# rednote-hilab/dots.ocr

Measured on AMD Instinct MI355X. Metric: pages/sec, dots.ocr 1.7B bf16, A4@200dpi page batch (preprocess + ViT + prefill + 1024-token greedy decode + detokenise), higher is better.
Workload: dtype bf16; 1 GPU; a4: 8 pages/GPU of 1654x2339 px -> 19824 patches, 5200 prompt tokens/page, max_new_tokens=1024, EOS disabled; pages_per_gpu=8, parallelism=dp1, decode_rows_in_flight=64

## Files before the change

### dots_ocr_amd/csrc/engine.hip

```cpp
#include "engine.h"

namespace engine {
namespace {
thread_local std::string g_create_error;

int dense_on(DotsEngine* e, hipStream_t st, uint8_t* aq, float* as, const bf16_t* A, const bf16_t* W, const uint8_t* W8, const float* wscale,
             const bf16_t* bias, const bf16_t* R, void* C, int64_t M, int N, int K, int ldc, int epi) {
    if (!W8) {
        CK(launch_gemm(st, A, W, bias, R, C, M, N, K, K, ldc, epi, wscale));
        return DOTS_OK;
    }
    CK(launch_quant_act_fp8(st, A, aq, as, M, K, K));
    CK(launch_gemm_fp8(st, aq, as, W8, wscale, bias, R, C, M, N, K, ldc, epi));
    return DOTS_OK;
}
int dense(DotsEngine* e, const bf16_t* A, const bf16_t* W, const uint8_t* W8, const float* wscale, const bf16_t* bias, const bf16_t* R, void* C,
          int64_t M, int N, int K, int ldc, int epi) {
    return dense_on(e, e->stream, e->act_q, e->act_s, A, W, W8, wscale, bias, R, C, M, N, K, ldc, epi);
}
int vdense(DotsEngine* e, const bf16_t* A, const bf16_t* W, const uint8_t* W8, const float* wscale, const bf16_t* bias, const bf16_t* R, void* C,
           int64_t M, int N, int K, int ldc, int epi) {
    return dense_on(e, e->vs, e->act_q_v, e->act_s_v, A, W, W8, wscale, bias, R, C, M, N, K, ldc, epi);
}

// ... 696 lines not shown
    if (n_eos) std::copy(eos_ids, eos_ids + n_eos, e->h_eos);
    e->out_cap = max_new_tokens;
    RET(prefill(e, input_ids, prompt_lens, B));

    CK(hipEventRecord(e->ev[4], s));
    const int n_splits = splits_for_ctx(e->cfg.max_seq_len);
    const bool use_graph = getenv("DOTS_OCR_NO_GRAPH") == nullptr;
    hipGraphExec_t exec = nullptr;
    hipGraphExec_t exec_part = nullptr;
    if (use_graph && max_new_tokens > 1) {
        if (e->step_graphs.size() >= 30) drop_step_graphs(e);
        if (e->s_vit) RET(step_graph(e, B, n_splits, max_new_tokens, &exec_part, 1));
        RET(step_graph(e, B, n_splits, max_new_tokens, &exec));
    }
    std::vector<int32_t> fin(DOTS_MAX_BATCH);
    int steps = 0;
    hipStream_t cur = s;
    for (int step = 1; step < max_new_tokens; ++step) {
        if (exec && (step & 15) == 1) RET(pick_decode_stream(e, &cur));
        if (exec) CK(hipGraphLaunch(cur != s && exec_part ? exec_part : exec, cur));
        else RET(decode_step_launches(e, n_splits));
        ++steps;
        if ((n_eos || e->stage.rows(ROW_STOP) > 0) && (step % 16 == 0)) {
            CK(hipMemcpyAsync(fin.data(), e->finished, B * 4, hipMemcpyDeviceToHost, cur));
            CK(hipStreamSynchronize(cur));
            bool all = true;
            for (int b = 0; b < B; ++b) all = all && fin[b];
            if (all) break;
        }
        if (exec && !n_eos && cur != s && (step & 63) == 0) CK(hipStreamSynchronize(cur));
    }
    RET(chain_streams(e, cur, s));
    CK(hipEventRecord(e->ev[5], s));
    CK(hipEventRecord(e->ev[7], s));
    e->steps_done = steps;
    std::vector<int32_t> tmp((size_t)B * max_new_tokens);
    CK(hipMemcpyAsync(tmp.data(), e->out_ids, tmp.size() * 4, hipMemcpyDeviceToHost, s));
    CK(hipMemcpyAsync(out_lens, e->out_lens, B * 4, hipMemcpyDeviceToHost, s));
    CK(hipStreamSynchronize(s));
    std::memcpy(out_ids, tmp.data(), tmp.size() * 4);

    e->stats.decode_steps = steps;
    int64_t newtok = 0;
    double kvb = 0;
    const double kv_tok = (double)e->cfg.num_layers * e->cfg.num_kv_heads * 128 * 2 * (e->kv8 ? 1 : 2);
    for (int b = 0; b < B; ++b) {
        newtok += out_lens[b];
        for (int st = 0; st < steps; ++st) kvb += (double)(prompt_lens[b] + st + 1) * kv_tok;
    }
    e->stats.new_tokens = newtok;
    e->stats.decode_bytes = (double)steps * decode_step_bytes(e->cfg) + kvb;
    return DOTS_OK;
}

int dots_get_stats(DotsEngine* e, DotsStats* out) {
    if (!e || !out) return DOTS_E_INVALID;
    CK(hipSetDevice(e->device));
    CK(hipStreamSynchronize(e->stream));
    if (e->s_vit) CK(hipStreamSynchronize(e->s_vit));
    auto elapsed = [&](hipEvent_t a, hipEvent_t b) {
        float ms = 0;
        if (hipEventElapsedTime(&ms, a, b) != hipSuccess) { (void)hipGetLastError(); ms = 0; }
        return ms;
    };
    auto el = [&](int a, int b) { return elapsed(e->ev[a], e->ev[b]); };
    e->stats.vit_ms = e->stats.vit_patches ? el(0, 1) : 0;
    e->stats.prefill_ms = e->stats.prefill_tokens ? el(2, 3) : 0;
    e->stats.decode_ms = e->stats.decode_steps ? el(4, 5) : 0;
    e->stats.total_ms = e->stats.decode_steps || e->stats.new_tokens ? el(6, 7) : 0;
    float a = 0;
    for (int i = 0; i < e->attn_pairs; ++i) a += elapsed(e->attn_ev[2 * i], e->attn_ev[2 * i + 1]);
    e->stats.vit_attn_ms = a;
    e->stats.vit_attn_launches = e->attn_pairs;
    *out = e->stats;
    return DOTS_OK;
}

int dots_preprocess_image(DotsEngine* e, const uint8_t* rgb, int on_device, int h, int w, int rh, int rw,
                          const int32_t* hcoef, const int32_t* hbounds, int hk, const int32_t* vcoef, const int32_t* vbounds, int vk,
                          const float* mean3, const float* std3, float rescale, float* out) {
    if (!e) return DOTS_E_INVALID;
    const DotsConfig& c = e->cfg;
    const int P = c.v_patch, m = c.v_merge;
    if (!rgb || !out || !mean3 || !std3 || h < 1 || w < 1 || rh < 1 || rw < 1) return e->fail(DOTS_E_INVALID, "bad preprocess arguments");
    if (rh % (P * m) || rw % (P * m)) return e->fail(DOTS_E_INVALID, "resized size %dx%d is not a multiple of patch*merge", rh, rw);
    if ((rw != w && (!hcoef || !hbounds || hk < 1)) || (rh != h && (!vcoef || !vbounds || vk < 1)))
        return e->fail(DOTS_E_INVALID, "missing resample table for a resized axis");
    if (c.v_channels != 3) return e->fail(DOTS_E_INVALID, "only 3-channel images are supported");
    CK(hipSetDevice(e->device));
    hipStream_t s = e->stream;
    auto grow = [&](uint8_t** p, size_t* cap, size_t need) -> hipError_t {
        if (need <= *cap) return hipSuccess;
        if (*p) { hipStreamSynchronize(s); e->release(*p); *p = nullptr; }
        *cap = need + need / 4;
        return e->alloc(p, *cap);
    };
    const size_t in_bytes = (size_t)h * w * 3, tmp_bytes = (size_t)h * rw * 3, out_bytes = (size_t)rh * rw * 3;
    const uint8_t* src = rgb;
    if (!on_device) {
        CK(grow(&e->pp_in, &e->pp_in_cap, in_bytes));
        CK(hipMemcpyAsync(e->pp_in, rgb, in_bytes, hipMemcpyHostToDevice, s));
        src = e->pp_in;
    }
    const size_t tab_ints = (rw != w ? (size_t)rw * (hk + 2) : 0) + (rh != h ? (size_t)rh * (vk + 2) : 0);
    if (tab_ints > e->pp_tab_cap) {
        if (e->pp_tab) { hipStreamSynchronize(s); e->release(e->pp_tab); e->pp_tab = nullptr; }
        e->pp_tab_cap = tab_ints + tab_ints / 4;
        CK(e->alloc(&e->pp_tab, e->pp_tab_cap));
    }
    int32_t* tab = e->pp_tab;
    if (rw != w) {
        CK(grow(&e->pp_tmp, &e->pp_tmp_cap, tmp_bytes));
        CK(hipMemcpyAsync(tab, hcoef, (size_t)rw * hk * 4, hipMemcpyHostToDevice, s));
        CK(hipMemcpyAsync(tab + (size_t)rw * hk, hbounds, (size_t)rw * 2 * 4, hipMemcpyHostToDevice, s));
        CK(launch_resize_h(s, src, e->pp_tmp, tab, tab + (size_t)rw * hk, hk, h, w, rw));
        src = e->pp_tmp;
        tab += (size_t)rw * (hk + 2);
    }
    if (rh != h) {
        CK(grow(&e->pp_out, &e->pp_out_cap, out_bytes));
        CK(hipMemcpyAsync(tab, vcoef, (size_t)rh * vk * 4, hipMemcpyHostToDevice, s));
        CK(hipMemcpyAsync(tab + (size_t)rh * vk, vbounds, (size_t)rh * 2 * 4, hipMemcpyHostToDevice, s));
        CK(launch_resize_v(s, src, e->pp_out, tab, tab + (size_t)rh * vk, vk, rw, rh));
        src = e->pp_out;
    }
    CK(launch_normalize_patchify(s, src, out, rw, rh / P, rw / P, P, m, rescale, mean3, std3));
    CK(hipStreamSynchronize(s));
    return DOTS_OK;
}

int dots_set_decode_plan(DotsEngine* e, int plan) {
    if (!e) return DOTS_E_INVALID;
    if (plan < 0 || plan > 5 || (plan & 6) == 6)
        return e->fail(DOTS_E_INVALID, "decode plan must be 0 (by stream) or 1 (partition plan on every step), + 2 (streaming attention) or + 4 (per-split attention)");
    const int part = plan & 1, stream = (plan & 2) ? 1 : (plan & 4) ? 0 : -1;
    if (part != e->force_part || stream != e->attn_stream) {
        e->force_part = part;
        e->attn_stream = stream;
        drop_step_graphs(e);
    }
    return DOTS_OK;
}

int dots_tower_tail(DotsEngine* e, int set, int* now) {
    if (!e) return DOTS_E_INVALID;
    if (set < -2 || set > e->cfg.v_layers) return e->fail(DOTS_E_INVALID, "tower tail must be -2 (query), -1 (adaptive) or 0 .. v_layers");
    if (set >= -1) e->tail_fixed = set;
    if (now) *now = e->tail_now;
    return DOTS_OK;
}

int dots_set_gemm_plan(DotsEngine* e, int plan) {
    if (!e) return DOTS_E_INVALID;
    if (plan < 0 || plan > 1) return e->fail(DOTS_E_INVALID, "gemm plan must be 0 (8-wave ping-pong) or 1 (one wave per SIMD)");
    gemm_set_plan(plan);
    return DOTS_OK;
}

int dots_get_logits(DotsEngine* e, float* out) {
    if (!e || !out) return DOTS_E_INVALID;
    if (e->B < 1) return e->fail(DOTS_E_STATE, "no prefilled batch");
    CK(hipSetDevice(e->device));
    CK(hipMemcpyAsync(out, e->d_logits, (size_t)e->B * e->cfg.vocab_size * 4, hipMemcpyDeviceToHost, e->stream));
    CK(hipStreamSynchronize(e->stream));
    return DOTS_OK;
}

int dots_set_next_tokens(DotsEngine* e, const int32_t* tokens, int B) {
    if (!e || !tokens || B != e->B) return e ? e->fail(DOTS_E_INVALID, "bad set_next_tokens arguments") : DOTS_E_INVALID;
    CK(hipSetDevice(e->device));
    CK(hipMemcpyAsync(e->cur_tokens, tokens, B * 4, hipMemcpyHostToDevice, e->stream));
    CK(hipStreamSynchronize(e->stream));
    return DOTS_OK;
}

int dots_get_last_tokens(DotsEngine* e, int32_t* out) {
    if (!e || !out) return DOTS_E_INVALID;
    if (e->B < 1) return e->fail(DOTS_E_STATE, "no prefilled batch");
    CK(hipSetDevice(e->device));
    std::vector<int32_t> lens(DOTS_MAX_BATCH), ids((size_t)DOTS_MAX_BATCH * std::max(1, e->out_cap));
    CK(hipMemcpyAsync(lens.data(), e->out_lens, e->B * 4, hipMemcpyDeviceToHost, e->stream));
    CK(hipMemcpyAsync(ids.data(), e->out_ids, (size_t)e->B * e->out_cap * 4, hipMemcpyDeviceToHost, e->stream));
    CK(hipStreamSynchronize(e->stream));
    for (int b = 0; b < e->B; ++b) out[b] = lens[b] > 0 ? ids[(size_t)b * e->out_cap + lens[b] - 1] : -1;
    return DOTS_OK;
}

int dots_debug_capture_hidden(DotsEngine* e, int64_t capacity_elems) {
    if (!e || capacity_elems < 0) return DOTS_E_INVALID;
    CK(hipSetDevice(e->device));
    CK(hipStreamSynchronize(e->stream));
    if (e->dbg_hidden) { e->release(e->dbg_hidden); e->dbg_hidden = nullptr; }
    e->dbg_cap = 0; e->dbg_vit_rows = e->dbg_lm_rows = 0;
    if (capacity_elems > 0) {
        CK(e->alloc(&e->dbg_hidden, (size_t)capacity_elems));
        e->dbg_cap = (size_t)capacity_elems;
    }
    return DOTS_OK;
}

int dots_debug_read_hidden(DotsEngine* e, int which, int layer, void* out_host, int64_t* rows_out) {
    if (!e || !out_host || !rows_out || !e->dbg_hidden) return e ? e->fail(DOTS_E_STATE, "hidden-state capture is off") : DOTS_E_INVALID;
    CK(hipSetDevice(e->device));
    const DotsConfig& c = e->cfg;
    const int64_t rows = which == 0 ? e->dbg_vit_rows : e->dbg_lm_rows;
    const int dim = which == 0 ? c.v_embed_dim : c.hidden_size, n_layers = which == 0 ? c.v_layers : c.num_layers;
    if (rows <= 0 || layer < 0 || layer >= n_layers) return e->fail(DOTS_E_INVALID, "no captured hidden state for layer %d", layer);
    const size_t off = (which == 0 ? 0 : (size_t)c.v_layers * e->dbg_vit_rows * c.v_embed_dim) + (size_t)layer * rows * dim;
    if (off + (size_t)rows * dim > e->dbg_cap) return e->fail(DOTS_E_CAPACITY, "capture buffer too small for layer %d", layer);
    CK(hipMemcpyAsync(out_host, e->dbg_hidden + off, (size_t)rows * dim * 2, hipMemcpyDeviceToHost, e->stream));
    CK(hipStreamSynchronize(e->stream));
    *rows_out = rows;
    return DOTS_OK;
}

int dots_debug_read_kv(DotsEngine* e, int layer, int seq, int pos0, int n, int which, void* out_host) {
    if (!e || !out_host) return e ? e->fail(DOTS_E_INVALID, "null argument") : DOTS_E_INVALID;
    const DotsConfig& c = e->cfg;
    if (layer < 0 || layer >= c.num_layers || seq < 0 || seq >= c.max_batch || pos0 < 0 || n < 1 || (which != 0 && which != 1) ||
        (int64_t)pos0 + n > (int64_t)e->max_pages * PAGE)
        return e->fail(DOTS_E_INVALID, "bad dots_debug_read_kv arguments (layer %d, row %d, positions %d + %d, which %d)", layer, seq, pos0, n, which);
    RET(dots_synchronize(e));
    const int Hkv = c.num_kv_heads, es = e->kv8 ? 1 : 2;
    const size_t page_bytes = (size_t)PAGE_ELEMS * es;
    const uint8_t* base = reinterpret_cast<const uint8_t*>(e->pool) + e->pool_layer_elems * 2 * layer;
    std::vector<uint8_t> pg(page_bytes);
    uint8_t* out = static_cast<uint8_t*>(out_host);
    for (int p = pos0 / PAGE; p <= (pos0 + n - 1) / PAGE; ++p) {
        const int page = e->hp_table[(size_t)seq * e->max_pages + p];
        if (page >= e->n_pool_pages) return e->fail(DOTS_E_STATE, "position %d of row %d is not in the KV cache", std::max(pos0, p * PAGE), seq);
        for (int h = 0; h < Hkv; ++h) {
            CK(hipMemcpyAsync(pg.data(), base + ((size_t)(page * Hkv + h) * 2 + which) * page_bytes, page_bytes, hipMemcpyDeviceToHost, e->stream));
            CK(hipStreamSynchronize(e->stream));
            for (int pos = std::max(pos0, p * PAGE); pos < std::min(pos0 + n, (p + 1) * PAGE); ++pos)
                for (int d = 0; d < 128; ++d) {
                    const int key = pos & (PAGE - 1), el = which == 0 ? k_chunk(key, d) * 8 + (d & 7) : v_off(key, d);
                    const size_t o = ((size_t)h * n + (pos - pos0)) * 128 + d;
                    if (e->kv8) out[o] = pg[kv8_byte(el)];
                    else std::memcpy(out + o * 2, pg.data() + (size_t)el * 2, 2);
                }
        }
    }
    return DOTS_OK;
}

int dots_synchronize(DotsEngine* e) {
    if (!e) return DOTS_E_INVALID;
    CK(hipSetDevice(e->device));
    if (e->s_vit) CK(hipStreamSynchronize(e->s_vit));
    if (e->s_dec) CK(hipStreamSynchronize(e->s_dec));
    CK(hipStreamSynchronize(e->stream));
    return DOTS_OK;
}

int dots_dev_alloc(DotsEngine* e, int64_t bytes, void** out) {
    if (!e || !out || bytes < 0) return DOTS_E_INVALID;
    CK(hipSetDevice(e->device));
    uint8_t* p = nullptr;
    CK(e->alloc(&p, (size_t)bytes));
    *out = p;
    return DOTS_OK;
}
int dots_dev_free(DotsEngine* e, void* p) {
    if (!e) return DOTS_E_INVALID;
    CK(hipSetDevice(e->device));
    CK(hipStreamSynchronize(e->stream));
    e->release(p);
    return DOTS_OK;
}
int dots_memcpy_h2d(DotsEngine* e, void* dst, const void* src, int64_t bytes) {
    if (!e) return DOTS_E_INVALID;
    CK(hipSetDevice(e->device));
    CK(hipMemcpyAsync(dst, src, bytes, hipMemcpyHostToDevice, e->stream));
    CK(hipStreamSynchronize(e->stream));
    return DOTS_OK;
}
int dots_memcpy_d2h(DotsEngine* e, void* dst, const void* src, int64_t bytes) {
    if (!e) return DOTS_E_INVALID;
    CK(hipSetDevice(e->device));
    CK(hipMemcpyAsync(dst, src, bytes, hipMemcpyDeviceToHost, e->stream));
    CK(hipStreamSynchronize(e->stream));
    return DOTS_OK;
}
}
```

### dots_ocr_amd/csrc/gemm.hip

```cpp
#include <cstdlib>
#include <utility>

#include "common.h"
#include "kernels.h"

namespace {

constexpr int BM = 128, BN = 128, BK = 64;
constexpr int TILE_BYTES = 128 * 128;
#ifndef GEMM_GROUP_M
#define GEMM_GROUP_M 8
#endif
constexpr int GROUP_M = GEMM_GROUP_M;

DEVI float gelu_erf(float x) { return 0.5f * x * (1.0f + erff(x * 0.70710678118654752440f)); }
#ifdef GEMM_EXACT_SILU
DEVI float silu(float x) { return x / (1.0f + __expf(-x)); }
#else
DEVI float silu(float x) {
    const float d = 1.0f + __expf(fminf(-x, 80.f));
    const float r = __builtin_amdgcn_rcpf(d);
    const float q = x * r;
    return __builtin_fmaf(__builtin_fmaf(-q, d, x), r, q);
}
#endif

template <int EPI, int FN, int FM = 2>
DEVI void gemm_epilogue(const f32x16 (&acc)[FN][FM], const bf16_t* __restrict__ bias, const float* __restrict__ colscale, const bf16_t* R,
                        void* Cout, int M, int ldc, int nw0, int mw0, int l31, int hi, const float* __restrict__ rowscale = nullptr) {
#pragma unroll
    for (int fm = 0; fm < FM; ++fm) {
        const int m = mw0 + fm * 32 + l31;
        if (m >= M) continue;
        const float rs = rowscale ? rowscale[m] : 1.f;
        if constexpr (EPI == EPI_SWIGLU) {
            bf16_t* C = reinterpret_cast<bf16_t*>(Cout);
#pragma unroll
            for (int fp = 0; fp < FN / 2; ++fp)
#pragma unroll
            for (int rq = 0; rq < 4; ++rq) {
                const int nb = nw0 + fp * 64 + 8 * rq + 4 * hi;
                float o[4];
#pragma unroll
                for (int e = 0; e < 4; ++e) {
                    float g = acc[2 * fp][fm][4 * rq + e], u = acc[2 * fp + 1][fm][4 * rq + e];
                    if (colscale) { g *= colscale[nb + e] * rs; u *= colscale[nb + 32 + e] * rs; }
                    if (bias) { g += bf2f(bias[nb + e]); u += bf2f(bias[nb + 32 + e]); }
                    o[e] = silu(g) * u;
                }
                const int j = (nw0 + fp * 64) / 2 + 8 * rq + 4 * hi;
                u32x2 pk = {pack_bf2(o[0], o[1]), pack_bf2(o[2], o[3])};
                *reinterpret_cast<u32x2*>(C + (size_t)m * ldc + j) = pk;
            }
        } else {
#pragma unroll
            for (int fn = 0; fn < FN; ++fn)
#pragma unroll
                for (int rq = 0; rq < 4; ++rq) {
                    const int nb = nw0 + fn * 32 + 8 * rq + 4 * hi;
                    float o[4];
#pragma unroll
                    for (int e = 0; e < 4; ++e) o[e] = acc[fn][fm][4 * rq + e];
                    if (colscale) {
                        const f32x4 sc = *reinterpret_cast<const f32x4*>(colscale + nb);
#pragma unroll
                        for (int e = 0; e < 4; ++e) o[e] *= sc[e] * rs;
                    }
                    if (bias) {
                        u32x2 bb = *reinterpret_cast<const u32x2*>(bias + nb);
                        o[0] += lo_bf(bb[0]); o[1] += hi_bf(bb[0]); o[2] += lo_bf(bb[1]); o[3] += hi_bf(bb[1]);
                    }
                    if constexpr (EPI == EPI_RESIDUAL) {
                        u32x2 rr = *reinterpret_cast<const u32x2*>(R + (size_t)m * ldc + nb);
                        o[0] += lo_bf(rr[0]); o[1] += hi_bf(rr[0]); o[2] += lo_bf(rr[1]); o[3] += hi_bf(rr[1]);
                    }
                    if constexpr (EPI == EPI_GELU) {
#pragma unroll
                        for (int e = 0; e < 4; ++e) o[e] = gelu_erf(o[e]);
                    }
                    if constexpr (EPI == EPI_F32) {
                        f32x4 v = {o[0], o[1], o[2], o[3]};
                        *reinterpret_cast<f32x4*>(reinterpret_cast<float*>(Cout) + (size_t)m * ldc + nb) = v;
                    } else {
                        u32x2 pk = {pack_bf2(o[0], o[1]), pack_bf2(o[2], o[3])};
                        *reinterpret_cast<u32x2*>(reinterpret_cast<bf16_t*>(Cout) + (size_t)m * ldc + nb) = pk;
                    }
                }
        }
    }
}

template <int EPI, int FM = 2>
DEVI void gemm_epilogue_lds(const f32x16 (&acc)[4][FM], const bf16_t* __restrict__ bias, const float* __restrict__ colscale, const bf16_t* R,
                            bf16_t* __restrict__ C, int M, int ldc, int nw0, int mw0, int l, char* stage, const float* __restrict__ rowscale = nullptr) {
    const int hi = l >> 5, l31 = l & 31;
    constexpr bool SW = EPI == EPI_SWIGLU;
    const int rrow = SW ? (l >> 3) : (l >> 4);
    const int gcol = SW ? ((l & 7) >> 2) * 64 + (l & 3) * 8 : (l & 15) * 8;
    float sc0[8], sc1[8], bi0[8], bi1[8];
#pragma unroll
    for (int e = 0; e < 8; ++e) {
        sc0[e] = colscale ? colscale[nw0 + gcol + e] : 1.f;
        bi0[e] = bias ? bf2f(bias[nw0 + gcol + e]) : 0.f;
        sc1[e] = (SW && colscale) ? colscale[nw0 + gcol + 32 + e] : 1.f;
        bi1[e] = (SW && bias) ? bf2f(bias[nw0 + gcol + 32 + e]) : 0.f;
    }
#pragma unroll
    for (int fm = 0; fm < FM; ++fm) {
#pragma unroll
        for (int fn = 0; fn < 4; ++fn)
#pragma unroll
            for (int rq = 0; rq < 4; ++rq) {
                const int slot = (fn * 8 + rq * 2 + hi) ^ ((l31 & 15) << 1);
                const f32x4 v = {acc[fn][fm][4 * rq], acc[fn][fm][4 * rq + 1], acc[fn][fm][4 * rq + 2], acc[fn][fm][4 * rq + 3]};
                *reinterpret_cast<f32x4*>(stage + l31 * 512 + slot * 16) = v;
            }
#pragma unroll
        for (int it = 0; it < (SW ? 4 : 8); ++it) {
            const int row = it * (SW ? 8 : 4) + rrow;
            const int m = mw0 + fm * 32 + row;
            const int sw = (row & 15) << 1;
            const char* rp = stage + row * 512;
            const int s0 = gcol >> 2;
            const f32x4 a0 = *reinterpret_cast<const f32x4*>(rp + ((s0 ^ sw) << 4)), a1 = *reinterpret_cast<const f32x4*>(rp + (((s0 + 1) ^ sw) << 4));
            float o[8] = {a0[0], a0[1], a0[2], a0[3], a1[0], a1[1], a1[2], a1[3]};
            const float rs = rowscale ? rowscale[min(m, M - 1)] : 1.f;
#pragma unroll
            for (int e = 0; e < 8; ++e) o[e] = o[e] * (sc0[e] * rs) + bi0[e];
            if constexpr (SW) {
                const f32x4 u0 = *reinterpret_cast<const f32x4*>(rp + (((s0 + 8) ^ sw) << 4)), u1 = *reinterpret_cast<const f32x4*>(rp + (((s0 + 9) ^ sw) << 4));
                const float u[8] = {u0[0], u0[1], u0[2], u0[3], u1[0], u1[1], u1[2], u1[3]};
#pragma unroll
                for (int e = 0; e < 8; ++e) o[e] = silu(o[e]) * (u[e] * (sc1[e] * rs) + bi1[e]);
            }
            if (m >= M) continue;
            const int col = SW ? nw0 / 2 + ((l & 7) >> 2) * 32 + (l & 3) * 8 : nw0 + gcol;
            if constexpr (EPI == EPI_RESIDUAL) {
                const u32x4 rr = *reinterpret_cast<const u32x4*>(R + (size_t)m * ldc + col);
#pragma unroll
                for (int e = 0; e < 4; ++e) { o[2 * e] += lo_bf(rr[e]); o[2 * e + 1] += hi_bf(rr[e]); }
            }
            if constexpr (EPI == EPI_GELU) {
#pragma unroll
                for (int e = 0; e < 8; ++e) o[e] = gelu_erf(o[e]);
            }
            const u32x4 pk = {pack_bf2(o[0], o[1]), pack_bf2(o[2], o[3]), pack_bf2(o[4], o[5]), pack_bf2(o[6], o[7])};
            *reinterpret_cast<u32x4*>(C + (size_t)m * ldc + col) = pk;
        }
    }
}

template <int EPI>
__global__ __launch_bounds__(256, 2) void gemm_bf16_kernel(
// ... 178 lines not shown

    const int tid = threadIdx.x;
    const int l = tid & 63;
    const int w = __builtin_amdgcn_readfirstlane(tid >> 6);
    const int hi = l >> 5, l31 = l & 31;
    const int grp = w >> 2;

    int bid = xcd_remap(blockIdx.x, m_tiles * n_tiles);
    const int per_group = group_m * n_tiles;
    const int g = bid / per_group;
    const int first_m = g * group_m;
    const int gsz = min(m_tiles - first_m, group_m);
    const int in_grp = bid - g * per_group;
    const int tm = first_m + in_grp % gsz;
    const int tn = in_grp / gsz;
    const int m0 = tm * BM2, n0 = tn * BN2;

    const bf16_t* gw[2];
    const bf16_t* gx[2];
#pragma unroll
    for (int i = 0; i < 2; ++i) {
        const int row = (i * 8 + w) * 16 + (l >> 2);
        const int slot = (l & 3) ^ ((l >> 4) & 3);
        gw[i] = W + (size_t)(n0 + row) * K + slot * 8;
        gx[i] = A + (size_t)min(m0 + row, M - 1) * lda + slot * 8;
    }
    auto issue_sub = [&](int p) {
        char* base = smem2 + (p & (PP_STAGES - 1)) * SUB_STAGE;
#ifdef PP_DMA_SAME
        p &= 1;
#endif
#pragma unroll
        for (int i = 0; i < 2; ++i) {
            __builtin_amdgcn_global_load_lds((const __attribute__((address_space(1))) void*)(gw[i] + p * SUBK),
                                             (__attribute__((address_space(3))) void*)(base + (i * 8 + w) * 1024), 16, 0, 0);
            __builtin_amdgcn_global_load_lds((const __attribute__((address_space(1))) void*)(gx[i] + p * SUBK),
                                             (__attribute__((address_space(3))) void*)(base + SUB_OP + (i * 8 + w) * 1024), 16, 0, 0);
        }
    };

    const int wn = w >> 2, wm = w & 3;
    const int rsw = (l31 >> 2) & 3;
    const int a_off = (wn * 128 + l31) * 64;
    const int b_off = SUB_OP + (wm * 64 + l31) * 64;

    f32x16 acc[4][2];
#pragma unroll
    for (int i = 0; i < 4; ++i)
#pragma unroll
        for (int j = 0; j < 2; ++j)
#pragma unroll
            for (int r = 0; r < 16; ++r) acc[i][j][r] = 0.f;

    const int ns = K / SUBK;
    issue_sub(0);
    if (ns > 1) issue_sub(1);
    if (ns > 2) issue_sub(2);
    if (ns > 2) asm volatile("s_waitcnt vmcnt(8)" ::: "memory");
    else if (ns > 1) asm volatile("s_waitcnt vmcnt(4)" ::: "memory");
    else asm volatile("s_waitcnt vmcnt(0)" ::: "memory");
    __builtin_amdgcn_s_barrier();
    if (grp == 1) __builtin_amdgcn_s_barrier();
    __builtin_amdgcn_sched_barrier(0);

    for (int p = 0; p < ns; ++p) {
        const char* base = smem2 + (p & (PP_STAGES - 1)) * SUB_STAGE;
        bf16x8 af[2][4], bf_[2][2];
#ifdef PP_NO_LDS
        if (p == 0)
#endif
#pragma unroll
        for (int ks = 0; ks < 2; ++ks) {
            const int slot = ((ks * 2 + hi) ^ rsw) << 4;
            bf_[ks][0] = *reinterpret_cast<const bf16x8*>(base + b_off + slot);
            bf_[ks][1] = *reinterpret_cast<const bf16x8*>(base + b_off + 32 * 64 + slot);
#pragma unroll
            for (int fn = 0; fn < 4; ++fn) af[ks][fn] = *reinterpret_cast<const bf16x8*>(base + a_off + fn * 32 * 64 + slot);
        }
        __builtin_amdgcn_sched_barrier(0);
#ifdef PP_NO_DMA
        if (false) {
#else
        if (p + PP_LOOKAHEAD < ns) {
#endif
            issue_sub(p + PP_LOOKAHEAD);
            asm volatile("s_waitcnt vmcnt(8)" ::: "memory");
        } else {
            asm volatile("s_waitcnt vmcnt(0)" ::: "memory");
        }
        asm volatile("s_waitcnt lgkmcnt(0)" ::: "memory");
        __builtin_amdgcn_sched_barrier(0);
        __builtin_amdgcn_s_barrier();
        __builtin_amdgcn_sched_barrier(0);
        __builtin_amdgcn_s_setprio(1);
#ifdef PP_NO_MFMA
        if (p == 0)
#endif
#pragma unroll
        for (int ks = 0; ks < 2; ++ks)
#pragma unroll
            for (int fn = 0; fn < 4; ++fn) {
                acc[fn][0] = __builtin_amdgcn_mfma_f32_32x32x16_bf16(af[ks][fn], bf_[ks][0], acc[fn][0], 0, 0, 0);
                acc[fn][1] = __builtin_amdgcn_mfma_f32_32x32x16_bf16(af[ks][fn], bf_[ks][1], acc[fn][1], 0, 0, 0);
            }
#ifdef PP_NO_MFMA
        else { PINV(af[0][0]); PINV(af[1][3]); PINV(bf_[0][0]); PINV(bf_[1][1]); }
#endif
        __builtin_amdgcn_s_setprio(0);
        __builtin_amdgcn_sched_barrier(0);
        if (grp == 0 || p + 1 < ns) __builtin_amdgcn_s_barrier();
        __builtin_amdgcn_sched_barrier(0);
    }
#ifdef PP_NO_STORE
#pragma unroll
    for (int i = 0; i < 4; ++i) { PINV(acc[i][0]); PINV(acc[i][1]); }
#else
    if constexpr (EPI == EPI_F32 || EPI == EPI_SWIGLU) {
        gemm_epilogue<EPI, 4>(acc, bias, colscale, R, Cout, M, ldc, n0 + wn * 128, m0 + wm * 64, l31, hi);
    } else {
        __syncthreads();
        gemm_epilogue_lds<EPI>(acc, bias, colscale, R, reinterpret_cast<bf16_t*>(Cout), M, ldc, n0 + wn * 128, m0 + wm * 64, l, smem2 + w * 16384);
    }
#endif
}

constexpr int W4_UNIT = 256 * 128, W4_RING = 5;

struct W4Cols { float sc0[8], bi0[8], sc1[8], bi1[8]; };
template <bool SW>
DEVI void w4_load_cols(W4Cols& cc, const bf16_t* __restrict__ bias, const float* __restrict__ colscale, int nw0, int l) {
    const int gcol = SW ? ((l & 7) >> 2) * 64 + (l & 3) * 8 : (l & 15) * 8;
    u32x4 b0 = {0, 0, 0, 0}, b1 = {0, 0, 0, 0};
    f32x4 s00 = {1.f, 1.f, 1.f, 1.f}, s01 = s00, s10 = s00, s11 = s00;
    if (bias) {
        b0 = *reinterpret_cast<const u32x4*>(bias + nw0 + gcol);
        if (SW) b1 = *reinterpret_cast<const u32x4*>(bias + nw0 + gcol + 32);
    }
    if (colscale) {
        s00 = *reinterpret_cast<const f32x4*>(colscale + nw0 + gcol);
        s01 = *reinterpret_cast<const f32x4*>(colscale + nw0 + gcol + 4);
        if (SW) {
            s10 = *reinterpret_cast<const f32x4*>(colscale + nw0 + gcol + 32);
            s11 = *reinterpret_cast<const f32x4*>(colscale + nw0 + gcol + 36);
        }
    }
#pragma unroll
    for (int e = 0; e < 4; ++e) {
        cc.sc0[e] = s00[e]; cc.sc0[4 + e] = s01[e]; cc.sc1[e] = s10[e]; cc.sc1[4 + e] = s11[e];
        cc.bi0[2 * e] = lo_bf(b0[e]); cc.bi0[2 * e + 1] = hi_bf(b0[e]);
        cc.bi1[2 * e] = lo_bf(b1[e]); cc.bi1[2 * e + 1] = hi_bf(b1[e]);
    }
}

template <int EPI, bool FULL>
DEVI void w4_epilogue_lds(const f32x16 (&acc)[4][4], const W4Cols& cc, bool has_cols, const bf16_t* R,
                          bf16_t* __restrict__ C, int M, int ldc, int nw0, int mw0, int l, char* stage2) {
    const int hi = l >> 5, l31 = l & 31;
    constexpr bool SW = EPI == EPI_SWIGLU;
    constexpr int ITS = SW ? 4 : 8, RPI = SW ? 8 : 4;
    const int rrow = SW ? (l >> 3) : (l >> 4);
    const int gcol = SW ? ((l & 7) >> 2) * 64 + (l & 3) * 8 : (l & 15) * 8;
    const int col = SW ? nw0 / 2 + ((l & 7) >> 2) * 32 + (l & 3) * 8 : nw0 + gcol;
    u32x4 rr[2][8];
    auto load_r = [&](int fm, u32x4 (&dst)[8]) {
        if constexpr (EPI == EPI_RESIDUAL) {
#pragma unroll
            for (int it = 0; it < ITS; ++it) {
                const int m = FULL ? mw0 + fm * 32 + it * RPI + rrow : min(mw0 + fm * 32 + it * RPI + rrow, M - 1);
                dst[it] = *reinterpret_cast<const u32x4*>(R + (size_t)m * ldc + col);
            }
        }
    };
#ifdef W4_OLD_SWZ
    auto swz = [](int row) { return (row & 15) << 1; };
#else
    auto swz = [](int row) { return ((row & 15) << 1) ^ (row & 1) ^ ((row & 2) << 2); };
#endif
    const int wslot = swz(l31);
    char* const wrow = stage2 + l31 * 512;
#define W4_PUT(FM, IMG)                                                                                                   \
    _Pragma("unroll") for (int fn = 0; fn < 4; ++fn) _Pragma("unroll") for (int rq = 0; rq < 4; ++rq) {                     \
        const f32x4 v = {acc[fn][FM][4 * rq], acc[fn][FM][4 * rq + 1], acc[fn][FM][4 * rq + 2], acc[fn][FM][4 * rq + 3]};   \
        *reinterpret_cast<f32x4*>(wrow + (IMG) * 16384 + (((fn * 8 + rq * 2 + hi) ^ wslot) << 4)) = v;                      \
    }
    load_r(0, rr[0]);
    W4_PUT(0, 0)
#pragma unroll
    for (int fm = 0; fm < 4; ++fm) {
        if (fm + 1 < 4) {
            load_r(fm + 1, rr[(fm + 1) & 1]);
            if (fm == 0) { W4_PUT(1, 1) } else if (fm == 1) { W4_PUT(2, 0) } else { W4_PUT(3, 1) }
        }
        __builtin_amdgcn_sched_barrier(0);
        const char* img = stage2 + (fm & 1) * 16384;
        f32x4 a[ITS][SW ? 4 : 2];
#pragma unroll
        for (int it = 0; it < ITS; ++it) {
            const int row = it * RPI + rrow;
            const int sw = swz(row);
            const char* rp = img + row * 512;
            const int s0 = gcol >> 2;
            a[it][0] = *reinterpret_cast<const f32x4*>(rp + ((s0 ^ sw) << 4));
            a[it][1] = *reinterpret_cast<const f32x4*>(rp + (((s0 + 1) ^ sw) << 4));
            if constexpr (SW) {
                a[it][2] = *reinterpret_cast<const f32x4*>(rp + (((s0 + 8) ^ sw) << 4));
                a[it][3] = *reinterpret_cast<const f32x4*>(rp + (((s0 + 9) ^ sw) << 4));
            }
        }
        __builtin_amdgcn_sched_barrier(0);
#pragma unroll
        for (int it = 0; it < ITS; ++it) {
            const int m = mw0 + fm * 32 + it * RPI + rrow;
            float o[8] = {a[it][0][0], a[it][0][1], a[it][0][2], a[it][0][3], a[it][1][0], a[it][1][1], a[it][1][2], a[it][1][3]};
            float u[8];
            if constexpr (SW) {
#pragma unroll
                for (int e = 0; e < 8; ++e) u[e] = a[it][2 + (e >> 2)][e & 3];
            }
            if (has_cols) {
#pragma unroll
                for (int e = 0; e < 8; ++e) o[e] = o[e] * cc.sc0[e] + cc.bi0[e];
                if constexpr (SW) {
#pragma unroll
                    for (int e = 0; e < 8; ++e) u[e] = u[e] * cc.sc1[e] + cc.bi1[e];
                }
            }
            if constexpr (SW) {
#pragma unroll
                for (int e = 0; e < 8; ++e) o[e] = silu(o[e]) * u[e];
            }
            if constexpr (EPI == EPI_RESIDUAL) {
                const u32x4 r4 = rr[fm & 1][it];
#pragma unroll
                for (int e = 0; e < 4; ++e) { o[2 * e] += lo_bf(r4[e]); o[2 * e + 1] += hi_bf(r4[e]); }
            }
            if constexpr (EPI == EPI_GELU) {
#pragma unroll
                for (int e = 0; e < 8; ++e) o[e] = gelu_erf(o[e]);
            }
            if (FULL || m < M) {
                const u32x4 pk = {pack_bf2(o[0], o[1]), pack_bf2(o[2], o[3]), pack_bf2(o[4], o[5]), pack_bf2(o[6], o[7])};
                *reinterpret_cast<u32x4*>(C + (size_t)m * ldc + col) = pk;
            }
        }
        __builtin_amdgcn_sched_barrier(0);
    }
#undef W4_PUT
}

DEVI void w4_load_cols_rope(W4Cols& cc, const bf16_t* __restrict__ bias, const float* __restrict__ colscale, int nw0, int l) {
    const int gcol = (l & 15) * 8, pcol = gcol ^ 64;
    u32x4 b0 = {0, 0, 0, 0}, b1 = {0, 0, 0, 0};
    f32x4 s00 = {1.f, 1.f, 1.f, 1.f}, s01 = s00, s10 = s00, s11 = s00;
    if (bias) {
        b0 = *reinterpret_cast<const u32x4*>(bias + nw0 + gcol);
        b1 = *reinterpret_cast<const u32x4*>(bias + nw0 + pcol);
    }
    if (colscale) {
        s00 = *reinterpret_cast<const f32x4*>(colscale + nw0 + gcol);
        s01 = *reinterpret_cast<const f32x4*>(colscale + nw0 + gcol + 4);
        s10 = *reinterpret_cast<const f32x4*>(colscale + nw0 + pcol);
        s11 = *reinterpret_cast<const f32x4*>(colscale + nw0 + pcol + 4);
    }
#pragma unroll
    for (int e = 0; e < 4; ++e) {
        cc.sc0[e] = s00[e]; cc.sc0[4 + e] = s01[e]; cc.sc1[e] = s10[e]; cc.sc1[4 + e] = s11[e];
        cc.bi0[2 * e] = lo_bf(b0[e]); cc.bi0[2 * e + 1] = hi_bf(b0[e]);
        cc.bi1[2 * e] = lo_bf(b1[e]); cc.bi1[2 * e + 1] = hi_bf(b1[e]);
    }
}

template <bool FULL>
DEVI void w4_epilogue_qkrope(const f32x16 (&acc)[4][4], const W4Cols& cc, bool has_cols, const float2* __restrict__ cs, bf16_t* __restrict__ dst,
                             int M, int mw0, int l, char* stage2) {
    const int hi = l >> 5, l31 = l & 31;
    const int rrow = l >> 4, gcol = (l & 15) * 8;
    const bool lo_half = (l & 8) == 0;
    const float2* const tab = cs + (gcol & 63);
    auto swz = [](int row) { return ((row & 15) << 1) ^ (row & 1) ^ ((row & 2) << 2); };
    const int wslot = swz(l31);
    char* const wrow = stage2 + l31 * 512;
#define W4_PUT(FM, IMG)                                                                                                   \
    _Pragma("unroll") for (int fn = 0; fn < 4; ++fn) _Pragma("unroll") for (int rq = 0; rq < 4; ++rq) {                     \
        const f32x4 v = {acc[fn][FM][4 * rq], acc[fn][FM][4 * rq + 1], acc[fn][FM][4 * rq + 2], acc[fn][FM][4 * rq + 3]};   \
        *reinterpret_cast<f32x4*>(wrow + (IMG) * 16384 + (((fn * 8 + rq * 2 + hi) ^ wslot) << 4)) = v;                      \
    }
    f32x4 tb[2][2][4];
    auto load_t = [&](int qb, f32x4 (&d)[2][4]) {
#pragma unroll
        for (int it = 0; it < 2; ++it) {
            const int m = FULL ? mw0 + qb * 8 + it * 4 + rrow : min(mw0 + qb * 8 + it * 4 + rrow, M - 1);
            const f32x4* tp = reinterpret_cast<const f32x4*>(tab + (size_t)m * 64);
#pragma unroll
            for (int c = 0; c < 4; ++c) d[it][c] = tp[c];
        }
    };
    load_t(0, tb[0]);
    W4_PUT(0, 0)
#pragma unroll
    for (int qb = 0; qb < 16; ++qb) {
        const int fm = qb >> 2;
        if (qb + 1 < 16) load_t(qb + 1, tb[(qb + 1) & 1]);
        if ((qb & 3) == 0 && fm + 1 < 4) {
            if (fm == 0) { W4_PUT(1, 1) } else if (fm == 1) { W4_PUT(2, 0) } else { W4_PUT(3, 1) }
        }
        __builtin_amdgcn_sched_barrier(0);
        const char* img = stage2 + (fm & 1) * 16384;
        f32x4 a[2][4];
#pragma unroll
        for (int it = 0; it < 2; ++it) {
            const int row = (qb & 3) * 8 + it * 4 + rrow;
            const int sw = swz(row);
            const char* rp = img + row * 512;
            const int s0 = gcol >> 2;
            a[it][0] = *reinterpret_cast<const f32x4*>(rp + ((s0 ^ sw) << 4));
            a[it][1] = *reinterpret_cast<const f32x4*>(rp + (((s0 + 1) ^ sw) << 4));
            a[it][2] = *reinterpret_cast<const f32x4*>(rp + ((s0 ^ 16 ^ sw) << 4));
            a[it][3] = *reinterpret_cast<const f32x4*>(rp + (((s0 + 1) ^ 16 ^ sw) << 4));
        }
        __builtin_amdgcn_sched_barrier(0);
#pragma unroll
        for (int it = 0; it < 2; ++it) {
            const int m = mw0 + qb * 8 + it * 4 + rrow;
            float o[8] = {a[it][0][0], a[it][0][1], a[it][0][2], a[it][0][3], a[it][1][0], a[it][1][1], a[it][1][2], a[it][1][3]};
            float u[8] = {a[it][2][0], a[it][2][1], a[it][2][2], a[it][2][3], a[it][3][0], a[it][3][1], a[it][3][2], a[it][3][3]};
            if (has_cols) {
#pragma unroll
                for (int e = 0; e < 8; ++e) { o[e] = o[e] * cc.sc0[e] + cc.bi0[e]; u[e] = u[e] * cc.sc1[e] + cc.bi1[e]; }
            }
            uint32_t pk[4];
#pragma unroll
            for (int e = 0; e < 4; ++e) {
                const uint32_t ow = pack_bf2(o[2 * e], o[2 * e + 1]), uw = pack_bf2(u[2 * e], u[2 * e + 1]);
                const float x0 = lo_bf(ow), x1 = hi_bf(ow), y0 = lo_bf(uw), y1 = hi_bf(uw);
                const f32x4 t4 = tb[qb & 1][it][e];
                const float f0 = lo_half ? x0 : y0, g0 = lo_half ? t4[0] : t4[1], m0 = lo_half ? y0 : x0, n0_ = lo_half ? t4[1] : t4[0];
                const float p0 = m0 * n0_, p1 = y1 * t4[3];
                const float r0 = __builtin_fmaf(f0, g0, lo_half ? -p0 : p0), r1 = __builtin_fmaf(x1, t4[2], lo_half ? -p1 : p1);
                pk[e] = pack_bf2(r0, r1);
            }
            if (FULL || m < M) *reinterpret_cast<u32x4*>(dst + (size_t)m * 128 + gcol) = u32x4{pk[0], pk[1], pk[2], pk[3]};
        }
        __builtin_amdgcn_sched_barrier(0);
    }
#undef W4_PUT
}

template <int... I, class F> DEVI void gemm_static_for_impl(std::integer_sequence<int, I...>, F&& f) { (f(std::integral_constant<int, I>{}), ...); }
template <int N, class F> DEVI void gemm_static_for(F&& f) { gemm_static_for_impl(std::make_integer_sequence<int, N>{}, f); }

template <int EPI>
DEVI void gemm_bf16_w4_body(
    const bf16_t* __restrict__ A, const bf16_t* __restrict__ W, const bf16_t* __restrict__ bias,
    const float* __restrict__ colscale, const bf16_t* R, void* Cout, int M, int N, int K, int lda, int ldc, int m_tiles, int n_tiles, int group_m, const QkRope& rope) {
    extern __shared__ __attribute__((aligned(16))) char smem2[];
    (void)rope;

    const int tid = threadIdx.x;
    const int l = tid & 63;
    const int w = __builtin_amdgcn_readfirstlane(tid >> 6);
    const int hi = l >> 5, l31 = l & 31;

    int bid = xcd_remap(blockIdx.x, m_tiles * n_tiles);
    const int per_group = group_m * n_tiles;
    const int g = bid / per_group;
    const int first_m = g * group_m;
    const int gsz = min(m_tiles - first_m, group_m);
    const int in_grp = bid - g * per_group;
    const int tm = first_m + in_grp % gsz;
    const int tn = in_grp / gsz;
    const int m0 = tm * BM2, n0 = tn * BN2;

    const int prow = 8 * w + (l >> 3);
    const int chunk = ((l & 7) ^ ((4 * w + (l >> 4)) & 7)) << 4;
    const int w_src = prow * (K * 2) + chunk;
    int x_src[8];
#pragma unroll
    for (int i = 0; i < 8; ++i) x_src[i] = (min(m0 + prow + 32 * i, M - 1) - m0) * (lda * 2) + chunk;
    const __amdgpu_buffer_rsrc_t rw = __builtin_amdgcn_make_buffer_rsrc((void*)(W + (size_t)n0 * K), 0, 0x7ffffff0, 0x00020000);
    const __amdgpu_buffer_rsrc_t rx = __builtin_amdgcn_make_buffer_rsrc((void*)(A + (size_t)m0 * lda), 0, 0x7ffffff0, 0x00020000);
    const int w_step = 32 * K * 2;
    auto dma_w = [&](int t, int slot, int i) {
        __builtin_amdgcn_raw_ptr_buffer_load_lds(rw, (__attribute__((address_space(3))) void*)(smem2 + slot * W4_UNIT + (w + 4 * i) * 1024), 16, w_src,
                                                 t * 128 + i * w_step, 0, 0);
    };
    auto dma_x = [&](int t, int slot, int i) {
        __builtin_amdgcn_raw_ptr_buffer_load_lds(rx, (__attribute__((address_space(3))) void*)(smem2 + slot * W4_UNIT + (w + 4 * i) * 1024), 16, x_src[i],
                                                 t * 128, 0, 0);
    };

    const int wn = w >> 1, wm = w & 1;
    const int rsw = (l31 >> 1) & 7;
    const int lane_sw = ((hi ^ (rsw & 1)) << 4) | ((rsw >> 1) << 5);
    const int lds0 = (int)(uintptr_t)(__attribute__((address_space(3))) char*)smem2;
    const int a_lane = lds0 + (wn * 128 + l31) * 128 + lane_sw;
    const int b_lane = lds0 + (wm * 128 + l31) * 128 + lane_sw;
    auto frag = [&](int base, int ks, int f) {
        return *reinterpret_cast<const __attribute__((address_space(3))) bf16x8*>((uintptr_t)(uint32_t)((base ^ (ks << 5)) + f * 4096));
    };

#ifdef W4_PROF
    const unsigned long long pt0 = __builtin_amdgcn_s_memtime(), pw0 = wall_clock64();
#endif
    W4Cols cols;
    if constexpr (EPI == EPI_QKROPE) w4_load_cols_rope(cols, bias, colscale, n0 + wn * 128, l);
    else if constexpr (EPI != EPI_F32) w4_load_cols<EPI == EPI_SWIGLU>(cols, bias, colscale, n0 + wn * 128, l);

    f32x16 acc[4][4];
#pragma unroll
    for (int i = 0; i < 4; ++i)
#pragma unroll
        for (int j = 0; j < 4; ++j)
#pragma unroll
            for (int r = 0; r < 16; ++r) acc[i][j][r] = 0.f;

    const int nt = K / BK;
#ifdef W4_STAGGER
    if (blockIdx.x < 256) {
        const int naps = ((blockIdx.x >> 3) & 7) * nt * W4_STAGGER / 8;
        for (int i = 0; i < naps; ++i) __builtin_amdgcn_s_sleep(8);
    }
#endif
#pragma unroll
    for (int u = 0; u < 4; ++u)
#pragma unroll
        for (int i = 0; i < 8; ++i) {
            if (u & 1) dma_x(u >> 1, u, i);
            else dma_w(u >> 1, u, i);
        }
    asm volatile("s_waitcnt vmcnt(16)" ::: "memory");
    __builtin_amdgcn_s_barrier();
    bf16x8 fa[2][4], fb[2][4];
#pragma unroll
    for (int f = 0; f < 4; ++f) { fa[0][f] = frag(a_lane, 0, f); fb[0][f] = frag(b_lane + W4_UNIT, 0, f); }
#ifdef W4_PROF
    const unsigned long long pt1 = __builtin_amdgcn_s_memtime(), pw1 = wall_clock64();
#endif

    auto tile_body = [&](auto mode_c, int t, int u0) {
        constexpr int MODE = decltype(mode_c)::value;
        const int s1 = u0 + 1 >= W4_RING ? u0 + 1 - W4_RING : u0 + 1, s2 = u0 + 2 >= W4_RING ? u0 + 2 - W4_RING : u0 + 2;
        const int s3 = u0 + 3 >= W4_RING ? u0 + 3 - W4_RING : u0 + 3, s4 = u0 + 4 >= W4_RING ? u0 + 4 - W4_RING : u0 + 4;
        const int aw = a_lane + u0 * W4_UNIT, ax = b_lane + s1 * W4_UNIT;
        const int awn = a_lane + s2 * W4_UNIT, axn = b_lane + s3 * W4_UNIT;
        gemm_static_for<64>([&acc, &fa, &fb, &frag, &dma_w, &dma_x, aw, ax, awn, axn, t, u0, s4](auto gc) {
            constexpr int gp = decltype(gc)::value;
            (void)acc; (void)t; (void)u0; (void)s4; (void)dma_w; (void)dma_x;
            constexpr int ks = gp >> 4, idx = gp & 15, fn = idx >> 2, fm = idx & 3, cur = ks & 1;
            if constexpr (gp == 48 && MODE < 2) {
                if constexpr (MODE == 0) asm volatile("s_waitcnt vmcnt(8) lgkmcnt(0)" ::: "memory");
                else asm volatile("s_waitcnt vmcnt(0) lgkmcnt(0)" ::: "memory");
                __builtin_amdgcn_s_barrier();
            }
            if constexpr (idx < 8 && (ks < 3 || MODE < 2)) {
                constexpr int f = idx & 3;
                if constexpr (ks < 3) {
                    if constexpr (idx < 4) fa[cur ^ 1][f] = frag(aw, ks + 1, f);
                    else fb[cur ^ 1][f] = frag(ax, ks + 1, f);
                } else {
                    if constexpr (idx < 4) fa[cur ^ 1][f] = frag(awn, 0, f);
                    else fb[cur ^ 1][f] = frag(axn, 0, f);
                }
            }
#ifndef W4_NO_DMA
            if constexpr (MODE == 0) {
                if constexpr (gp == 8 || gp == 11 || gp == 14 || gp == 24 || gp == 27 || gp == 30 || gp == 40 || gp == 43) {
                    constexpr int i = gp < 16 ? (gp - 8) / 3 : gp < 32 ? 3 + (gp - 24) / 3 : 6 + (gp - 40) / 3;
                    dma_w(t + 2, s4, i);
                }
                if constexpr (gp >= 56) dma_x(t + 2, u0, gp - 56);
            }
#endif
            asm volatile("v_mfma_f32_32x32x16_bf16 %[d], %[a], %[b], %[d]" : [d] "+a"(acc[fn][fm]) : [a] "v"(fa[cur][fn]), [b] "v"(fb[cur][fm]));
        });
    };
    int u0 = 0;
    for (int t = 0; t < nt - 2; ++t) {
        tile_body(std::integral_constant<int, 0>{}, t, u0);
        u0 = u0 + 2 >= W4_RING ? u0 + 2 - W4_RING : u0 + 2;
    }
    tile_body(std::integral_constant<int, 1>{}, nt - 2, u0);
    u0 = u0 + 2 >= W4_RING ? u0 + 2 - W4_RING : u0 + 2;
    tile_body(std::integral_constant<int, 2>{}, nt - 1, u0);

#ifdef W4_PROF
    const unsigned long long pt2 = __builtin_amdgcn_s_memtime(), pw2 = wall_clock64();
#endif
    __syncthreads();
#ifdef W4_NO_STORE
#pragma unroll
    for (int i = 0; i < 4; ++i)
#pragma unroll
        for (int j = 0; j < 4; ++j) asm volatile("" ::"a"(acc[i][j]));
    return;
#endif
#ifdef W4_OLD_EPILOGUE
    if constexpr (EPI == EPI_F32 || EPI == EPI_SWIGLU) {
        gemm_epilogue<EPI, 4, 4>(acc, bias, colscale, R, Cout, M, ldc, n0 + wn * 128, m0 + wm * 128, l31, hi);
    } else {
        gemm_epilogue_lds<EPI, 4>(acc, bias, colscale, R, reinterpret_cast<bf16_t*>(Cout), M, ldc, n0 + wn * 128, m0 + wm * 128, l, smem2 + w * 16384);
    }
#else
    if constexpr (EPI == EPI_QKROPE) {
        const int head = (n0 + wn * 128) >> 7;
        const bool full = m0 + wm * 128 + 128 <= M, has_cols = bias != nullptr || colscale != nullptr;
        if (head < rope.n_rope_heads) {
            bf16_t* dst = head < rope.Hq ? rope.q + (size_t)head * rope.T * 128 : rope.k + (size_t)(head - rope.Hq) * rope.T * 128;
            if (full) w4_epilogue_qkrope<true>(acc, cols, has_cols, rope.cs, dst, M, m0 + wm * 128, l, smem2 + w * 32768);
            else w4_epilogue_qkrope<false>(acc, cols, has_cols, rope.cs, dst, M, m0 + wm * 128, l, smem2 + w * 32768);
        } else if (full) {
            w4_epilogue_lds<EPI_NONE, true>(acc, cols, has_cols, R, reinterpret_cast<bf16_t*>(Cout), M, ldc, n0 + wn * 128, m0 + wm * 128, l, smem2 + w * 32768);
        } else {
            w4_epilogue_lds<EPI_NONE, false>(acc, cols, has_cols, R, reinterpret_cast<bf16_t*>(Cout), M, ldc, n0 + wn * 128, m0 + wm * 128, l, smem2 + w * 32768);
        }
    } else if constexpr (EPI == EPI_F32) {
        gemm_epilogue<EPI, 4, 4>(acc, bias, colscale, R, Cout, M, ldc, n0 + wn * 128, m0 + wm * 128, l31, hi);
    } else if (m0 + wm * 128 + 128 <= M) {
        w4_epilogue_lds<EPI, true>(acc, cols, bias != nullptr || colscale != nullptr, R, reinterpret_cast<bf16_t*>(Cout), M, ldc, n0 + wn * 128, m0 + wm * 128, l, smem2 + w * 32768);
    } else {
        w4_epilogue_lds<EPI, false>(acc, cols, bias != nullptr || colscale != nullptr, R, reinterpret_cast<bf16_t*>(Cout), M, ldc, n0 + wn * 128, m0 + wm * 128, l, smem2 + w * 32768);
    }
#endif
#ifdef W4_PROF
    const unsigned long long pt2b = __builtin_amdgcn_s_memtime();
    asm volatile("s_waitcnt vmcnt(0)" ::: "memory");
    const unsigned long long pt3 = __builtin_amdgcn_s_memtime(), pw3 = wall_clock64();
    if ((blockIdx.x == 1000 || blockIdx.x == 2001 || blockIdx.x == 3002) && tid == 0)
        printf("W4_PROF epi %d N %d K %d blk %d: prologue %llu cyc / %.2f us, main loop %llu cyc / %.2f us (%.0f cyc per K tile), epilogue + drain %llu cyc / %.2f us; issue %llu drain %llu\n", EPI, N, K,
               (int)blockIdx.x, pt1 - pt0, (pw1 - pw0) * 0.01, pt2 - pt1, (pw2 - pw1) * 0.01, (double)(pt2 - pt1) / nt, pt3 - pt2, (pw3 - pw2) * 0.01, pt2b - pt2, pt3 - pt2b);
#endif
}

template <int EPI>
__global__ __launch_bounds__(256) void gemm_bf16_w4_kernel(
    const bf16_t* __restrict__ A, const bf16_t* __restrict__ W, const bf16_t* __restrict__ bias,
    const float* __restrict__ colscale, const bf16_t* R, void* Cout, int M, int N, int K, int lda, int ldc, int m_tiles, int n_tiles, int group_m) {
    gemm_bf16_w4_body<EPI>(A, W, bias, colscale, R, Cout, M, N, K, lda, ldc, m_tiles, n_tiles, group_m, QkRope{});
}
__global__ __launch_bounds__(256) void gemm_bf16_w4_qkrope_kernel(
    const bf16_t* __restrict__ A, const bf16_t* __restrict__ W, const bf16_t* __restrict__ bias,
    const float* __restrict__ colscale, void* Cout, int M, int N, int K, int lda, int ldc, int m_tiles, int n_tiles, int group_m, QkRope rope) {
    gemm_bf16_w4_body<EPI_QKROPE>(A, W, bias, colscale, nullptr, Cout, M, N, K, lda, ldc, m_tiles, n_tiles, group_m, rope);
}

typedef __attribute__((ext_vector_type(8))) int i32x8;

template <int EPI>
__global__ __launch_bounds__(512, 2) void gemm_fp8_256pp_kernel(
    const uint8_t* __restrict__ A, const float* __restrict__ rowscale, const uint8_t* __restrict__ W, const float* __restrict__ colscale,
    const bf16_t* __restrict__ bias, const bf16_t* R, void* Cout, int M, int N, int K, int ldc, int m_tiles, int n_tiles, int group_m) {
    extern __shared__ __attribute__((aligned(16))) char smem2[];
    constexpr int SUBK8 = 64;

    const int tid = threadIdx.x;
    const int l = tid & 63;
    const int w = __builtin_amdgcn_readfirstlane(tid >> 6);
    const int hi = l >> 5, l31 = l & 31;
    const int grp = w >> 2;

    int bid = xcd_remap(blockIdx.x, m_tiles * n_tiles);
    const int per_group = group_m * n_tiles;
    const int g = bid / per_group;
    const int first_m = g * group_m;
    const int gsz = min(m_tiles - first_m, group_m);
    const int in_grp = bid - g * per_group;
    const int tm = first_m + in_grp % gsz;
    const int tn = in_grp / gsz;
    const int m0 = tm * BM2, n0 = tn * BN2;

    const uint8_t* gw[2];
    const uint8_t* gx[2];
#pragma unroll
    for (int i = 0; i < 2; ++i) {
        const int row = (i * 8 + w) * 16 + (l >> 2);
        const int slot = (l & 3) ^ ((l >> 4) & 3);
        gw[i] = W + (size_t)(n0 + row) * K + slot * 16;
        gx[i] = A + (size_t)min(m0 + row, M - 1) * K + slot * 16;
    }
    auto issue_sub = [&](int p) {
        char* base = smem2 + (p & (PP_STAGES - 1)) * SUB_STAGE;
#pragma unroll
        for (int i = 0; i < 2; ++i) {
            __builtin_amdgcn_global_load_lds((const __attribute__((address_space(1))) void*)(gw[i] + p * SUBK8),
                                             (__attribute__((address_space(3))) void*)(base + (i * 8 + w) * 1024), 16, 0, 0);
            __builtin_amdgcn_global_load_lds((const __attribute__((address_space(1))) void*)(gx[i] + p * SUBK8),
                                             (__attribute__((address_space(3))) void*)(base + SUB_OP + (i * 8 + w) * 1024), 16, 0, 0);
        }
    };

    const int wn = w >> 2, wm = w & 3;
    const int rsw = (l31 >> 2) & 3;
    const int a_off = (wn * 128 + l31) * 64;
    const int b_off = SUB_OP + (wm * 64 + l31) * 64;
    const int s_lo = ((2 * hi) ^ rsw) << 4, s_hi = ((2 * hi + 1) ^ rsw) << 4;

    f32x16 acc[4][2];
#pragma unroll
    for (int i = 0; i < 4; ++i)
#pragma unroll
        for (int j = 0; j < 2; ++j)
#pragma unroll
            for (int r = 0; r < 16; ++r) acc[i][j][r] = 0.f;

    const int ns = K / SUBK8;
    issue_sub(0);
    if (ns > 1) issue_sub(1);
    if (ns > 2) issue_sub(2);
    if (ns > 2) asm volatile("s_waitcnt vmcnt(8)" ::: "memory");
    else if (ns > 1) asm volatile("s_waitcnt vmcnt(4)" ::: "memory");
    else asm volatile("s_waitcnt vmcnt(0)" ::: "memory");
    __builtin_amdgcn_s_barrier();
    if (grp == 1) __builtin_amdgcn_s_barrier();
    __builtin_amdgcn_sched_barrier(0);

    auto frag = [&](const char* rowp) {
        const u32x4 lo = *reinterpret_cast<const u32x4*>(rowp + s_lo), hi4 = *reinterpret_cast<const u32x4*>(rowp + s_hi);
        const i32x8 v = {(int)lo[0], (int)lo[1], (int)lo[2], (int)lo[3], (int)hi4[0], (int)hi4[1], (int)hi4[2], (int)hi4[3]};
        return v;
    };
    for (int p = 0; p < ns; ++p) {
        const char* base = smem2 + (p & (PP_STAGES - 1)) * SUB_STAGE;
        i32x8 af[4], bf_[2];
        bf_[0] = frag(base + b_off);
        bf_[1] = frag(base + b_off + 32 * 64);
#pragma unroll
        for (int fn = 0; fn < 4; ++fn) af[fn] = frag(base + a_off + fn * 32 * 64);
        __builtin_amdgcn_sched_barrier(0);
        if (p + PP_LOOKAHEAD < ns) {
            issue_sub(p + PP_LOOKAHEAD);
            asm volatile("s_waitcnt vmcnt(8)" ::: "memory");
        } else {
            asm volatile("s_waitcnt vmcnt(0)" ::: "memory");
        }
        asm volatile("s_waitcnt lgkmcnt(0)" ::: "memory");
        __builtin_amdgcn_sched_barrier(0);
        __builtin_amdgcn_s_barrier();
        __builtin_amdgcn_sched_barrier(0);
        __builtin_amdgcn_s_setprio(1);
#pragma unroll
        for (int fn = 0; fn < 4; ++fn) {
            acc[fn][0] = __builtin_amdgcn_mfma_scale_f32_32x32x64_f8f6f4(af[fn], bf_[0], acc[fn][0], 0, 0, 0, 0x7f7f7f7f, 0, 0x7f7f7f7f);
            acc[fn][1] = __builtin_amdgcn_mfma_scale_f32_32x32x64_f8f6f4(af[fn], bf_[1], acc[fn][1], 0, 0, 0, 0x7f7f7f7f, 0, 0x7f7f7f7f);
        }
        __builtin_amdgcn_s_setprio(0);
        __builtin_amdgcn_sched_barrier(0);
        if (grp == 0 || p + 1 < ns) __builtin_amdgcn_s_barrier();
        __builtin_amdgcn_sched_barrier(0);
    }
    if constexpr (EPI == EPI_SWIGLU) {
        gemm_epilogue<EPI, 4>(acc, bias, colscale, R, Cout, M, ldc, n0 + wn * 128, m0 + wm * 64, l31, hi, rowscale);
    } else {
        __syncthreads();
        gemm_epilogue_lds<EPI>(acc, bias, colscale, R, reinterpret_cast<bf16_t*>(Cout), M, ldc, n0 + wn * 128, m0 + wm * 64, l, smem2 + w * 16384, rowscale);
    }
}

}

static int raster_group_m(int row_bytes) {
    const int panel = 256 * row_bytes;
    return panel >= (4 << 20) ? 2 : panel >= (3 << 19) ? 4 : GROUP_M;
}

static int g_gemm_plan = -1;
int gemm_get_plan() {
    int p = __atomic_load_n(&g_gemm_plan, __ATOMIC_RELAXED);
    if (p < 0) {
        const char* ev = getenv("DOTS_OCR_GEMM_PLAN");
        p = ev ? (atoi(ev) != 0) : 1;
        __atomic_store_n(&g_gemm_plan, p, __ATOMIC_RELAXED);
    }
    return p;
}
void gemm_set_plan(int plan) { __atomic_store_n(&g_gemm_plan, plan != 0, __ATOMIC_RELAXED); }

template <int E>
static hipError_t launch_256(hipStream_t s, const bf16_t* A, const bf16_t* W, const bf16_t* bias, const float* colscale, const bf16_t* R, void* C,
                                int M, int N, int K, int lda, int ldc) {
    static uint32_t configured = 0;
    int dev = 0;
    hipError_t e = hipGetDevice(&dev);
    if (e != hipSuccess) return e;
    const uint32_t bit = 1u << (dev & 31);
    if (!(__atomic_load_n(&configured, __ATOMIC_ACQUIRE) & bit)) {
        e = hipFuncSetAttribute(reinterpret_cast<const void*>(&gemm_bf16_256_kernel<E>), hipFuncAttributeMaxDynamicSharedMemorySize, 2 * STAGE2);
        if (e != hipSuccess) return e;
        __atomic_fetch_or(&configured, bit, __ATOMIC_RELEASE);
    }
    const int m_tiles = (M + BM2 - 1) / BM2, n_tiles = N / BN2;
    static const bool lockstep = getenv("DOTS_OCR_GEMM_LOCKSTEP") != nullptr;
    if (lockstep || ldc % 8 != 0) {
        hipLaunchKernelGGL(gemm_bf16_256_kernel<E>, dim3(m_tiles * n_tiles), dim3(512), 2 * STAGE2, s, A, W, bias, colscale, R, C, M, N, K,
                           lda, ldc, m_tiles, n_tiles);
        return hipGetLastError();
    }
    if (gemm_get_plan() == 1 && K / BK >= 3) {
        static uint32_t configured_w4 = 0;
        if (!(__atomic_load_n(&configured_w4, __ATOMIC_ACQUIRE) & bit)) {
            e = hipFuncSetAttribute(reinterpret_cast<const void*>(&gemm_bf16_w4_kernel<E>), hipFuncAttributeMaxDynamicSharedMemorySize, W4_RING * W4_UNIT);
            if (e != hipSuccess) return e;
            __atomic_fetch_or(&configured_w4, bit, __ATOMIC_RELEASE);
        }
        hipLaunchKernelGGL(gemm_bf16_w4_kernel<E>, dim3(m_tiles * n_tiles), dim3(256), W4_RING * W4_UNIT, s, A, W, bias, colscale, R, C, M, N, K,
                           lda, ldc, m_tiles, n_tiles, raster_group_m(K * 2));
        return hipGetLastError();
    }
    static uint32_t configured_pp = 0;
    if (!(__atomic_load_n(&configured_pp, __ATOMIC_ACQUIRE) & bit)) {
        e = hipFuncSetAttribute(reinterpret_cast<const void*>(&gemm_bf16_256pp_kernel<E>), hipFuncAttributeMaxDynamicSharedMemorySize,
                                PP_STAGES * SUB_STAGE);
        if (e != hipSuccess) return e;
        __atomic_fetch_or(&configured_pp, bit, __ATOMIC_RELEASE);
    }
    hipLaunchKernelGGL(gemm_bf16_256pp_kernel<E>, dim3(m_tiles * n_tiles), dim3(512), PP_STAGES * SUB_STAGE, s, A, W, bias, colscale, R, C, M, N, K,
                       lda, ldc, m_tiles, n_tiles, raster_group_m(K * 2));
    return hipGetLastError();
}

hipError_t launch_gemm(hipStream_t s, const bf16_t* A, const bf16_t* W, const bf16_t* bias, const bf16_t* R,
                       void* C, int64_t M, int N, int K, int lda, int ldc, int epi, const float* colscale) {
    if (M <= 0) return hipSuccess;
    if (N % BN != 0 || K % BK != 0 || (lda % 8) != 0 || (ldc % 4) != 0) return hipErrorInvalidValue;
    static const bool force_small = getenv("DOTS_OCR_GEMM_128") != nullptr;
    if (N % BN2 == 0 && !force_small) {
        switch (epi) {
            case EPI_NONE: return launch_256<EPI_NONE>(s, A, W, bias, colscale, R, C, (int)M, N, K, lda, ldc);
            case EPI_RESIDUAL: return launch_256<EPI_RESIDUAL>(s, A, W, bias, colscale, R, C, (int)M, N, K, lda, ldc);
            case EPI_SWIGLU: return launch_256<EPI_SWIGLU>(s, A, W, bias, colscale, R, C, (int)M, N, K, lda, ldc);
            case EPI_GELU: return launch_256<EPI_GELU>(s, A, W, bias, colscale, R, C, (int)M, N, K, lda, ldc);
            case EPI_F32: return launch_256<EPI_F32>(s, A, W, bias, colscale, R, C, (int)M, N, K, lda, ldc);
            default: return hipErrorInvalidValue;
        }
    }
    const int m_tiles = (int)((M + BM - 1) / BM), n_tiles = N / BN;
    dim3 grid(m_tiles * n_tiles), block(256);
#define LAUNCH(E)                                                                                       \
    hipLaunchKernelGGL(gemm_bf16_kernel<E>, grid, block, 0, s, A, W, bias, colscale, R, C, (int)M, N, K, lda, ldc, \
                       m_tiles, n_tiles)
    switch (epi) {
        case EPI_NONE: LAUNCH(EPI_NONE); break;
        case EPI_RESIDUAL: LAUNCH(EPI_RESIDUAL); break;
        case EPI_SWIGLU: LAUNCH(EPI_SWIGLU); break;
        case EPI_GELU: LAUNCH(EPI_GELU); break;
        case EPI_F32: LAUNCH(EPI_F32); break;
        default: return hipErrorInvalidValue;
    }
#undef LAUNCH
    return hipGetLastError();
}

hipError_t launch_gemm_qk_rope(hipStream_t s, const bf16_t* A, const bf16_t* W, const bf16_t* bias, bf16_t* qkv, int64_t M, int N, int K, int lda, int ldc,
                               const float2* cs, bf16_t* q, bf16_t* k, int Hq, int Hkv) {
    static const bool off = getenv("DOTS_OCR_QK_FUSE") && atoi(getenv("DOTS_OCR_QK_FUSE")) == 0;
    static const bool lockstep = getenv("DOTS_OCR_GEMM_LOCKSTEP") != nullptr, force_small = getenv("DOTS_OCR_GEMM_128") != nullptr;
    if (off || lockstep || force_small || gemm_get_plan() != 1 || N != (Hq + 2 * Hkv) * 128 || N % BN2 != 0 || K % BK != 0 || K / BK < 3 || lda % 8 != 0 || ldc % 8 != 0 ||
        !cs || !q || !k || M > 0x7fffffff)
        return hipErrorNotSupported;
    if (M <= 0) return hipSuccess;
    static uint32_t configured = 0;
    int dev = 0;
    hipError_t e = hipGetDevice(&dev);
    if (e != hipSuccess) return e;
    const uint32_t bit = 1u << (dev & 31);
    if (!(__atomic_load_n(&configured, __ATOMIC_ACQUIRE) & bit)) {
        e = hipFuncSetAttribute(reinterpret_cast<const void*>(&gemm_bf16_w4_qkrope_kernel), hipFuncAttributeMaxDynamicSharedMemorySize, W4_RING * W4_UNIT);
        if (e != hipSuccess) return e;
        __atomic_fetch_or(&configured, bit, __ATOMIC_RELEASE);
    }
    const int m_tiles = (int)((M + BM2 - 1) / BM2), n_tiles = N / BN2;
    const QkRope rope{cs, q, k, (long long)M, Hq, Hq + Hkv};
    hipLaunchKernelGGL(gemm_bf16_w4_qkrope_kernel, dim3(m_tiles * n_tiles), dim3(256), W4_RING * W4_UNIT, s, A, W, bias, (const float*)nullptr, (void*)qkv, (int)M, N, K,
                       lda, ldc, m_tiles, n_tiles, raster_group_m(K * 2), rope);
    return hipGetLastError();
}

bool gemm_fp8_supports(int N, int K) { return N % BN2 == 0 && K % 64 == 0; }

template <int E>
static hipError_t launch_fp8_t(hipStream_t s, const uint8_t* Aq, const float* rowscale, const uint8_t* Wq, const float* colscale, const bf16_t* bias,
                               const bf16_t* R, void* C, int M, int N, int K, int ldc) {
    static uint32_t configured = 0;
    int dev = 0;
    hipError_t e = hipGetDevice(&dev);
    if (e != hipSuccess) return e;
    const uint32_t bit = 1u << (dev & 31);
    if (!(__atomic_load_n(&configured, __ATOMIC_ACQUIRE) & bit)) {
        e = hipFuncSetAttribute(reinterpret_cast<const void*>(&gemm_fp8_256pp_kernel<E>), hipFuncAttributeMaxDynamicSharedMemorySize, PP_STAGES * SUB_STAGE);
        if (e != hipSuccess) return e;
        __atomic_fetch_or(&configured, bit, __ATOMIC_RELEASE);
    }
    const int m_tiles = (M + BM2 - 1) / BM2, n_tiles = N / BN2;
    hipLaunchKernelGGL(gemm_fp8_256pp_kernel<E>, dim3(m_tiles * n_tiles), dim3(512), PP_STAGES * SUB_STAGE, s, Aq, rowscale, Wq, colscale, bias, R, C, M, N, K,
                       ldc, m_tiles, n_tiles, raster_group_m(K));
    return hipGetLastError();
}

hipError_t launch_gemm_fp8(hipStream_t s, const uint8_t* Aq, const float* rowscale, const uint8_t* Wq, const float* colscale, const bf16_t* bias,
                           const bf16_t* R, void* C, int64_t M, int N, int K, int ldc, int epi) {
    if (M <= 0) return hipSuccess;
    if (!gemm_fp8_supports(N, K) || ldc % 8 != 0 || !rowscale || !colscale) return hipErrorInvalidValue;
    switch (epi) {
        case EPI_NONE: return launch_fp8_t<EPI_NONE>(s, Aq, rowscale, Wq, colscale, bias, R, C, (int)M, N, K, ldc);
        case EPI_RESIDUAL: return launch_fp8_t<EPI_RESIDUAL>(s, Aq, rowscale, Wq, colscale, bias, R, C, (int)M, N, K, ldc);
        case EPI_SWIGLU: return launch_fp8_t<EPI_SWIGLU>(s, Aq, rowscale, Wq, colscale, bias, R, C, (int)M, N, K, ldc);
        case EPI_GELU: return launch_fp8_t<EPI_GELU>(s, Aq, rowscale, Wq, colscale, bias, R, C, (int)M, N, K, ldc);
        default: return hipErrorInvalidValue;
    }
}
```

### dots_ocr_amd/csrc/ops.hip

```cpp
#include "engine.h"

using namespace engine;

namespace {
int op_weight(DotsEngine* e, Scratch& sc, const bf16_t* w, int64_t rows, int K, int Hq, int Hkv, bool qkv, int fp8, void** wd, float** scale) {
    *scale = nullptr;
    if (fp8) {
        bf16_t* q = nullptr;
        uint8_t* d = nullptr;
        CK(sc.get(&q, (size_t)rows * K));
        CK(sc.get(scale, (size_t)rows));
        CK(sc.get(&d, (size_t)((rows + 15) / 16 * 16) * K));
        CK(hipMemcpyAsync(q, w, (size_t)rows * K * 2, hipMemcpyDeviceToDevice, e->stream));
        CK(launch_quant_rows_fp8(e->stream, q, *scale, rows, K));
        CK(launch_pack_frag_fp8(e->stream, q, d, rows, K, qkv ? (Hq + Hkv) * 128 : 0));
        *wd = d;
    } else {
        bf16_t* d = nullptr;
        CK(sc.get(&d, (size_t)((rows + 15) / 16 * 16) * K));
        if (qkv) CK(launch_pack_frag_qkv(e->stream, w, d, Hq, Hkv, K));
        else CK(launch_pack_frag(e->stream, w, d, rows, K));
        *wd = d;
    }
    return DOTS_OK;
// ... 101 lines not shown
    CK(sc.get(&own_d, B));
    CK(sc.get(&thr, B));
    CK(sc.get(&cnt, (size_t)B * V));
    CK(sc.get(&seen, (size_t)B * W));
    CK(sc.get(&pen, (size_t)B * V));
    CK(sc.get(&pval, (size_t)B * 64));
    CK(sc.get(&pidx, (size_t)B * 64));
    CK(sc.get(&cur, B));
    CK(sc.get(&ctx, B));
    CK(sc.get(&ids, (size_t)B * (hist_stride + 1)));
    CK(sc.get(&lens, B));
    CK(sc.get(&fin, B));
    CK(hipMemcpyAsync(tab, rp.data(), B * sizeof(RowParams), hipMemcpyHostToDevice, e->stream));
    CK(hipMemcpyAsync(own_d, own.data(), B * 4, hipMemcpyHostToDevice, e->stream));
    CK(launch_pen_history(e->stream, hist_dev, hist_lens_dev, hist_stride, n_prompt_dev, B, V, cnt, seen, lens));
    StepState st;
    st.cur_tokens = cur; st.ctx_len = ctx; st.out_ids = ids; st.out_lens = lens; st.finished = fin;
    st.eos_ids = e->eos_ids; st.sel = nullptr; st.max_len = nullptr;
    st.n_eos = rules_host ? e->n_eos : 0; st.out_stride = hist_stride + 1; st.cap = hist_stride + 2; st.advance_ctx = 0;
    RowRules* rtab = nullptr;
    float* img = nullptr;
    if (rules_host) {
        int32_t* stage = nullptr;
        CK(sc.get(&rtab, DOTS_MAX_BATCH));
        CK(sc.get(&img, (size_t)B * V));
        CK(sc.get(&stage, (size_t)V + 2 * DOTS_MAX_LOGIT_BIAS));
        for (int b = 0; b < B; ++b) {
            const DotsLogitRules& r = rules_host[b];
            if (!r.n_bias && !r.allowed_ids && !r.min_tokens && !r.n_stop && !r.ignore_eos) continue;
            RowRules rr;
            RET(check_logit_rules(e, r, V, e->h_eos, e->n_eos, &rr));
            const int n_allowed = r.allowed_ids ? r.n_allowed : 0;
            if (n_allowed) CK(hipMemcpyAsync(stage, r.allowed_ids, (size_t)n_allowed * 4, hipMemcpyHostToDevice, e->stream));
            if (r.n_bias) {
                CK(hipMemcpyAsync(stage + V, r.bias_ids, (size_t)r.n_bias * 4, hipMemcpyHostToDevice, e->stream));
                CK(hipMemcpyAsync(stage + V + DOTS_MAX_LOGIT_BIAS, r.bias_values, (size_t)r.n_bias * 4, hipMemcpyHostToDevice, e->stream));
            }
            CK(launch_set_row_rules(e->stream, rtab, img, b, V, rr, stage, n_allowed, stage + V,
                                    reinterpret_cast<const float*>(stage + V + DOTS_MAX_LOGIT_BIAS), r.n_bias));
            CK(hipStreamSynchronize(e->stream));
        }
        if (n_gen_host) CK(hipMemcpyAsync(lens, n_gen_host, B * 4, hipMemcpyHostToDevice, e->stream));
    }
    RowSel rs{tab, own_d, cnt, seen, pen, thr, 0, rtab, img, GuideSel{}, NgramSel{}};
    if (ngram_host) {
        RowNgram* ntab = nullptr;
        uint32_t* nmask = nullptr;
        CK(sc.get(&ntab, DOTS_MAX_BATCH));
        CK(sc.get(&nmask, (size_t)B * ngram_mask_words(V)));
        CK(hipMemcpyAsync(ntab, ngrams.data(), DOTS_MAX_BATCH * sizeof(RowNgram), hipMemcpyHostToDevice, e->stream));
        CK(launch_ngram_history(e->stream, hist_dev, hist_lens_dev, hist_stride, n_prompt_dev, B, ids, st.out_stride));
        rs.ngram = NgramSel{ntab, nmask, ngram_mask_words(V), V};
    }
    RowGuide* gtab = nullptr;
    int32_t* gstates = nullptr;
    if (guide_ids_host) {
        uint32_t* gmask = nullptr;
        CK(sc.get(&gtab, DOTS_MAX_BATCH));
        CK(sc.get(&gstates, DOTS_MAX_BATCH));
        CK(sc.get(&gmask, (size_t)B * guide_mask_words(V)));
        std::vector<RowGuide> rows(DOTS_MAX_BATCH, RowGuide{});
        for (int b = 0; b < B; ++b) {
            if (guide_ids_host[b] < 0) continue;
            const DotsEngine::Guide& g = e->guides[guide_ids_host[b]];
            rows[b] = RowGuide{g.table, g.accepting, g.n_states, g.start, states_host[b], 0};
        }
        CK(hipMemcpyAsync(gtab, rows.data(), DOTS_MAX_BATCH * sizeof(RowGuide), hipMemcpyHostToDevice, e->stream));
        CK(hipMemcpyAsync(gstates, states_host, B * 4, hipMemcpyHostToDevice, e->stream));
        CK(hipStreamSynchronize(e->stream));
        rs.guide = GuideSel{gtab, gmask, e->tok_off, e->tok_bytes, guide_mask_words(V), V};
    }
    auto run = [&]() -> hipError_t {
        if (rs.guide.rows) {
            hipError_t r = launch_guide_set_states(e->stream, gtab, gstates, B);
            if (r != hipSuccess) return r;
        }
        if (mode == 0) return launch_argmax_step(e->stream, logits_dev, V, V, B, pval, pidx, st);
        if (mode == 1) return launch_sample_step(e->stream, logits_dev, V, V, B, rp[0].temperature, rp[0].top_p, rp[0].seed, st);
        return launch_row_stage(e->stream, logits_dev, V, V, B, rs, pval, pidx, st, iters > 0 ? nullptr : st.finished);
    };
    if (iters <= 0) {
        CK(run());
        CK(hipMemcpyAsync(out_tokens_dev, cur, B * 4, hipMemcpyDeviceToDevice, e->stream));
        std::vector<RowGuide> after(states_out_host ? B : 0);
        if (states_out_host) CK(hipMemcpyAsync(after.data(), gtab, B * sizeof(RowGuide), hipMemcpyDeviceToHost, e->stream));
        CK(hipStreamSynchronize(e->stream));
        for (size_t b = 0; b < after.size(); ++b) states_out_host[b] = after[b].table ? after[b].state : -1;
        return DOTS_OK;
    }
    const std::vector<int32_t> ones(B, 1);
    CK(hipMemcpyAsync(fin, ones.data(), B * 4, hipMemcpyHostToDevice, e->stream));
    for (int i = 0; i < 3; ++i) CK(run());
    return time_replays(e, iters, run, ms);
}

int logprobs_op(DotsEngine* e, const float* logits_dev, int B, int V, int ld, const int32_t* top_n_host, const int32_t* chosen_dev,
                float* tok_lp_dev, int32_t* top_ids_dev, float* top_lp_dev, int which, int iters, float* ms) {
    if (!e || !logits_dev || B < 1 || B > DOTS_MAX_BATCH || V < 1 || V > LP_MAX_V || ld < V || !top_n_host || which < 0 || which > 2)
        return e ? e->fail(DOTS_E_INVALID, "bad logprobs arguments") : DOTS_E_INVALID;
    for (int b = 0; b < B; ++b)
        if (top_n_host[b] < -1 || top_n_host[b] > DOTS_MAX_TOP_LOGPROBS) return e->fail(DOTS_E_INVALID, "top_n of row %d not in [-1, %d]", b, DOTS_MAX_TOP_LOGPROBS);
    CK(hipSetDevice(e->device));
    Scratch sc(e);
    const size_t K = DOTS_MAX_TOP_LOGPROBS;
    int32_t *tn = nullptr, *pi = nullptr, *pos = nullptr, *cho = nullptr, *ids = nullptr;
    float *ms_p = nullptr, *pv = nullptr, *tok = nullptr, *top = nullptr;
    CK(sc.get(&tn, B));
    CK(sc.get(&ms_p, (size_t)B * LP_CHUNKS * 2));
    CK(sc.get(&pv, (size_t)B * LP_CHUNKS * K));
    CK(sc.get(&pi, (size_t)B * LP_CHUNKS * K));
    CK(sc.get(&pos, B));
    if (!chosen_dev) { CK(sc.get(&cho, B)); chosen_dev = cho; }
    if (!tok_lp_dev) { CK(sc.get(&tok, B)); CK(sc.get(&ids, (size_t)B * K)); CK(sc.get(&top, (size_t)B * K)); tok_lp_dev = tok; top_ids_dev = ids; top_lp_dev = top; }
    CK(hipMemcpyAsync(tn, top_n_host, B * 4, hipMemcpyHostToDevice, e->stream));
    const LogprobState ls{tn, nullptr, nullptr, nullptr, chosen_dev, ms_p, pv, pi, pos, tok_lp_dev, top_ids_dev, top_lp_dev, 1};
    auto run = [&](int w) -> hipError_t {
        hipError_t r = hipSuccess;
        if (w != 2) r = launch_logprob_partial(e->stream, logits_dev, V, ld, B, ls);
        if (r == hipSuccess && w != 1) r = launch_logprob_final(e->stream, logits_dev, V, ld, B, ls);
        return r;
    };
    if (iters <= 0) {
        CK(run(0));
        CK(hipStreamSynchronize(e->stream));
        return DOTS_OK;
    }
    for (int i = 0; i < 3; ++i) CK(run(0));
    return time_replays(e, iters, [&] { return run(which); }, ms);
}
}

extern "C" {
int dots_op_rmsnorm(DotsEngine* e, const void* x, const void* w, void* y, int64_t rows, int dim, float eps) {
    if (!e) return DOTS_E_INVALID;
    CK(hipSetDevice(e->device));
    CK(launch_rmsnorm(e->stream, (const bf16_t*)x, (const bf16_t*)w, (bf16_t*)y, rows, dim, eps));
    return DOTS_OK;
}
int dots_op_layernorm(DotsEngine* e, const void* x, const void* w, const void* b, void* y, int64_t rows, int dim, float eps) {
    if (!e) return DOTS_E_INVALID;
    CK(hipSetDevice(e->device));
    CK(launch_layernorm(e->stream, (const bf16_t*)x, (const bf16_t*)w, (const bf16_t*)b, (bf16_t*)y, rows, dim, eps));
    return DOTS_OK;
}
int dots_op_gemm(DotsEngine* e, const void* A, const void* W, const void* bias, const void* residual, void* C,
                 int64_t M, int N, int K, int epilogue, const float* colscale) {
    if (!e) return DOTS_E_INVALID;
    CK(hipSetDevice(e->device));
    const int ldc = epilogue == EPI_SWIGLU ? N / 2 : N;
    CK(launch_gemm(e->stream, (const bf16_t*)A, (const bf16_t*)W, (const bf16_t*)bias, (const bf16_t*)residual, C, M, N, K, K, ldc, epilogue, colscale));
    return DOTS_OK;
}

int dots_op_gemm_fp8(DotsEngine* e, const void* A, const void* W, const void* bias, const void* residual, void* C, int64_t M, int N, int K,
                     int epilogue) {
    if (!e || !A || !W || !C) return e ? e->fail(DOTS_E_INVALID, "null argument") : DOTS_E_INVALID;
    if (!gemm_fp8_supports(N, K) || epilogue == EPI_F32) return e->fail(DOTS_E_INVALID, "fp8 GEMM needs N %% 256 == 0, K %% 64 == 0 and a bf16 output");
    CK(hipSetDevice(e->device));
    Scratch sc(e);
    bf16_t* wq = nullptr;
    uint8_t *w8 = nullptr, *a8 = nullptr;
    float *ws = nullptr, *as = nullptr;
    CK(sc.get(&wq, (size_t)N * K));
    CK(sc.get(&w8, (size_t)N * K));
    CK(sc.get(&ws, (size_t)N));
    CK(sc.get(&a8, (size_t)M * K));
    CK(sc.get(&as, (size_t)M));
    CK(hipMemcpyAsync(wq, W, (size_t)N * K * 2, hipMemcpyDeviceToDevice, e->stream));
    CK(launch_quant_rows_fp8(e->stream, wq, ws, N, K));
    CK(launch_bf16q_to_fp8(e->stream, wq, w8, (int64_t)N * K));
    CK(launch_quant_act_fp8(e->stream, (const bf16_t*)A, a8, as, M, K, K));
    const int ldc = epilogue == EPI_SWIGLU ? N / 2 : N;
    CK(launch_gemm_fp8(e->stream, a8, as, w8, ws, (const bf16_t*)bias, (const bf16_t*)residual, C, M, N, K, ldc, epilogue));
    CK(hipStreamSynchronize(e->stream));
    return DOTS_OK;
}

int dots_op_quant_fp8(DotsEngine* e, void* w_inout, float* scale_out, int64_t N, int K) {
    if (!e || !w_inout || !scale_out) return e ? e->fail(DOTS_E_INVALID, "null argument") : DOTS_E_INVALID;
    CK(hipSetDevice(e->device));
    CK(launch_quant_rows_fp8(e->stream, (bf16_t*)w_inout, scale_out, N, K));
    CK(hipStreamSynchronize(e->stream));
    return DOTS_OK;
}

static int upload_lists(DotsEngine* e, const int32_t* cu, int n_seq, int Hq, std::vector<Tile64>& tiles, std::vector<QBlock>& qb,
                        Tile64** d_tiles, QBlock** d_qb, int64_t* Tpad) {
    std::vector<int> lens(n_seq);
    for (int i = 0; i < n_seq; ++i) lens[i] = cu[i + 1] - cu[i];
    build_worklists(lens, Hq, tiles, qb, Tpad);
    CK(e->alloc(d_tiles, tiles.size() + 1));
    CK(e->alloc(d_qb, qb.size() + 1));
    CK(hipMemcpyAsync(*d_tiles, tiles.data(), tiles.size() * sizeof(Tile64), hipMemcpyHostToDevice, e->stream));
    CK(hipMemcpyAsync(*d_qb, qb.data(), qb.size() * sizeof(QBlock), hipMemcpyHostToDevice, e->stream));
    CK(hipStreamSynchronize(e->stream));
    return DOTS_OK;
}

int dots_op_flash_attn(DotsEngine* e, const void* q, const void* k, const void* vt, void* out, const int32_t* cu, int n_seq,
                       int Hq, int Hkv, int causal, float scale) {
    if (!e || !cu || n_seq < 1) return DOTS_E_INVALID;
    CK(hipSetDevice(e->device));
    std::vector<Tile64> tiles;
    std::vector<QBlock> qb;
    Tile64* dt = nullptr;
    QBlock* dq = nullptr;
    int64_t Tpad = 0;
    RET(upload_lists(e, cu, n_seq, Hq, tiles, qb, &dt, &dq, &Tpad));
    const int64_t T = cu[n_seq];
    const XcdPlan xcd_plan = make_xcd_plan(qb.data(), (int)qb.size());
    hipError_t r = launch_flash_attn(e->stream, (const bf16_t*)q, (const bf16_t*)k, (const bf16_t*)vt, (bf16_t*)out, dq, (int)qb.size(), T, Tpad, Hq, Hkv, causal, scale, &xcd_plan);
    hipStreamSynchronize(e->stream);
    e->release(dt);
    e->release(dq);
    CK(r);
    return DOTS_OK;
}

int dots_plan_flash_xcd(const int32_t* lens, int n_seq, int Hq, int32_t* base8, int32_t* cnt8, int64_t* cost8) {
    if (!lens || n_seq < 1 || Hq < 1 || !base8 || !cnt8 || !cost8) return DOTS_E_INVALID;
    std::vector<int> L(lens, lens + n_seq);
    for (int n : L)
        if (n < 1) return DOTS_E_INVALID;
    std::vector<Tile64> tiles;
    std::vector<QBlock> qb;
    int64_t Tpad = 0;
    build_worklists(L, Hq, tiles, qb, &Tpad);
    const XcdPlan p = make_xcd_plan(qb.data(), (int)qb.size());
    for (int x = 0; x < 8; ++x) {
        base8[x] = p.base[x];
        cnt8[x] = p.cnt[x];
        cost8[x] = 0;
        for (int i = p.base[x]; i < p.base[x] + p.cnt[x]; ++i) cost8[x] += ((qb[i].n + 63) / 64 + 1) & ~1;
    }
    return (int)qb.size();
}

int dots_op_qkv_rope_split(DotsEngine* e, const void* qkv, void* q, void* k, void* vt, const int32_t* cu, int n_seq,
                           const int32_t* pos_host, int Hq, int Hkv, int rope2d, float theta) {
    if (!e || !cu || n_seq < 1 || !pos_host) return DOTS_E_INVALID;
    CK(hipSetDevice(e->device));
    std::vector<Tile64> tiles;
    std::vector<QBlock> qb;
    Tile64* dt = nullptr;
    QBlock* dq = nullptr;
    int64_t Tpad = 0;
    RET(upload_lists(e, cu, n_seq, Hq, tiles, qb, &dt, &dq, &Tpad));
    const int64_t T = cu[n_seq];
    int32_t* dpos = nullptr;
    float2* cs = nullptr;
    float* freq = nullptr;
    const int nf = rope2d ? 32 : 64;
    std::vector<float> f(nf);
    for (int i = 0; i < nf; ++i) f[i] = 1.0f / powf(theta, (float)(2 * i) / (rope2d ? 64.0f : 128.0f));
    CK(e->alloc(&dpos, (size_t)T * (rope2d ? 2 : 1)));
    CK(e->alloc(&cs, (size_t)T * 64));
    CK(e->alloc(&freq, (size_t)nf));
    CK(hipMemcpyAsync(dpos, pos_host, (size_t)T * (rope2d ? 2 : 1) * 4, hipMemcpyHostToDevice, e->stream));
    CK(hipMemcpyAsync(freq, f.data(), nf * 4, hipMemcpyHostToDevice, e->stream));
    CK(launch_rope_table(e->stream, dpos, freq, cs, T, rope2d));
    hipError_t r = launch_qkv_rope_split(e->stream, (const bf16_t*)qkv, cs, dt, (int)tiles.size(), (bf16_t*)q, (bf16_t*)k, (bf16_t*)vt, T, Tpad, Hq, Hkv);
    hipStreamSynchronize(e->stream);
    e->release(dt); e->release(dq); e->release(dpos); e->release(cs); e->release(freq);
    CK(r);
    return DOTS_OK;
}

int dots_op_qkv_proj_rope(DotsEngine* e, const void* x, const void* w, const void* bias, void* qkv_ws, void* q, void* k, void* vt, const int32_t* cu, int n_seq,
                          const int32_t* pos_host, int K, int Hq, int Hkv, int rope2d, float theta, int fused) {
    if (!e || !x || !w || !qkv_ws || !q || !k || !vt || !cu || n_seq < 1 || !pos_host) return DOTS_E_INVALID;
    CK(hipSetDevice(e->device));
    std::vector<Tile64> tiles;
    std::vector<QBlock> qb;
    Tile64* dt = nullptr;
    QBlock* dq = nullptr;
    int64_t Tpad = 0;
    RET(upload_lists(e, cu, n_seq, Hq, tiles, qb, &dt, &dq, &Tpad));
    const int64_t T = cu[n_seq];
    const int N = (Hq + 2 * Hkv) * 128;
    int32_t* dpos = nullptr;
    float2* cs = nullptr;
    float* freq = nullptr;
    const int nf = rope2d ? 32 : 64;
    std::vector<float> f(nf);
    for (int i = 0; i < nf; ++i) f[i] = 1.0f / powf(theta, (float)(2 * i) / (rope2d ? 64.0f : 128.0f));
    CK(e->alloc(&dpos, (size_t)T * (rope2d ? 2 : 1)));
    CK(e->alloc(&cs, (size_t)T * 64));
    CK(e->alloc(&freq, (size_t)nf));
    CK(hipMemcpyAsync(dpos, pos_host, (size_t)T * (rope2d ? 2 : 1) * 4, hipMemcpyHostToDevice, e->stream));
    CK(hipMemcpyAsync(freq, f.data(), nf * 4, hipMemcpyHostToDevice, e->stream));
    CK(launch_rope_table(e->stream, dpos, freq, cs, T, rope2d));
    hipError_t r;
    if (fused) {
        r = launch_gemm_qk_rope(e->stream, (const bf16_t*)x, (const bf16_t*)w, (const bf16_t*)bias, (bf16_t*)qkv_ws, T, N, K, K, N, cs, (bf16_t*)q, (bf16_t*)k, Hq, Hkv);
        if (r == hipSuccess) r = launch_qkv_rope_split(e->stream, (const bf16_t*)qkv_ws, cs, dt, (int)tiles.size(), (bf16_t*)q, (bf16_t*)k, (bf16_t*)vt, T, Tpad, Hq, Hkv, true);
    } else {
        r = launch_gemm(e->stream, (const bf16_t*)x, (const bf16_t*)w, (const bf16_t*)bias, nullptr, qkv_ws, T, N, K, K, N, EPI_NONE);
        if (r == hipSuccess) r = launch_qkv_rope_split(e->stream, (const bf16_t*)qkv_ws, cs, dt, (int)tiles.size(), (bf16_t*)q, (bf16_t*)k, (bf16_t*)vt, T, Tpad, Hq, Hkv);
    }
    hipStreamSynchronize(e->stream);
    e->release(dt); e->release(dq); e->release(dpos); e->release(cs); e->release(freq);
    if (r == hipErrorNotSupported) { (void)hipGetLastError(); return e->fail(DOTS_E_INVALID, "no fused qkv + rope kernel for this shape / GEMM plan"); }
    CK(r);
    return DOTS_OK;
}

// ... 161 lines not shown
```

### dots_ocr_amd/csrc/probe_mfma.hip

```cpp
#include <hip/hip_runtime.h>
#include <stdint.h>

typedef __attribute__((ext_vector_type(8))) short bf16x8;
typedef __attribute__((ext_vector_type(16))) float f32x16;
typedef __attribute__((ext_vector_type(4))) float f32x4;

__global__ void probe_mfma_32x32x16(const uint16_t* A, const uint16_t* Bt, float* D) {
    const int l = threadIdx.x;
    bf16x8 a = *reinterpret_cast<const bf16x8*>(A + (l & 31) * 16 + 8 * (l >> 5));
    bf16x8 b = *reinterpret_cast<const bf16x8*>(Bt + (l & 31) * 16 + 8 * (l >> 5));
    f32x16 c = {0};
    c = __builtin_amdgcn_mfma_f32_32x32x16_bf16(a, b, c, 0, 0, 0);
#pragma unroll
    for (int r = 0; r < 16; ++r) {
        int row = (r & 3) + 8 * (r >> 2) + 4 * (l >> 5);
        D[row * 32 + (l & 31)] = c[r];
    }
}

__global__ void probe_mfma_16x16x32(const uint16_t* A, const uint16_t* Bt, float* D) {
    const int l = threadIdx.x;
    bf16x8 a = *reinterpret_cast<const bf16x8*>(A + (l & 15) * 32 + 8 * (l >> 4));
    bf16x8 b = *reinterpret_cast<const bf16x8*>(Bt + (l & 15) * 32 + 8 * (l >> 4));
    f32x4 c = {0};
    c = __builtin_amdgcn_mfma_f32_16x16x32_bf16(a, b, c, 0, 0, 0);
#pragma unroll
    for (int r = 0; r < 4; ++r) D[(4 * (l >> 4) + r) * 16 + (l & 15)] = c[r];
}

typedef __attribute__((ext_vector_type(8))) int i32x8;
__global__ void probe_mfma_32x32x64_fp8(const uint8_t* A, const uint8_t* Bt, float* D) {
    const int l = threadIdx.x;
    i32x8 a = *reinterpret_cast<const i32x8*>(A + (l & 31) * 64 + 32 * (l >> 5));
    i32x8 b = *reinterpret_cast<const i32x8*>(Bt + (l & 31) * 64 + 32 * (l >> 5));
    f32x16 c = {0};
    c = __builtin_amdgcn_mfma_scale_f32_32x32x64_f8f6f4(a, b, c, 0, 0, 0, 0x7f7f7f7f, 0, 0x7f7f7f7f);
#pragma unroll
    for (int r = 0; r < 16; ++r) {
        int row = (r & 3) + 8 * (r >> 2) + 4 * (l >> 5);
        D[row * 32 + (l & 31)] = c[r];
    }
}

__global__ void probe_glds(const uint32_t* in, uint32_t* out) {
    __shared__ __attribute__((aligned(16))) uint32_t lds[256];
    const int l = threadIdx.x;
    __builtin_amdgcn_global_load_lds(
        (const __attribute__((address_space(1))) void*)(in + l * 4),
        (__attribute__((address_space(3))) void*)lds, 16, 0, 0);
    asm volatile("s_waitcnt vmcnt(0)" ::: "memory");
    __syncthreads();
#pragma unroll
    for (int i = 0; i < 4; ++i) out[l * 4 + i] = lds[l * 4 + i];
}

extern "C" int dots_probe_mfma(int which, const void* A, const void* Bt, void* D, void* stream) {
    hipStream_t s = (hipStream_t)stream;
    if (which == 0) hipLaunchKernelGGL(probe_mfma_32x32x16, dim3(1), dim3(64), 0, s, (const uint16_t*)A, (const uint16_t*)Bt, (float*)D);
    else if (which == 1) hipLaunchKernelGGL(probe_mfma_16x16x32, dim3(1), dim3(64), 0, s, (const uint16_t*)A, (const uint16_t*)Bt, (float*)D);
    else if (which == 3) hipLaunchKernelGGL(probe_mfma_32x32x64_fp8, dim3(1), dim3(64), 0, s, (const uint8_t*)A, (const uint8_t*)Bt, (float*)D);
    else hipLaunchKernelGGL(probe_glds, dim3(1), dim3(64), 0, s, (const uint32_t*)A, (uint32_t*)D);
    return (int)hipGetLastError();
}
```

### dots_ocr_amd/engine.py

```python
from __future__ import annotations

import ctypes as C
import math
import os
from collections import OrderedDict
from dataclasses import dataclass
from typing import Dict, Optional, Sequence

import numpy as np

from . import _lib
from .config import DotsConfig

EPI_NONE, EPI_RESIDUAL, EPI_SWIGLU, EPI_GELU, EPI_F32 = range(5)
DTYPE_BF16, DTYPE_F32, DTYPE_F16 = 0, 1, 2


class CDotsConfig(C.Structure):
    _fields_ = [
        ("hidden_size", C.c_int32), ("num_layers", C.c_int32), ("num_heads", C.c_int32), ("num_kv_heads", C.c_int32),
        ("head_dim", C.c_int32), ("intermediate_size", C.c_int32), ("vocab_size", C.c_int32),
        ("rope_theta", C.c_float), ("rms_norm_eps", C.c_float),
        ("attention_bias", C.c_int32), ("image_token_id", C.c_int32),
        ("v_embed_dim", C.c_int32), ("v_layers", C.c_int32), ("v_heads", C.c_int32), ("v_intermediate", C.c_int32),
# ... 146 lines not shown
        object.__setattr__(self, "allowed", allowed)
        object.__setattr__(self, "min_tokens", int(self.min_tokens))
        object.__setattr__(self, "stop", stop)
        object.__setattr__(self, "ignore_eos", bool(self.ignore_eos))
        object.__setattr__(self, "vocab_size", None if self.vocab_size is None else int(self.vocab_size))
        object.__setattr__(self, "eos_ids", None if self.eos_ids is None else tuple(int(t) for t in self.eos_ids))

    @property
    def empty(self) -> bool:
        return not self.bias and self.allowed is None and self.min_tokens == 0 and not self.stop and not self.ignore_eos

    def to_c(self) -> CDotsLogitRules:
        ids = np.asarray([t for t, _ in self.bias], np.int32)
        vals = np.asarray([v for _, v in self.bias], np.float32)
        allowed = None if self.allowed is None else np.asarray(self.allowed, np.int32)
        c = CDotsLogitRules()
        c.bias_ids = _i32p(ids) if len(ids) else None
        c.bias_values = vals.ctypes.data_as(C.POINTER(C.c_float)) if len(ids) else None
        c.n_bias = len(ids)
        c.allowed_ids = _i32p(allowed) if allowed is not None else None
        c.n_allowed = 0 if allowed is None else len(allowed)
        c.min_tokens = self.min_tokens
        for j, t in enumerate(self.stop):
            c.stop_ids[j] = t
        c.n_stop = len(self.stop)
        c.ignore_eos = int(self.ignore_eos)
        c._keep = (ids, vals, allowed)
        return c


MAX_NGRAM_SIZE = 64
MAX_NGRAM_WHITELIST = 16


class CDotsNgramRule(C.Structure):
    _fields_ = [("size", C.c_int32), ("window", C.c_int32), ("n_whitelist", C.c_int32), ("whitelist", C.c_int32 * MAX_NGRAM_WHITELIST)]


@dataclass(frozen=True)
class NgramRule:
    size: int
    window: int = 0
    whitelist: tuple = ()
    vocab_size: Optional[int] = None
    max_seq_len: Optional[int] = None

    def __post_init__(self):
        for name in ("size", "window"):
            v = getattr(self, name)
            if isinstance(v, bool) or not isinstance(v, (int, np.integer)):
                raise ValueError(f"{name} must be an integer, got {v!r}")
        n, w = int(self.size), int(self.window)
        if not 1 <= n <= MAX_NGRAM_SIZE:
            raise ValueError(f"size must be in [1, {MAX_NGRAM_SIZE}], got {n}")
        if w != 0 and w < n:
            raise ValueError(f"window must be 0 (the whole output) or >= size = {n}, got {w}")
        if self.max_seq_len is not None and w > int(self.max_seq_len):
            raise ValueError(f"window {w} exceeds max_seq_len {int(self.max_seq_len)}")
        white = _id_tuple("whitelist", self.whitelist)
        if len(white) > MAX_NGRAM_WHITELIST:
            raise ValueError(f"at most {MAX_NGRAM_WHITELIST} whitelist ids, got {len(white)}")
        if len(set(white)) != len(white):
            raise ValueError("whitelist holds an id twice")
        if self.vocab_size is not None:
            for t in white:
                if t >= int(self.vocab_size):
                    raise ValueError(f"whitelist id {t} outside [0, {int(self.vocab_size)})")
        object.__setattr__(self, "size", n)
        object.__setattr__(self, "window", w)
        object.__setattr__(self, "whitelist", white)
        object.__setattr__(self, "vocab_size", None if self.vocab_size is None else int(self.vocab_size))
        object.__setattr__(self, "max_seq_len", None if self.max_seq_len is None else int(self.max_seq_len))

    def to_c(self) -> CDotsNgramRule:
        c = CDotsNgramRule(self.size, self.window, len(self.whitelist))
        for j, t in enumerate(self.whitelist):
            c.whitelist[j] = t
        return c


def banned_ngram_ids(out, n: int, window: int = 0, whitelist=()) -> set:
    out = [int(t) for t in out]
    L, n, window = len(out), int(n), int(window)
    if n < 1 or L < n - 1:
        return set()
    prefix = out[L - n + 1:] if n > 1 else []
    white = set(int(t) for t in whitelist)
    banned = set()
    for i in range(max(0, L - window) if window > 0 else 0, L - n + 1):
        if out[i:i + n - 1] == prefix and out[i + n - 1] not in white:
            banned.add(out[i + n - 1])
    return banned


class DotsEngineError(RuntimeError):
    pass


_SIGNATURES_SET = False


def _prototypes(lib):
    global _SIGNATURES_SET
    if _SIGNATURES_SET:
        return
    vp, i32, i64, f32 = C.c_void_p, C.c_int32, C.c_int64, C.c_float
    P = C.POINTER
    sig = {
        "dots_create": (i32, [P(CDotsConfig), i32, P(vp)]),
        "dots_destroy": (None, [vp]),
        "dots_last_error": (C.c_char_p, [vp]),
        "dots_stream": (vp, [vp]),
        "dots_load_weight": (i32, [vp, C.c_char_p, vp, i32, P(i64), i32]),
        "dots_finalize_weights": (i32, [vp]),
        "dots_vit_forward": (i32, [vp, vp, i32, i64, P(i64), i32, vp]),
        "dots_vit_prefetch": (i32, [vp, vp, i32, i64, P(i64), i32, i32]),
        "dots_vit_take_prefetched": (i32, [vp]),
        "dots_vit_prefetch_ready": (i32, [vp, P(i32)]),
        "dots_prefill": (i32, [vp, P(i32), P(i32), i32]),
        "dots_decode_step": (i32, [vp]),
        "dots_generate": (i32, [vp, P(i32), P(i32), i32, vp, i32, i64, P(i64), i32, i32, P(i32), i32, P(i32), P(i32)]),
        "dots_preprocess_image": (i32, [vp, vp, i32, i32, i32, i32, i32, P(i32), P(i32), i32, P(i32), P(i32), i32, P(f32), P(f32), f32, vp]),
        "dots_set_sampling": (i32, [vp, f32, f32, C.c_uint64]),
        "dots_set_row_sampling": (i32, [vp, i32, P(CDotsSamplingParams)]),
        "dots_set_decode_plan": (i32, [vp, i32]),
        "dots_set_gemm_plan": (i32, [vp, i32]),
        "dots_tower_tail": (i32, [vp, i32, P(i32)]),
        "dots_slot_capacity": (i32, [vp, i32, P(i32), P(i32)]),
        "dots_slots_reset": (i32, [vp]),
        "dots_set_eos": (i32, [vp, P(i32), i32]),
        "dots_slots_prefill": (i32, [vp, P(i32), i32, P(i32), P(i32), P(i32)]),
        "dots_slots_decode": (i32, [vp, i32]),
        "dots_slots_fork": (i32, [vp, i32, P(i32), i32]),
        "dots_slots_poll": (i32, [vp, P(i32), P(i32)]),
        "dots_slot_read": (i32, [vp, i32, P(i32), i32, P(i32)]),
        "dots_slot_release": (i32, [vp, i32]),
        "dots_kv_pool_info": (i32, [vp, P(i32), P(i32)]),
        "dots_set_kv_scales": (i32, [vp, P(f32)]),
        "dots_get_logits": (i32, [vp, P(f32)]),
        "dots_set_next_tokens": (i32, [vp, P(i32), i32]),
        "dots_get_last_tokens": (i32, [vp, P(i32)]),
        "dots_get_stats": (i32, [vp, P(CDotsStats)]),
        "dots_synchronize": (i32, [vp]),
        "dots_debug_capture_hidden": (i32, [vp, i64]),
        "dots_debug_read_hidden": (i32, [vp, i32, i32, vp, P(i64)]),
        "dots_debug_read_kv": (i32, [vp, i32, i32, i32, i32, i32, vp]),
        "dots_dev_alloc": (i32, [vp, i64, P(vp)]),
        "dots_dev_free": (i32, [vp, vp]),
        "dots_memcpy_h2d": (i32, [vp, vp, vp, i64]),
        "dots_memcpy_d2h": (i32, [vp, vp, vp, i64]),
        "dots_op_rmsnorm": (i32, [vp, vp, vp, vp, i64, i32, f32]),
        "dots_op_layernorm": (i32, [vp, vp, vp, vp, vp, i64, i32, f32]),
        "dots_op_gemm": (i32, [vp, vp, vp, vp, vp, vp, i64, i32, i32, i32, vp]),
        "dots_op_quant_fp8": (i32, [vp, vp, vp, i64, i32]),
        "dots_op_gemm_fp8": (i32, [vp, vp, vp, vp, vp, vp, i64, i32, i32, i32]),
        "dots_op_flash_attn": (i32, [vp, vp, vp, vp, vp, P(i32), i32, i32, i32, i32, f32]),
        "dots_plan_flash_xcd": (i32, [P(i32), i32, i32, P(i32), P(i32), P(i64)]),
        "dots_op_qkv_rope_split": (i32, [vp, vp, vp, vp, vp, P(i32), i32, P(i32), i32, i32, i32, f32]),
        "dots_op_qkv_proj_rope": (i32, [vp, vp, vp, vp, vp, vp, vp, vp, P(i32), i32, P(i32), i32, i32, i32, i32, f32, i32]),
        "dots_op_dec_qkv": (i32, [vp, vp, vp, vp, vp, vp, vp, i32, vp, vp, i32, i32, i32, i32, f32, f32, i32]),
        "dots_op_decode_attn": (i32, [vp, vp, vp, vp, vp, i32, vp, i32, i32, i32, i32]),
        "dots_op_dec_qkv_kv8": (i32, [vp, vp, vp, vp, vp, vp, vp, i32, vp, vp, i32, i32, i32, i32, f32, f32, i32, vp]),
        "dots_op_decode_attn_kv8": (i32, [vp, vp, vp, vp, vp, i32, vp, i32, i32, i32, i32, vp]),
        "dots_op_dec_proj": (i32, [vp, vp, vp, vp, i32, i32, i32, i32]),
        "dots_op_dec_gateup": (i32, [vp, vp, vp, vp, vp, vp, i32, i32, i32, f32, i32]),
        "dots_op_dec_lmhead": (i32, [vp, vp, vp, vp, vp, i32, i32, i32, f32, i32]),
        "dots_op_select_tokens": (i32, [vp, vp, i32, i32, P(CDotsSamplingParams), vp, vp, i32, vp, vp]),
        "dots_bench_select_tokens": (i32, [vp, vp, i32, i32, P(CDotsSamplingParams), vp, vp, i32, vp, i32, i32, P(f32)]),
        "dots_set_row_logit_rules": (i32, [vp, i32, P(CDotsLogitRules)]),
        "dots_op_select_tokens_rules": (i32, [vp, vp, i32, i32, P(CDotsSamplingParams), P(CDotsLogitRules), P(i32), vp, vp, i32, vp, vp]),
        "dots_bench_select_tokens_rules": (i32, [vp, vp, i32, i32, P(CDotsSamplingParams), P(CDotsLogitRules), P(i32), vp, vp, i32, vp, i32, P(f32)]),
        "dots_set_token_bytes": (i32, [vp, P(i32), vp]),
        "dots_guide_create": (i32, [vp, vp, i32, vp, i32, P(i32)]),
        "dots_guide_destroy": (i32, [vp, i32]),
        "dots_set_row_guide": (i32, [vp, i32, i32]),
        "dots_row_guide_state": (i32, [vp, i32, P(i32)]),
        "dots_op_select_tokens_guided": (i32, [vp, vp, i32, i32, P(CDotsSamplingParams), P(CDotsLogitRules), P(i32), P(i32), P(i32), vp, vp, i32, vp, vp,
                                               P(i32)]),
        "dots_bench_select_tokens_guided": (i32, [vp, vp, i32, i32, P(CDotsSamplingParams), P(CDotsLogitRules), P(i32), P(i32), P(i32), vp, vp, i32, vp,
                                                  i32, P(f32)]),
        "dots_set_row_ngram": (i32, [vp, i32, P(CDotsNgramRule)]),
        "dots_op_select_tokens_ngram": (i32, [vp, vp, i32, i32, P(CDotsSamplingParams), P(CDotsLogitRules), P(CDotsNgramRule), vp, vp, i32, vp, vp]),
        "dots_bench_select_tokens_ngram": (i32, [vp, vp, i32, i32, P(CDotsSamplingParams), P(CDotsLogitRules), P(CDotsNgramRule), vp, vp, i32, vp, i32,
                                                 P(f32)]),
        "dots_stop_create": (i32, [vp, vp, i32, vp, vp, P(i32)]),
        "dots_stop_destroy": (i32, [vp, i32]),
        "dots_set_row_stop": (i32, [vp, i32, i32, i32]),
        "dots_row_stop_hit": (i32, [vp, i32, P(i32)]),
        "dots_set_speculation": (i32, [vp, i32, i32, i32]),
        "dots_set_speculation_rows": (i32, [vp, i32]),
        "dots_set_row_drafts": (i32, [vp, i32, P(i32), i32]),
        "dots_spec_stats": (i32, [vp, i32, P(i64), P(i64), P(i64)]),
        "dots_op_ngram_draft": (i32, [vp, vp, vp, i32, i32, i32, i32, i32, vp, vp]),
        "dots_set_row_logprobs": (i32, [vp, i32, i32]),
        "dots_row_logprobs": (i32, [vp, i32, i32, i32, P(f32), P(i32), P(f32), P(i32)]),
        "dots_op_logprobs": (i32, [vp, vp, i32, i32, i32, P(i32), vp, vp, vp, vp]),
        "dots_bench_logprobs": (i32, [vp, vp, i32, i32, i32, P(i32), i32, i32, P(f32)]),
        "dots_probe_mfma": (i32, [i32, vp, vp, vp, vp]),
        "dots_probe_grid_barrier": (i32, [i32, i32, i32, i32, i32, P(f32), P(i32)]),
        "dots_probe_cu_mask": (i32, [P(C.c_uint32), i32, i32, i32, i32, P(C.c_uint32)]),
    }
    for name, (res, args) in sig.items():
        fn = getattr(lib, name)
        fn.restype = res
        fn.argtypes = args
    _SIGNATURES_SET = True


EXPORTED_SYMBOLS = [
    "dots_create", "dots_destroy", "dots_last_error", "dots_stream", "dots_load_weight", "dots_finalize_weights",
    "dots_vit_forward", "dots_vit_prefetch", "dots_vit_take_prefetched", "dots_vit_prefetch_ready", "dots_preprocess_image", "dots_prefill", "dots_decode_step", "dots_generate", "dots_set_sampling", "dots_set_decode_plan", "dots_set_gemm_plan", "dots_tower_tail", "dots_get_logits",
    "dots_set_eos", "dots_slots_prefill", "dots_slots_decode", "dots_slots_poll", "dots_slot_read", "dots_slot_release", "dots_kv_pool_info", "dots_slot_capacity", "dots_slots_reset",
    "dots_set_next_tokens", "dots_get_last_tokens", "dots_get_stats", "dots_synchronize", "dots_debug_capture_hidden",
    "dots_debug_read_hidden", "dots_dev_alloc",
    "dots_dev_free", "dots_memcpy_h2d", "dots_memcpy_d2h", "dots_op_rmsnorm", "dots_op_layernorm", "dots_op_gemm", "dots_op_quant_fp8", "dots_op_gemm_fp8",
    "dots_op_flash_attn", "dots_plan_flash_xcd", "dots_op_qkv_rope_split", "dots_op_qkv_proj_rope", "dots_op_dec_qkv", "dots_op_decode_attn", "dots_op_dec_proj", "dots_op_dec_gateup",
    "dots_op_dec_lmhead", "dots_probe_mfma", "dots_probe_grid_barrier", "dots_probe_cu_mask",
    "dots_set_kv_scales", "dots_debug_read_kv", "dots_op_dec_qkv_kv8", "dots_op_decode_attn_kv8",
    "dots_set_row_sampling", "dots_op_select_tokens", "dots_bench_select_tokens",
    "dots_set_row_logprobs", "dots_row_logprobs", "dots_op_logprobs", "dots_bench_logprobs",
    "dots_set_row_logit_rules", "dots_op_select_tokens_rules", "dots_bench_select_tokens_rules",
    "dots_set_token_bytes", "dots_guide_create", "dots_guide_destroy", "dots_set_row_guide", "dots_row_guide_state",
    "dots_op_select_tokens_guided", "dots_bench_select_tokens_guided",
    "dots_set_row_ngram", "dots_op_select_tokens_ngram", "dots_bench_select_tokens_ngram",
    "dots_set_speculation", "dots_set_speculation_rows", "dots_set_row_drafts", "dots_spec_stats", "dots_op_ngram_draft",
    "dots_slots_fork",
    "dots_stop_create", "dots_stop_destroy", "dots_set_row_stop", "dots_row_stop_hit",
]

MAX_SPEC_DRAFTS = 15
MAX_NGRAM_SIZE = 64


def ngram_draft(history: Sequence[int], k: int, min_n: int = 2, max_n: int = 4) -> list:
    out = [int(t) for t in history]
    L = len(out)
    if k < 1 or min_n < 1 or max_n < min_n:
        raise ValueError("ngram_draft needs k >= 1 and 1 <= min_n <= max_n")
    for n in range(max_n, min_n - 1, -1):
        if n + 1 > L:
            continue
        key = out[L - n:]
        hits = [i for i in range(L - n) if out[i:i + n] == key]
        if not hits:
            continue
        full = [i for i in hits if i + n + k <= L]
        i = max(full) if full else min(hits)
        return out[i + n:min(i + n + k, L)]
    return []


def spec_usable_slots(max_batch: int, k: int) -> int:
    return int(max_batch) // (int(k) + 1)


SPEC_ROWS = {"sampled": 1, "stop": 2}


def spec_rows_flags(value) -> int:
    if value is None:
        return 0
    names = (value,) if isinstance(value, str) else tuple(value)
    flags = 0
    for n in names:
        if n == "all":
            flags |= sum(SPEC_ROWS.values())
        elif n == "greedy" and len(names) == 1:
            pass
        elif isinstance(n, str) and n in SPEC_ROWS:
            flags |= SPEC_ROWS[n]
        else:
            raise ValueError(f"speculative_rows takes \"all\", \"greedy\" or names out of {sorted(SPEC_ROWS)}, got {value!r}")
    return flags


MAX_TOP_LOGPROBS = 20

KV_CACHE_DTYPES = {"bf16": 0, "fp8": 1}


def resolve_kv_cache_dtype(kv_cache_dtype: Optional[str]) -> str:
    if kv_cache_dtype is None:
        kv_cache_dtype = os.environ.get("DOTS_OCR_KV_CACHE_DTYPE", "") or "bf16"
    if kv_cache_dtype not in KV_CACHE_DTYPES:
        raise ValueError(f"kv_cache_dtype must be one of {sorted(KV_CACHE_DTYPES)}, got {kv_cache_dtype!r}")
    return kv_cache_dtype


def c_config(cfg: DotsConfig, max_batch: int, max_seq_len: int, max_patches: int, max_prefill_tokens: int, kv_pool_tokens: int = 0,
             fp8_weights: bool = False, kv_cache_dtype: str = "bf16") -> CDotsConfig:
    v = cfg.vision
    return CDotsConfig(
        hidden_size=cfg.hidden_size, num_layers=cfg.num_hidden_layers, num_heads=cfg.num_attention_heads,
        num_kv_heads=cfg.num_key_value_heads, head_dim=cfg.head_dim, intermediate_size=cfg.intermediate_size,
        vocab_size=cfg.vocab_size, rope_theta=cfg.rope_theta, rms_norm_eps=cfg.rms_norm_eps,
        attention_bias=int(cfg.attention_bias), image_token_id=cfg.image_token_id,
        v_embed_dim=v.embed_dim, v_layers=v.num_hidden_layers, v_heads=v.num_attention_heads,
        v_intermediate=v.intermediate_size, v_patch=v.patch_size, v_merge=v.spatial_merge_size,
        v_channels=v.num_channels, v_temporal_patch=v.temporal_patch_size, v_rms_eps=v.rms_norm_eps,
        v_ln_eps=v.merger_ln_eps, v_use_bias=int(v.use_bias), v_post_norm=int(v.post_norm),
        max_batch=max_batch, max_seq_len=max_seq_len, max_patches=max_patches,
        max_prefill_tokens=max_prefill_tokens, kv_pool_tokens=kv_pool_tokens, fp8_weights=int(bool(fp8_weights)),
        kv_cache_dtype=KV_CACHE_DTYPES[kv_cache_dtype])


def plan_flash_xcd(lens: Sequence[int], heads: int):
    lib = _lib.load()
    _prototypes(lib)
    L = np.ascontiguousarray(lens, dtype=np.int32)
    base, cnt, cost = np.zeros(8, np.int32), np.zeros(8, np.int32), np.zeros(8, np.int64)
    n = lib.dots_plan_flash_xcd(_i32p(L), int(L.shape[0]), int(heads), _i32p(base), _i32p(cnt), _i64p(cost))
    if n < 0:
        raise DotsEngineError(f"dots_plan_flash_xcd failed ({n})")
    return base, cnt, cost, int(n)


def _i32p(a: np.ndarray):
    return a.ctypes.data_as(C.POINTER(C.c_int32))


def _i64p(a: np.ndarray):
    return a.ctypes.data_as(C.POINTER(C.c_int64))


class Engine:

    def __init__(self, cfg: DotsConfig, device: int = 0, max_batch: int = 8, max_seq_len: int = 8192,
                 max_patches: int = 8 * 19824 + 64, max_prefill_tokens: Optional[int] = None, kv_pool_tokens: int = 0,
                 fp8_weights: bool = False, kv_cache_dtype: Optional[str] = None):
        self.kv_cache_dtype = resolve_kv_cache_dtype(kv_cache_dtype)
        self.lib = _lib.load()
        _prototypes(self.lib)
        self.cfg = cfg
        self.device = device
        self.max_batch = max_batch
        self.max_seq_len = max_seq_len
        self.max_patches = max_patches
        if max_prefill_tokens is None:
            max_prefill_tokens = max_batch * max_seq_len
        self.max_prefill_tokens = max_prefill_tokens
        self.kv_pool_tokens = kv_pool_tokens
        self.fp8_weights = bool(fp8_weights)
        self._cc = c_config(cfg, max_batch, max_seq_len, max_patches, max_prefill_tokens, kv_pool_tokens, fp8_weights, self.kv_cache_dtype)
        h = C.c_void_p()
        rc = self.lib.dots_create(C.byref(self._cc), device, C.byref(h))
        if rc != 0:
            raise DotsEngineError(f"dots_create failed ({rc}): {self.lib.dots_last_error(None).decode()}")
        self.h = h
        self.token_bytes = None
        self._stops = OrderedDict()

    def _ck(self, rc: int, what: str):
        if rc != 0:
            raise DotsEngineError(f"{what} failed ({rc}): {self.lib.dots_last_error(self.h).decode()}")

    def close(self):
        if getattr(self, "h", None):
            self.lib.dots_destroy(self.h)
            self.h = None

    def __del__(self):
        try:
            self.close()
        except Exception:
            pass

    @property
    def stream(self) -> int:
        return int(self.lib.dots_stream(self.h) or 0)

# ... 371 lines not shown
                 "dots_op_logprobs")

    def bench_logprobs(self, logits, B: int, V: int, ld: int, top_n: Sequence[int], which: int = 0, iters: int = 200) -> float:
        tn = np.ascontiguousarray(top_n, dtype=np.int32)
        ms = C.c_float()
        self._ck(self.lib.dots_bench_logprobs(self.h, logits, int(B), int(V), int(ld), _i32p(tn), int(which), int(iters), C.byref(ms)),
                 "dots_bench_logprobs")
        return float(ms.value)

    def set_decode_plan(self, plan: int):
        self._ck(self.lib.dots_set_decode_plan(self.h, int(plan)), "dots_set_decode_plan")

    def set_gemm_plan(self, plan: int):
        self._ck(self.lib.dots_set_gemm_plan(self.h, int(plan)), "dots_set_gemm_plan")

    def tower_tail(self, set: int = -2) -> int:
        now = C.c_int32(0)
        self._ck(self.lib.dots_tower_tail(self.h, int(set), C.byref(now)), "dots_tower_tail")
        return int(now.value)

    def decode_step(self):
        self._ck(self.lib.dots_decode_step(self.h), "dots_decode_step")

    def set_eos(self, eos_ids: Sequence[int]):
        eos = np.ascontiguousarray(list(eos_ids), dtype=np.int32)
        self._ck(self.lib.dots_set_eos(self.h, _i32p(eos) if len(eos) else None, len(eos)), "dots_set_eos")

    def slots_prefill(self, slots: Sequence[int], input_ids: np.ndarray, prompt_lens: Sequence[int], max_new_tokens: Sequence[int]):
        sl = np.ascontiguousarray(slots, dtype=np.int32)
        ids = np.ascontiguousarray(input_ids, dtype=np.int32)
        lens = np.ascontiguousarray(prompt_lens, dtype=np.int32)
        cap = np.ascontiguousarray(max_new_tokens, dtype=np.int32)
        assert sl.shape == lens.shape == cap.shape and ids.shape[0] == int(lens.sum())
        self._ck(self.lib.dots_slots_prefill(self.h, _i32p(sl), sl.shape[0], _i32p(ids), _i32p(lens), _i32p(cap)), "dots_slots_prefill")

    def slots_fork(self, src: int, dst_slots: Sequence[int]):
        dst = np.ascontiguousarray(dst_slots, dtype=np.int32)
        assert dst.ndim == 1
        self._ck(self.lib.dots_slots_fork(self.h, int(src), _i32p(dst) if dst.shape[0] else None, dst.shape[0]), "dots_slots_fork")

    def slots_reset(self):
        self._ck(self.lib.dots_slots_reset(self.h), "dots_slots_reset")

    def slots_decode(self, n_steps: int):
        self._ck(self.lib.dots_slots_decode(self.h, int(n_steps)), "dots_slots_decode")

    def slots_poll(self):
        fin = np.empty((self.max_batch,), dtype=np.int32)
        lens = np.empty((self.max_batch,), dtype=np.int32)
        self._ck(self.lib.dots_slots_poll(self.h, _i32p(fin), _i32p(lens)), "dots_slots_poll")
        return fin, lens

    def slot_read(self, slot: int, capacity: int) -> np.ndarray:
        out = np.empty((max(1, capacity),), dtype=np.int32)
        n = C.c_int32(0)
        self._ck(self.lib.dots_slot_read(self.h, int(slot), _i32p(out), int(capacity), C.byref(n)), "dots_slot_read")
        return out[:min(int(n.value), capacity)].copy()

    def slot_release(self, slot: int):
        self._ck(self.lib.dots_slot_release(self.h, int(slot)), "dots_slot_release")

    def slot_capacity(self, slot: int):
        pg, lim = C.c_int32(0), C.c_int32(0)
        self._ck(self.lib.dots_slot_capacity(self.h, int(slot), C.byref(pg), C.byref(lim)), "dots_slot_capacity")
        return pg.value, lim.value

    def kv_pool_info(self):
        tot, free = C.c_int32(0), C.c_int32(0)
        self._ck(self.lib.dots_kv_pool_info(self.h, C.byref(tot), C.byref(free)), "dots_kv_pool_info")
        return int(tot.value), int(free.value)

    def set_kv_scales(self, scales):
        shape = (self.cfg.num_hidden_layers, self.cfg.num_key_value_heads, 2)
        s = np.ascontiguousarray(np.broadcast_to(np.asarray(scales, dtype=np.float32), shape))
        self._ck(self.lib.dots_set_kv_scales(self.h, s.ctypes.data_as(C.POINTER(C.c_float))), "dots_set_kv_scales")

    def read_kv(self, layer: int, seq: int, pos0: int, n: int, which: str = "k") -> np.ndarray:
        dt = np.uint8 if self.kv_cache_dtype == "fp8" else np.uint16
        out = np.empty((self.cfg.num_key_value_heads, int(n), 128), dtype=dt)
        self._ck(self.lib.dots_debug_read_kv(self.h, int(layer), int(seq), int(pos0), int(n), {"k": 0, "v": 1}[which],
                                             out.ctypes.data_as(C.c_void_p)), "dots_debug_read_kv")
        return out

    def get_logits(self) -> np.ndarray:
        out = np.empty((self._B, self.cfg.vocab_size), dtype=np.float32)
        self._ck(self.lib.dots_get_logits(self.h, out.ctypes.data_as(C.POINTER(C.c_float))), "dots_get_logits")
        return out

    def get_last_tokens(self) -> np.ndarray:
        out = np.empty((self._B,), dtype=np.int32)
        self._ck(self.lib.dots_get_last_tokens(self.h, _i32p(out)), "dots_get_last_tokens")
        return out

    def set_next_tokens(self, tokens: Sequence[int]):
        t = np.ascontiguousarray(tokens, dtype=np.int32)
        self._ck(self.lib.dots_set_next_tokens(self.h, _i32p(t), t.shape[0]), "dots_set_next_tokens")

    def generate(self, input_ids: np.ndarray, prompt_lens: np.ndarray, pixel_values=None,
                 grid_thw: Optional[np.ndarray] = None, max_new_tokens: int = 128, eos_ids: Sequence[int] = (),
                 pixel_on_device: bool = False, vision_taken: bool = False):
        ids = np.ascontiguousarray(input_ids, dtype=np.int32)
        lens = np.ascontiguousarray(prompt_lens, dtype=np.int32)
        B = int(lens.shape[0])
        assert ids.shape[0] == int(lens.sum())
        out_ids = np.zeros((B, max_new_tokens), dtype=np.int32)
        out_lens = np.zeros((B,), dtype=np.int32)
        eos = np.ascontiguousarray(list(eos_ids), dtype=np.int32)
        if vision_taken:
            ptr, n, gp, n_img = None, 0, None, -1
        elif grid_thw is not None and len(grid_thw):
            grid = np.ascontiguousarray(grid_thw, dtype=np.int64)
            n = int((grid[:, 0] * grid[:, 1] * grid[:, 2]).sum())
            if pixel_on_device:
                ptr = C.c_void_p(int(pixel_values))
            else:
                pv = np.ascontiguousarray(pixel_values, dtype=np.float32)
                assert pv.shape[0] == n
                ptr = pv.ctypes.data_as(C.c_void_p)
            gp, n_img = _i64p(grid), grid.shape[0]
        else:
            ptr, n, gp, n_img = None, 0, None, 0
        self._ck(self.lib.dots_generate(self.h, _i32p(ids), _i32p(lens), B, ptr, int(pixel_on_device), n, gp, n_img,
                                        max_new_tokens, _i32p(eos) if len(eos) else None, len(eos),
                                        _i32p(out_ids), _i32p(out_lens)), "dots_generate")
        self._B = B
        return out_ids, out_lens

    def capture_hidden(self, capacity_elems: int):
        self._ck(self.lib.dots_debug_capture_hidden(self.h, int(capacity_elems)), "dots_debug_capture_hidden")

    def read_hidden(self, which: str, layer: int) -> np.ndarray:
        dim = self.cfg.vision.embed_dim if which == "vit" else self.cfg.hidden_size
        cap = (self.max_patches if which == "vit" else self.max_prefill_tokens) * dim
        buf = np.empty(cap, dtype=np.uint16)
        rows = C.c_int64(0)
        self._ck(self.lib.dots_debug_read_hidden(self.h, 0 if which == "vit" else 1, int(layer), buf.ctypes.data_as(C.c_void_p), C.byref(rows)),
                 "dots_debug_read_hidden")
        return buf[: rows.value * dim].reshape(rows.value, dim).copy()

    def stats(self) -> dict:
        st = CDotsStats()
        self._ck(self.lib.dots_get_stats(self.h, C.byref(st)), "dots_get_stats")
        return {k: getattr(st, k) for k, _ in CDotsStats._fields_}

    def op_rmsnorm(self, x, w, y, rows, dim, eps):
        self._ck(self.lib.dots_op_rmsnorm(self.h, x, w, y, rows, dim, eps), "dots_op_rmsnorm")

    def op_layernorm(self, x, w, b, y, rows, dim, eps):
        self._ck(self.lib.dots_op_layernorm(self.h, x, w, b, y, rows, dim, eps), "dots_op_layernorm")

    def op_gemm(self, A, W, bias, residual, Cout, M, N, K, epilogue=EPI_NONE, colscale=None):
        self._ck(self.lib.dots_op_gemm(self.h, A, W, bias or None, residual or None, Cout, M, N, K, epilogue, colscale or None), "dots_op_gemm")

    def op_gemm_fp8(self, A, W, bias, residual, Cout, M, N, K, epilogue=EPI_NONE):
        self._ck(self.lib.dots_op_gemm_fp8(self.h, A, W, bias or None, residual or None, Cout, M, N, K, epilogue), "dots_op_gemm_fp8")

    def op_quant_fp8(self, w_inout, scale_out, N, K):
        self._ck(self.lib.dots_op_quant_fp8(self.h, w_inout, scale_out, N, K), "dots_op_quant_fp8")

    def op_flash_attn(self, q, k, vt, out, cu_seqlens, Hq, Hkv, causal, scale):
        cu = np.ascontiguousarray(cu_seqlens, dtype=np.int32)
        self._ck(self.lib.dots_op_flash_attn(self.h, q, k, vt, out, _i32p(cu), cu.shape[0] - 1, Hq, Hkv, int(causal), scale),
                 "dots_op_flash_attn")

    def op_qkv_rope_split(self, qkv, q, k, vt, cu_seqlens, pos, Hq, Hkv, rope2d, theta):
        cu = np.ascontiguousarray(cu_seqlens, dtype=np.int32)
        pos = np.ascontiguousarray(pos, dtype=np.int32)
        self._ck(self.lib.dots_op_qkv_rope_split(self.h, qkv, q, k, vt, _i32p(cu), cu.shape[0] - 1, _i32p(pos), Hq, Hkv,
                                                 int(rope2d), theta), "dots_op_qkv_rope_split")

    def op_qkv_proj_rope(self, x, w, bias, qkv_ws, q, k, vt, cu_seqlens, pos, K, Hq, Hkv, rope2d, theta, fused):
        cu = np.ascontiguousarray(cu_seqlens, dtype=np.int32)
        pos = np.ascontiguousarray(pos, dtype=np.int32)
        self._ck(self.lib.dots_op_qkv_proj_rope(self.h, x, w, bias, qkv_ws, q, k, vt, _i32p(cu), cu.shape[0] - 1, _i32p(pos), K, Hq, Hkv,
                                                int(rope2d), theta, int(fused)), "dots_op_qkv_proj_rope")

    def op_dec_qkv(self, h, ln_w, wqkv, bias, ctx_len, block_table, max_pages, pool_layer, q_out, B, H, Hq, Hkv, eps, rope_theta, fp8=False):
        self._ck(self.lib.dots_op_dec_qkv(self.h, h, ln_w, wqkv, bias or None, ctx_len, block_table, max_pages, pool_layer, q_out,
                                          B, H, Hq, Hkv, eps, rope_theta, int(fp8)), "dots_op_dec_qkv")

    def op_decode_attn(self, q, pool_layer, ctx_len, block_table, max_pages, out, B, Hq, Hkv, max_seq_len):
        self._ck(self.lib.dots_op_decode_attn(self.h, q, pool_layer, ctx_len, block_table, max_pages, out, B, Hq, Hkv, max_seq_len),
                 "dots_op_decode_attn")

    def op_dec_qkv_kv8(self, h, ln_w, wqkv, bias, ctx_len, block_table, max_pages, pool_layer, q_out, B, H, Hq, Hkv, eps, rope_theta, kv_scales,
                       fp8=False):
        self._ck(self.lib.dots_op_dec_qkv_kv8(self.h, h, ln_w, wqkv, bias or None, ctx_len, block_table, max_pages, pool_layer, q_out,
                                              B, H, Hq, Hkv, eps, rope_theta, int(fp8), kv_scales), "dots_op_dec_qkv_kv8")

    def op_decode_attn_kv8(self, q, pool_layer, ctx_len, block_table, max_pages, out, B, Hq, Hkv, max_seq_len, kv_scales):
        self._ck(self.lib.dots_op_decode_attn_kv8(self.h, q, pool_layer, ctx_len, block_table, max_pages, out, B, Hq, Hkv, max_seq_len,
                                                  kv_scales), "dots_op_decode_attn_kv8")

    def op_dec_proj(self, x, w, h_inout, B, N, K, fp8=False):
        self._ck(self.lib.dots_op_dec_proj(self.h, x, w, h_inout, B, N, K, int(fp8)), "dots_op_dec_proj")

    def op_dec_gateup(self, h, ln_w, gate_w, up_w, act_out, B, H, I, eps, fp8=False):
        self._ck(self.lib.dots_op_dec_gateup(self.h, h, ln_w, gate_w, up_w, act_out, B, H, I, eps, int(fp8)), "dots_op_dec_gateup")

    def op_dec_lmhead(self, h, ln_w, w, logits_out, B, H, V, eps, fp8=False):
        self._ck(self.lib.dots_op_dec_lmhead(self.h, h, ln_w, w, logits_out, B, H, V, eps, int(fp8)), "dots_op_dec_lmhead")
```

### include/dots_ocr_hip.h

```cpp
#ifndef DOTS_OCR_HIP_H
#define DOTS_OCR_HIP_H

#include <stdint.h>

#ifdef __cplusplus
extern "C" {
#endif

#define DOTS_OK 0
#define DOTS_E_INVALID (-1)
#define DOTS_E_HIP (-2)
#define DOTS_E_STATE (-3)
#define DOTS_E_CAPACITY (-4)

#define DOTS_DTYPE_BF16 0
#define DOTS_DTYPE_F32 1
#define DOTS_DTYPE_F16 2

typedef struct DotsEngine DotsEngine;

typedef struct DotsConfig {
    int32_t hidden_size, num_layers, num_heads, num_kv_heads, head_dim, intermediate_size, vocab_size;
    float rope_theta, rms_norm_eps;
    int32_t attention_bias;
// ... 2 lines not shown
    float v_rms_eps, v_ln_eps;
    int32_t v_use_bias, v_post_norm;
    int32_t max_batch;
    int32_t max_seq_len;
    int64_t max_patches;
    int64_t max_prefill_tokens;
    int64_t kv_pool_tokens;
    int32_t fp8_weights;
    int32_t kv_cache_dtype;
} DotsConfig;

typedef struct DotsStats {
    float vit_ms, prefill_ms, decode_ms, total_ms;
    float vit_attn_ms;
    int32_t vit_attn_launches;
    float vit_gemm_ms;
    int32_t decode_steps;
    int64_t vit_patches, prefill_tokens, new_tokens;
    double vit_attn_flops;
    double vit_flops;
    double prefill_flops;
    double decode_bytes;
} DotsStats;

int dots_create(const DotsConfig* cfg, int device, DotsEngine** out);
void dots_destroy(DotsEngine* e);
const char* dots_last_error(DotsEngine* e);
void* dots_stream(DotsEngine* e);

int dots_load_weight(DotsEngine* e, const char* name, const void* data_host, int dtype,
                     const int64_t* shape, int ndim);
int dots_finalize_weights(DotsEngine* e);

int dots_vit_forward(DotsEngine* e, const float* pixel_values, int pixel_values_on_device,
                     int64_t total_patches, const int64_t* grid_thw_host, int n_img,
                     void* out_embeds_dev);

int dots_vit_prefetch(DotsEngine* e, const float* pixel_values, int pixel_values_on_device, int64_t total_patches,
                      const int64_t* grid_thw_host, int n_img, int after_prefill);
int dots_vit_take_prefetched(DotsEngine* e);
int dots_vit_prefetch_ready(DotsEngine* e, int* ready);

int dots_prefill(DotsEngine* e, const int32_t* input_ids_host, const int32_t* prompt_lens_host, int B);

int dots_decode_step(DotsEngine* e);

int dots_generate(DotsEngine* e, const int32_t* input_ids_host, const int32_t* prompt_lens_host, int B,
                  const float* pixel_values, int pixel_values_on_device, int64_t total_patches,
                  const int64_t* grid_thw_host, int n_img, int max_new_tokens,
                  const int32_t* eos_ids_host, int n_eos, int32_t* out_ids_host, int32_t* out_lens_host);

int dots_preprocess_image(DotsEngine* e, const uint8_t* rgb, int rgb_on_device, int h, int w, int rh, int rw,
                          const int32_t* hcoef_host, const int32_t* hbounds_host, int hksize,
                          const int32_t* vcoef_host, const int32_t* vbounds_host, int vksize,
                          const float* mean3_host, const float* std3_host, float rescale, float* out_pixel_values_dev);

int dots_set_sampling(DotsEngine* e, float temperature, float top_p, uint64_t seed);

typedef struct DotsSamplingParams {
    float temperature, top_p;
    int32_t top_k;
    float repetition_penalty, frequency_penalty, presence_penalty;
    uint64_t seed;
} DotsSamplingParams;
int dots_set_row_sampling(DotsEngine* e, int row, const DotsSamplingParams* p);

#define DOTS_MAX_LOGIT_BIAS 1024
#define DOTS_MAX_STOP_IDS 16
typedef struct DotsLogitRules {
    const int32_t* bias_ids;
    const float* bias_values;
    int32_t n_bias;
    const int32_t* allowed_ids;
    int32_t n_allowed;
    int32_t min_tokens;
    int32_t stop_ids[DOTS_MAX_STOP_IDS];
    int32_t n_stop;
    int32_t ignore_eos;
} DotsLogitRules;
int dots_set_row_logit_rules(DotsEngine* e, int row, const DotsLogitRules* r);

#define DOTS_MAX_GUIDE_STATES 4096
int dots_set_token_bytes(DotsEngine* e, const int32_t* offsets_host, const uint8_t* bytes_host);
int dots_guide_create(DotsEngine* e, const uint16_t* table_host, int n_states, const uint8_t* accepting_host, int start, int32_t* id_out);
int dots_guide_destroy(DotsEngine* e, int32_t id);
int dots_set_row_guide(DotsEngine* e, int row, int32_t id);
int dots_row_guide_state(DotsEngine* e, int row, int32_t* state_out);

#define DOTS_MAX_NGRAM_SIZE 64
#define DOTS_MAX_NGRAM_WHITELIST 16
typedef struct DotsNgramRule {
    int32_t size;
    int32_t window;
    int32_t n_whitelist;
    int32_t whitelist[DOTS_MAX_NGRAM_WHITELIST];
} DotsNgramRule;
int dots_set_row_ngram(DotsEngine* e, int row, const DotsNgramRule* r);

#define DOTS_MAX_STOP_STRINGS 16
#define DOTS_MAX_STOP_BYTES 64
int dots_stop_create(DotsEngine* e, const uint16_t* table_host, int n_states, const uint16_t* match_len_host, const uint8_t* match_id_host,
                     int32_t* handle_out);
int dots_stop_destroy(DotsEngine* e, int32_t handle);
int dots_set_row_stop(DotsEngine* e, int row, int32_t handle, int min_tokens);
int dots_row_stop_hit(DotsEngine* e, int row, int32_t* out);

#define DOTS_MAX_SPEC_DRAFTS 15
#define DOTS_SPEC_ROWS_SAMPLED 1
#define DOTS_SPEC_ROWS_STOP 2
int dots_set_speculation(DotsEngine* e, int k, int min_n, int max_n);
int dots_set_speculation_rows(DotsEngine* e, int flags);
int dots_set_row_drafts(DotsEngine* e, int row, const int32_t* ids_host, int n);
int dots_spec_stats(DotsEngine* e, int row, int64_t* steps, int64_t* drafted, int64_t* accepted);

#define DOTS_MAX_TOP_LOGPROBS 20
int dots_set_row_logprobs(DotsEngine* e, int row, int top_n);
int dots_row_logprobs(DotsEngine* e, int row, int pos0, int n, float* tok_lp_host, int32_t* top_ids_host, float* top_lp_host, int32_t* n_out);
int dots_set_decode_plan(DotsEngine* e, int plan);
int dots_tower_tail(DotsEngine* e, int set, int* now);
int dots_set_gemm_plan(DotsEngine* e, int plan);

int dots_slots_reset(DotsEngine* e);
int dots_slots_fork(DotsEngine* e, int src_slot, const int32_t* dst_slots_host, int n);
int dots_set_eos(DotsEngine* e, const int32_t* eos_ids_host, int n_eos);
int dots_slots_prefill(DotsEngine* e, const int32_t* slots_host, int n, const int32_t* input_ids_host,
                       const int32_t* prompt_lens_host, const int32_t* max_new_tokens_host);
int dots_slots_decode(DotsEngine* e, int n_steps);
int dots_slots_poll(DotsEngine* e, int32_t* finished_host, int32_t* out_lens_host);
int dots_slot_read(DotsEngine* e, int slot, int32_t* out_ids_host, int capacity, int32_t* n_out);
int dots_slot_release(DotsEngine* e, int slot);
int dots_kv_pool_info(DotsEngine* e, int32_t* total_pages, int32_t* free_pages);
int dots_set_kv_scales(DotsEngine* e, const float* scales_host);
int dots_slot_capacity(DotsEngine* e, int slot, int32_t* pages_owned, int32_t* token_limit);

int dots_get_logits(DotsEngine* e, float* out_host);
int dots_set_next_tokens(DotsEngine* e, const int32_t* tokens_host, int B);
int dots_get_last_tokens(DotsEngine* e, int32_t* out_host);
int dots_get_stats(DotsEngine* e, DotsStats* out);
int dots_debug_capture_hidden(DotsEngine* e, int64_t capacity_elems);
int dots_debug_read_hidden(DotsEngine* e, int which, int layer, void* out_host, int64_t* rows_out);
int dots_debug_read_kv(DotsEngine* e, int layer, int seq_or_slot, int pos0, int n, int which, void* out_host);
int dots_synchronize(DotsEngine* e);

int dots_dev_alloc(DotsEngine* e, int64_t bytes, void** out_dev);
int dots_dev_free(DotsEngine* e, void* dev);
int dots_memcpy_h2d(DotsEngine* e, void* dst_dev, const void* src_host, int64_t bytes);
int dots_memcpy_d2h(DotsEngine* e, void* dst_host, const void* src_dev, int64_t bytes);

int dots_op_rmsnorm(DotsEngine* e, const void* x_dev, const void* w_dev, void* y_dev, int64_t rows, int dim, float eps);
int dots_op_layernorm(DotsEngine* e, const void* x_dev, const void* w_dev, const void* b_dev, void* y_dev,
                      int64_t rows, int dim, float eps);
int dots_op_gemm(DotsEngine* e, const void* A_dev, const void* W_dev, const void* bias_dev,
                 const void* residual_dev, void* C_dev, int64_t M, int N, int K, int epilogue, const float* colscale_dev);
int dots_op_quant_fp8(DotsEngine* e, void* w_inout_dev, float* scale_out_dev, int64_t N, int K);
int dots_op_gemm_fp8(DotsEngine* e, const void* A_dev, const void* W_dev, const void* bias_dev, const void* residual_dev, void* C_dev,
                     int64_t M, int N, int K, int epilogue);
int dots_op_flash_attn(DotsEngine* e, const void* q_dev, const void* k_dev, const void* vt_dev, void* out_dev,
                       const int32_t* cu_seqlens_host, int n_seq, int Hq, int Hkv, int causal, float scale);
int dots_plan_flash_xcd(const int32_t* lens, int n_seq, int Hq, int32_t* base8, int32_t* cnt8, int64_t* cost8);
int dots_op_qkv_rope_split(DotsEngine* e, const void* qkv_dev, void* q_dev, void* k_dev, void* vt_dev,
                           const int32_t* cu_seqlens_host, int n_seq, const int32_t* pos_host,
                           int Hq, int Hkv, int rope2d, float theta);
int dots_op_qkv_proj_rope(DotsEngine* e, const void* x_dev, const void* w_dev, const void* bias_dev, void* qkv_ws_dev, void* q_dev, void* k_dev, void* vt_dev,
                          const int32_t* cu_seqlens_host, int n_seq, const int32_t* pos_host, int K, int Hq, int Hkv, int rope2d, float theta, int fused);
int dots_op_dec_qkv(DotsEngine* e, const void* h_dev, const void* ln_w_dev, const void* wqkv_dev, const void* bias_dev,
                    const int32_t* ctx_len_dev, const int32_t* block_table_dev, int max_pages, void* pool_layer_dev, void* q_out_dev,
                    int B, int H, int Hq, int Hkv, float eps, float rope_theta, int fp8);
int dots_op_decode_attn(DotsEngine* e, const void* q_dev, const void* pool_layer_dev, const int32_t* ctx_len_dev,
                        const int32_t* block_table_dev, int max_pages, void* out_dev, int B, int Hq, int Hkv, int max_seq_len);
int dots_op_dec_qkv_kv8(DotsEngine* e, const void* h_dev, const void* ln_w_dev, const void* wqkv_dev, const void* bias_dev,
                        const int32_t* ctx_len_dev, const int32_t* block_table_dev, int max_pages, void* pool_layer_dev, void* q_out_dev,
                        int B, int H, int Hq, int Hkv, float eps, float rope_theta, int fp8, const float* kv_scales_dev);
int dots_op_decode_attn_kv8(DotsEngine* e, const void* q_dev, const void* pool_layer_dev, const int32_t* ctx_len_dev,
                            const int32_t* block_table_dev, int max_pages, void* out_dev, int B, int Hq, int Hkv, int max_seq_len,
                            const float* kv_scales_dev);
int dots_op_dec_proj(DotsEngine* e, const void* x_dev, const void* w_dev, void* h_inout_dev, int B, int N, int K, int fp8);
int dots_op_dec_gateup(DotsEngine* e, const void* h_dev, const void* ln_w_dev, const void* gate_w_dev, const void* up_w_dev, void* act_out_dev,
                       int B, int H, int I, float eps, int fp8);
int dots_op_dec_lmhead(DotsEngine* e, const void* h_dev, const void* ln_w_dev, const void* w_dev, void* logits_out_dev, int B, int H, int V,
                       float eps, int fp8);
int dots_op_select_tokens(DotsEngine* e, const float* logits_dev, int B, int V, const DotsSamplingParams* params_host, const int32_t* hist_dev,
                          const int32_t* hist_lens_dev, int hist_stride, const int32_t* n_prompt_dev, int32_t* out_tokens_dev);
int dots_bench_select_tokens(DotsEngine* e, const float* logits_dev, int B, int V, const DotsSamplingParams* params_host, const int32_t* hist_dev,
                             const int32_t* hist_lens_dev, int hist_stride, const int32_t* n_prompt_dev, int mode, int iters, float* ms_out);
int dots_op_select_tokens_rules(DotsEngine* e, const float* logits_dev, int B, int V, const DotsSamplingParams* params_host, const DotsLogitRules* rules_host,
                                const int32_t* n_gen_host, const int32_t* hist_dev, const int32_t* hist_lens_dev, int hist_stride,
                                const int32_t* n_prompt_dev, int32_t* out_tokens_dev);
int dots_bench_select_tokens_rules(DotsEngine* e, const float* logits_dev, int B, int V, const DotsSamplingParams* params_host, const DotsLogitRules* rules_host,
                                   const int32_t* n_gen_host, const int32_t* hist_dev, const int32_t* hist_lens_dev, int hist_stride,
                                   const int32_t* n_prompt_dev, int iters, float* ms_out);
int dots_op_select_tokens_guided(DotsEngine* e, const float* logits_dev, int B, int V, const DotsSamplingParams* params_host, const DotsLogitRules* rules_host,
                                 const int32_t* n_gen_host, const int32_t* guide_ids_host, const int32_t* states_host, const int32_t* hist_dev,
                                 const int32_t* hist_lens_dev, int hist_stride, const int32_t* n_prompt_dev, int32_t* out_tokens_dev, int32_t* states_out_host);
int dots_bench_select_tokens_guided(DotsEngine* e, const float* logits_dev, int B, int V, const DotsSamplingParams* params_host, const DotsLogitRules* rules_host,
                                    const int32_t* n_gen_host, const int32_t* guide_ids_host, const int32_t* states_host, const int32_t* hist_dev,
                                    const int32_t* hist_lens_dev, int hist_stride, const int32_t* n_prompt_dev, int iters, float* ms_out);
int dots_op_select_tokens_ngram(DotsEngine* e, const float* logits_dev, int B, int V, const DotsSamplingParams* params_host, const DotsLogitRules* rules_host,
                                const DotsNgramRule* ngram_host, const int32_t* hist_dev, const int32_t* hist_lens_dev, int hist_stride,
                                const int32_t* n_prompt_dev, int32_t* out_tokens_dev);
int dots_bench_select_tokens_ngram(DotsEngine* e, const float* logits_dev, int B, int V, const DotsSamplingParams* params_host, const DotsLogitRules* rules_host,
                                   const DotsNgramRule* ngram_host, const int32_t* hist_dev, const int32_t* hist_lens_dev, int hist_stride,
                                   const int32_t* n_prompt_dev, int iters, float* ms_out);
int dots_op_ngram_draft(DotsEngine* e, const int32_t* hist_dev, const int32_t* hist_lens_dev, int hist_stride, int B, int k, int min_n, int max_n,
                        int32_t* drafts_dev, int32_t* n_drafts_dev);
int dots_op_logprobs(DotsEngine* e, const float* logits_dev, int B, int V, int ld, const int32_t* top_n_host,
                     const int32_t* chosen_dev, float* tok_lp_dev, int32_t* top_ids_dev, float* top_lp_dev);
int dots_bench_logprobs(DotsEngine* e, const float* logits_dev, int B, int V, int ld, const int32_t* top_n_host, int which, int iters,
                        float* ms_out);

int dots_probe_mfma(int which, const void* A, const void* Bt, void* D, void* stream);
int dots_probe_grid_barrier(int n_wg, int threads, int n_barriers, int mode, int lds_bytes, float* ms_out, int32_t* stats_out);
int dots_probe_cu_mask(const uint32_t* mask, int words, int n_wg, int threads, int lds_bytes, uint32_t* ids_out_host);

#ifdef __cplusplus
}
#endif
#endif
```

Measured before the change: 6.330 pages/s.

## Add 16x16x32 MFMA variant of one-wave-per-SIMD GEMM and make it default

Adds a third GEMM plan that runs the one-wave-per-SIMD bf16 body with v_mfma_f32_16x16x32_bf16 instead of 32x32x16. It reworks the LDS fragment addressing and swizzle, the accumulator layout (8x8 f32x4), the prefetch and DMA schedule inside the unrolled K loop, and the LDS-staged and f32 epilogues to match the new fragment shape. The plan becomes the default. The aim is higher MFMA throughput or better issue overlap on MI355X. The change also adds a gemm_lda op binding and an MFMA-shape probe, at the cost of a new, complex code path that could have layout bugs.

```diff
diff --git a/dots_ocr_amd/csrc/engine.hip b/dots_ocr_amd/csrc/engine.hip
--- a/dots_ocr_amd/csrc/engine.hip
+++ b/dots_ocr_amd/csrc/engine.hip
@@ -872,7 +872,7 @@
 
 int dots_set_gemm_plan(DotsEngine* e, int plan) {
     if (!e) return DOTS_E_INVALID;
-    if (plan < 0 || plan > 1) return e->fail(DOTS_E_INVALID, "gemm plan must be 0 (8-wave ping-pong) or 1 (one wave per SIMD)");
+    if (plan < 0 || plan > 2) return e->fail(DOTS_E_INVALID, "gemm plan must be 0 (8-wave ping-pong), 1 (one wave per SIMD) or 2 (one wave per SIMD, 16x16x32 MFMA)");
     gemm_set_plan(plan);
     return DOTS_OK;
 }
diff --git a/dots_ocr_amd/csrc/gemm.hip b/dots_ocr_amd/csrc/gemm.hip
--- a/dots_ocr_amd/csrc/gemm.hip
+++ b/dots_ocr_amd/csrc/gemm.hip
@@ -1,4 +1,5 @@
 #include <cstdlib>
+#include <type_traits>
 #include <utility>
 
 #include "common.h"
@@ -483,8 +484,8 @@
     }
 }
 
-template <int EPI, bool FULL>
-DEVI void w4_epilogue_lds(const f32x16 (&acc)[4][4], const W4Cols& cc, bool has_cols, const bf16_t* R,
+template <int EPI, bool FULL, int SH = 0, class ACC>
+DEVI void w4_epilogue_lds(const ACC& acc, const W4Cols& cc, bool has_cols, const bf16_t* R,
                           bf16_t* __restrict__ C, int M, int ldc, int nw0, int mw0, int l, char* stage2) {
     const int hi = l >> 5, l31 = l & 31;
     constexpr bool SW = EPI == EPI_SWIGLU;
@@ -509,10 +510,18 @@
 #endif
     const int wslot = swz(l31);
     char* const wrow = stage2 + l31 * 512;
+    const int g16 = l >> 4, wslot16 = swz(l & 15);
+    char* const wrow16 = stage2 + (l & 15) * 512;
+    (void)hi; (void)wslot; (void)wrow; (void)g16; (void)wslot16; (void)wrow16;
 #define W4_PUT(FM, IMG)                                                                                                   \
-    _Pragma("unroll") for (int fn = 0; fn < 4; ++fn) _Pragma("unroll") for (int rq = 0; rq < 4; ++rq) {                     \
-        const f32x4 v = {acc[fn][FM][4 * rq], acc[fn][FM][4 * rq + 1], acc[fn][FM][4 * rq + 2], acc[fn][FM][4 * rq + 3]};   \
-        *reinterpret_cast<f32x4*>(wrow + (IMG) * 16384 + (((fn * 8 + rq * 2 + hi) ^ wslot) << 4)) = v;                      \
+    if constexpr (SH == 0) {                                                                                              \
+        _Pragma("unroll") for (int fn = 0; fn < 4; ++fn) _Pragma("unroll") for (int rq = 0; rq < 4; ++rq) {                 \
+            const f32x4 v = {acc[fn][FM][4 * rq], acc[fn][FM][4 * rq + 1], acc[fn][FM][4 * rq + 2], acc[fn][FM][4 * rq + 3]}; \
+            *reinterpret_cast<f32x4*>(wrow + (IMG) * 16384 + (((fn * 8 + rq * 2 + hi) ^ wslot) << 4)) = v;                  \
+        }                                                                                                                 \
+    } else {                                                                                                              \
+        _Pragma("unroll") for (int h = 0; h < 2; ++h) _Pragma("unroll") for (int fn = 0; fn < 8; ++fn)                      \
+            *reinterpret_cast<f32x4*>(wrow16 + h * 8192 + (IMG) * 16384 + (((fn * 4 + g16) ^ wslot16) << 4)) = acc[fn][2 * (FM) + h]; \
     }
     load_r(0, rr[0]);
     W4_PUT(0, 0)
@@ -601,8 +610,8 @@
     }
 }
 
-template <bool FULL>
-DEVI void w4_epilogue_qkrope(const f32x16 (&acc)[4][4], const W4Cols& cc, bool has_cols, const float2* __restrict__ cs, bf16_t* __restrict__ dst,
+template <bool FULL, int SH = 0, class ACC>
+DEVI void w4_epilogue_qkrope(const ACC& acc, const W4Cols& cc, bool has_cols, const float2* __restrict__ cs, bf16_t* __restrict__ dst,
                              int M, int mw0, int l, char* stage2) {
     const int hi = l >> 5, l31 = l & 31;
     const int rrow = l >> 4, gcol = (l & 15) * 8;
@@ -611,10 +620,18 @@
     auto swz = [](int row) { return ((row & 15) << 1) ^ (row & 1) ^ ((row & 2) << 2); };
     const int wslot = swz(l31);
     char* const wrow = stage2 + l31 * 512;
+    const int g16 = l >> 4, wslot16 = swz(l & 15);
+    char* const wrow16 = stage2 + (l & 15) * 512;
+    (void)hi; (void)wslot; (void)wrow; (void)g16; (void)wslot16; (void)wrow16;
 #define W4_PUT(FM, IMG)                                                                                                   \
-    _Pragma("unroll") for (int fn = 0; fn < 4; ++fn) _Pragma("unroll") for (int rq = 0; rq < 4; ++rq) {                     \
-        const f32x4 v = {acc[fn][FM][4 * rq], acc[fn][FM][4 * rq + 1], acc[fn][FM][4 * rq + 2], acc[fn][FM][4 * rq + 3]};   \
-        *reinterpret_cast<f32x4*>(wrow + (IMG) * 16384 + (((fn * 8 + rq * 2 + hi) ^ wslot) << 4)) = v;                      \
+    if constexpr (SH == 0) {                                                                                              \
+        _Pragma("unroll") for (int fn = 0; fn < 4; ++fn) _Pragma("unroll") for (int rq = 0; rq < 4; ++rq) {                 \
+            const f32x4 v = {acc[fn][FM][4 * rq], acc[fn][FM][4 * rq + 1], acc[fn][FM][4 * rq + 2], acc[fn][FM][4 * rq + 3]}; \
+            *reinterpret_cast<f32x4*>(wrow + (IMG) * 16384 + (((fn * 8 + rq * 2 + hi) ^ wslot) << 4)) = v;                  \
+        }                                                                                                                 \
+    } else {                                                                                                              \
+        _Pragma("unroll") for (int h = 0; h < 2; ++h) _Pragma("unroll") for (int fn = 0; fn < 8; ++fn)                      \
+            *reinterpret_cast<f32x4*>(wrow16 + h * 8192 + (IMG) * 16384 + (((fn * 4 + g16) ^ wslot16) << 4)) = acc[fn][2 * (FM) + h]; \
     }
     f32x4 tb[2][2][4];
     auto load_t = [&](int qb, f32x4 (&d)[2][4]) {
@@ -677,10 +694,34 @@
 #undef W4_PUT
 }
 
+DEVI void w4_epilogue_f32_16(const f32x4 (&acc)[8][8], const bf16_t* __restrict__ bias, const float* __restrict__ colscale, float* __restrict__ C, int M, int ldc,
+                             int nw0, int mw0, int l) {
+#pragma unroll
+    for (int fm = 0; fm < 8; ++fm) {
+        const int m = mw0 + fm * 16 + (l & 15);
+        if (m >= M) continue;
+#pragma unroll
+        for (int fn = 0; fn < 8; ++fn) {
+            const int nb = nw0 + fn * 16 + 4 * (l >> 4);
+            f32x4 o = acc[fn][fm];
+            if (colscale) {
+                const f32x4 sc = *reinterpret_cast<const f32x4*>(colscale + nb);
+#pragma unroll
+                for (int e = 0; e < 4; ++e) o[e] *= sc[e] * 1.f;
+            }
+            if (bias) {
+                const u32x2 bb = *reinterpret_cast<const u32x2*>(bias + nb);
+                o[0] += lo_bf(bb[0]); o[1] += hi_bf(bb[0]); o[2] += lo_bf(bb[1]); o[3] += hi_bf(bb[1]);
+            }
+            *reinterpret_cast<f32x4*>(C + (size_t)m * ldc + nb) = o;
+        }
+    }
+}
+
 template <int... I, class F> DEVI void gemm_static_for_impl(std::integer_sequence<int, I...>, F&& f) { (f(std::integral_constant<int, I>{}), ...); }
 template <int N, class F> DEVI void gemm_static_for(F&& f) { gemm_static_for_impl(std::make_integer_sequence<int, N>{}, f); }
 
-template <int EPI>
+template <int EPI, int SH = 0>
 DEVI void gemm_bf16_w4_body(
     const bf16_t* __restrict__ A, const bf16_t* __restrict__ W, const bf16_t* __restrict__ bias,
     const float* __restrict__ colscale, const bf16_t* R, void* Cout, int M, int N, int K, int lda, int ldc, int m_tiles, int n_tiles, int group_m, const QkRope& rope) {
@@ -721,13 +762,14 @@
     };
 
     const int wn = w >> 1, wm = w & 1;
-    const int rsw = (l31 >> 1) & 7;
-    const int lane_sw = ((hi ^ (rsw & 1)) << 4) | ((rsw >> 1) << 5);
+    const int lrow = SH ? (l & 15) : l31;
+    const int rsw = (lrow >> 1) & 7;
+    const int lane_sw = SH ? ((l >> 4) ^ rsw) << 4 : ((hi ^ (rsw & 1)) << 4) | ((rsw >> 1) << 5);
     const int lds0 = (int)(uintptr_t)(__attribute__((address_space(3))) char*)smem2;
-    const int a_lane = lds0 + (wn * 128 + l31) * 128 + lane_sw;
-    const int b_lane = lds0 + (wm * 128 + l31) * 128 + lane_sw;
+    const int a_lane = lds0 + (wn * 128 + lrow) * 128 + lane_sw;
+    const int b_lane = lds0 + (wm * 128 + lrow) * 128 + lane_sw;
     auto frag = [&](int base, int ks, int f) {
-        return *reinterpret_cast<const __attribute__((address_space(3))) bf16x8*>((uintptr_t)(uint32_t)((base ^ (ks << 5)) + f * 4096));
+        return *reinterpret_cast<const __attribute__((address_space(3))) bf16x8*>((uintptr_t)(uint32_t)((base ^ (ks << (SH ? 6 : 5))) + f * (SH ? 2048 : 4096)));
     };
 
 #ifdef W4_PROF
@@ -737,13 +779,14 @@
     if constexpr (EPI == EPI_QKROPE) w4_load_cols_rope(cols, bias, colscale, n0 + wn * 128, l);
     else if constexpr (EPI != EPI_F32) w4_load_cols<EPI == EPI_SWIGLU>(cols, bias, colscale, n0 + wn * 128, l);
 
-    f32x16 acc[4][4];
-#pragma unroll
-    for (int i = 0; i < 4; ++i)
-#pragma unroll
-        for (int j = 0; j < 4; ++j)
-#pragma unroll
-            for (int r = 0; r < 16; ++r) acc[i][j][r] = 0.f;
+    constexpr int NF = SH ? 8 : 4;
+    std::conditional_t<SH != 0, f32x4, f32x16> acc[NF][NF];
+#pragma unroll
+    for (int i = 0; i < NF; ++i)
+#pragma unroll
+        for (int j = 0; j < NF; ++j)
+#pragma unroll
+            for (int r = 0; r < 256 / (NF * NF); ++r) acc[i][j][r] = 0.f;
 
     const int nt = K / BK;
 #ifdef W4_STAGGER
@@ -761,9 +804,9 @@
         }
     asm volatile("s_waitcnt vmcnt(16)" ::: "memory");
     __builtin_amdgcn_s_barrier();
-    bf16x8 fa[2][4], fb[2][4];
-#pragma unroll
-    for (int f = 0; f < 4; ++f) { fa[0][f] = frag(a_lane, 0, f); fb[0][f] = frag(b_lane + W4_UNIT, 0, f); }
+    bf16x8 fa[2][NF], fb[2][NF];
+#pragma unroll
+    for (int f = 0; f < NF; ++f) { fa[0][f] = frag(a_lane, 0, f); fb[0][f] = frag(b_lane + W4_UNIT, 0, f); }
 #ifdef W4_PROF
     const unsigned long long pt1 = __builtin_amdgcn_s_memtime(), pw1 = wall_clock64();
 #endif
@@ -774,6 +817,35 @@
         const int s3 = u0 + 3 >= W4_RING ? u0 + 3 - W4_RING : u0 + 3, s4 = u0 + 4 >= W4_RING ? u0 + 4 - W4_RING : u0 + 4;
         const int aw = a_lane + u0 * W4_UNIT, ax = b_lane + s1 * W4_UNIT;
         const int awn = a_lane + s2 * W4_UNIT, axn = b_lane + s3 * W4_UNIT;
+        if constexpr (SH != 0) {
+            gemm_static_for<128>([&acc, &fa, &fb, &frag, &dma_w, &dma_x, aw, ax, awn, axn, t, u0, s4](auto gc) {
+                constexpr int gp = decltype(gc)::value;
+                (void)acc; (void)t; (void)u0; (void)s4; (void)dma_w; (void)dma_x; (void)aw; (void)ax; (void)awn; (void)axn;
+                constexpr int ks = gp >> 6, idx = gp & 63, fn = idx >> 3, fm = idx & 7, cur = ks;
+                if constexpr (gp == 96 && MODE < 2) {
+                    if constexpr (MODE == 0) asm volatile("s_waitcnt vmcnt(8) lgkmcnt(0)" ::: "memory");
+                    else asm volatile("s_waitcnt vmcnt(0) lgkmcnt(0)" ::: "memory");
+                    __builtin_amdgcn_s_barrier();
+                }
+                if constexpr (ks == 0 && idx < 32 && (idx & 1) == 0) {
+                    constexpr int f = (idx >> 1) & 7;
+                    if constexpr (idx < 16) fa[1][f] = frag(aw, 1, f);
+                    else fb[1][f] = frag(ax, 1, f);
+                }
+                if constexpr (ks == 1 && idx >= 32 && (idx & 1) == 0 && MODE < 2) {
+                    constexpr int f = (idx >> 1) & 7;
+                    if constexpr (idx < 48) fa[0][f] = frag(awn, 0, f);
+                    else fb[0][f] = frag(axn, 0, f);
+                }
+#ifndef W4_NO_DMA
+                if constexpr (MODE == 0) {
+                    if constexpr (gp >= 35 && gp < 96 && (gp - 35) % 8 == 0) dma_w(t + 2, s4, (gp - 35) / 8);
+                    if constexpr (gp >= 97 && (gp - 97) % 4 == 0) dma_x(t + 2, u0, (gp - 97) / 4);
+                }
+#endif
+                asm volatile("v_mfma_f32_16x16x32_bf16 %[d], %[a], %[b], %[d]" : [d] "+a"(acc[fn][fm]) : [a] "v"(fa[cur][fn]), [b] "v"(fb[cur][fm]));
+            });
+        } else
         gemm_static_for<64>([&acc, &fa, &fb, &frag, &dma_w, &dma_x, aw, ax, awn, axn, t, u0, s4](auto gc) {
             constexpr int gp = decltype(gc)::value;
             (void)acc; (void)t; (void)u0; (void)s4; (void)dma_w; (void)dma_x;
@@ -826,6 +898,7 @@
     return;
 #endif
 #ifdef W4_OLD_EPILOGUE
+    static_assert(SH == 0, "the W4_OLD_EPILOGUE ablation exists for the 32x32x16 body only");
     if constexpr (EPI == EPI_F32 || EPI == EPI_SWIGLU) {
         gemm_epilogue<EPI, 4, 4>(acc, bias, colscale, R, Cout, M, ldc, n0 + wn * 128, m0 + wm * 128, l31, hi);
     } else {
@@ -837,19 +910,20 @@
         const bool full = m0 + wm * 128 + 128 <= M, has_cols = bias != nullptr || colscale != nullptr;
         if (head < rope.n_rope_heads) {
             bf16_t* dst = head < rope.Hq ? rope.q + (size_t)head * rope.T * 128 : rope.k + (size_t)(head - rope.Hq) * rope.T * 128;
-            if (full) w4_epilogue_qkrope<true>(acc, cols, has_cols, rope.cs, dst, M, m0 + wm * 128, l, smem2 + w * 32768);
-            else w4_epilogue_qkrope<false>(acc, cols, has_cols, rope.cs, dst, M, m0 + wm * 128, l, smem2 + w * 32768);
+            if (full) w4_epilogue_qkrope<true, SH>(acc, cols, has_cols, rope.cs, dst, M, m0 + wm * 128, l, smem2 + w * 32768);
+            else w4_epilogue_qkrope<false, SH>(acc, cols, has_cols, rope.cs, dst, M, m0 + wm * 128, l, smem2 + w * 32768);
         } else if (full) {
-            w4_epilogue_lds<EPI_NONE, true>(acc, cols, has_cols, R, reinterpret_cast<bf16_t*>(Cout), M, ldc, n0 + wn * 128, m0 + wm * 128, l, smem2 + w * 32768);
+            w4_epilogue_lds<EPI_NONE, true, SH>(acc, cols, has_cols, R, reinterpret_cast<bf16_t*>(Cout), M, ldc, n0 + wn * 128, m0 + wm * 128, l, smem2 + w * 32768);
         } else {
-            w4_epilogue_lds<EPI_NONE, false>(acc, cols, has_cols, R, reinterpret_cast<bf16_t*>(Cout), M, ldc, n0 + wn * 128, m0 + wm * 128, l, smem2 + w * 32768);
+            w4_epilogue_lds<EPI_NONE, false, SH>(acc, cols, has_cols, R, reinterpret_cast<bf16_t*>(Cout), M, ldc, n0 + wn * 128, m0 + wm * 128, l, smem2 + w * 32768);
         }
     } else if constexpr (EPI == EPI_F32) {
-        gemm_epilogue<EPI, 4, 4>(acc, bias, colscale, R, Cout, M, ldc, n0 + wn * 128, m0 + wm * 128, l31, hi);
+        if constexpr (SH != 0) w4_epilogue_f32_16(acc, bias, colscale, reinterpret_cast<float*>(Cout), M, ldc, n0 + wn * 128, m0 + wm * 128, l);
+        else gemm_epilogue<EPI, 4, 4>(acc, bias, colscale, R, Cout, M, ldc, n0 + wn * 128, m0 + wm * 128, l31, hi);
     } else if (m0 + wm * 128 + 128 <= M) {
-        w4_epilogue_lds<EPI, true>(acc, cols, bias != nullptr || colscale != nullptr, R, reinterpret_cast<bf16_t*>(Cout), M, ldc, n0 + wn * 128, m0 + wm * 128, l, smem2 + w * 32768);
+        w4_epilogue_lds<EPI, true, SH>(acc, cols, bias != nullptr || colscale != nullptr, R, reinterpret_cast<bf16_t*>(Cout), M, ldc, n0 + wn * 128, m0 + wm * 128, l, smem2 + w * 32768);
     } else {
-        w4_epilogue_lds<EPI, false>(acc, cols, bias != nullptr || colscale != nullptr, R, reinterpret_cast<bf16_t*>(Cout), M, ldc, n0 + wn * 128, m0 + wm * 128, l, smem2 + w * 32768);
+        w4_epilogue_lds<EPI, false, SH>(acc, cols, bias != nullptr || colscale != nullptr, R, reinterpret_cast<bf16_t*>(Cout), M, ldc, n0 + wn * 128, m0 + wm * 128, l, smem2 + w * 32768);
     }
 #endif
 #ifdef W4_PROF
@@ -862,16 +936,17 @@
 #endif
 }
 
-template <int EPI>
+template <int EPI, int SH = 0>
 __global__ __launch_bounds__(256) void gemm_bf16_w4_kernel(
     const bf16_t* __restrict__ A, const bf16_t* __restrict__ W, const bf16_t* __restrict__ bias,
     const float* __restrict__ colscale, const bf16_t* R, void* Cout, int M, int N, int K, int lda, int ldc, int m_tiles, int n_tiles, int group_m) {
-    gemm_bf16_w4_body<EPI>(A, W, bias, colscale, R, Cout, M, N, K, lda, ldc, m_tiles, n_tiles, group_m, QkRope{});
-}
+    gemm_bf16_w4_body<EPI, SH>(A, W, bias, colscale, R, Cout, M, N, K, lda, ldc, m_tiles, n_tiles, group_m, QkRope{});
+}
+template <int SH>
 __global__ __launch_bounds__(256) void gemm_bf16_w4_qkrope_kernel(
     const bf16_t* __restrict__ A, const bf16_t* __restrict__ W, const bf16_t* __restrict__ bias,
     const float* __restrict__ colscale, void* Cout, int M, int N, int K, int lda, int ldc, int m_tiles, int n_tiles, int group_m, QkRope rope) {
-    gemm_bf16_w4_body<EPI_QKROPE>(A, W, bias, colscale, nullptr, Cout, M, N, K, lda, ldc, m_tiles, n_tiles, group_m, rope);
+    gemm_bf16_w4_body<EPI_QKROPE, SH>(A, W, bias, colscale, nullptr, Cout, M, N, K, lda, ldc, m_tiles, n_tiles, group_m, rope);
 }
 
 typedef __attribute__((ext_vector_type(8))) int i32x8;
@@ -993,17 +1068,18 @@
     return panel >= (4 << 20) ? 2 : panel >= (3 << 19) ? 4 : GROUP_M;
 }
 
+static int gemm_plan_of(int v) { return v == 0 || v == 2 ? v : 1; }
 static int g_gemm_plan = -1;
 int gemm_get_plan() {
     int p = __atomic_load_n(&g_gemm_plan, __ATOMIC_RELAXED);
     if (p < 0) {
         const char* ev = getenv("DOTS_OCR_GEMM_PLAN");
-        p = ev ? (atoi(ev) != 0) : 1;
+        p = ev ? gemm_plan_of(atoi(ev)) : 2;
         __atomic_store_n(&g_gemm_plan, p, __ATOMIC_RELAXED);
     }
     return p;
 }
-void gemm_set_plan(int plan) { __atomic_store_n(&g_gemm_plan, plan != 0, __ATOMIC_RELAXED); }
+void gemm_set_plan(int plan) { __atomic_store_n(&g_gemm_plan, gemm_plan_of(plan), __ATOMIC_RELAXED); }
 
 template <int E>
 static hipError_t launch_256(hipStream_t s, const bf16_t* A, const bf16_t* W, const bf16_t* bias, const float* colscale, const bf16_t* R, void* C,
@@ -1025,7 +1101,19 @@
                            lda, ldc, m_tiles, n_tiles);
         return hipGetLastError();
     }
-    if (gemm_get_plan() == 1 && K / BK >= 3) {
+    const int plan = gemm_get_plan();
+    if (plan == 2 && K / BK >= 3) {
+        static uint32_t configured_w4s = 0;
+        if (!(__atomic_load_n(&configured_w4s, __ATOMIC_ACQUIRE) & bit)) {
+            e = hipFuncSetAttribute(reinterpret_cast<const void*>(&gemm_bf16_w4_kernel<E, 1>), hipFuncAttributeMaxDynamicSharedMemorySize, W4_RING * W4_UNIT);
+            if (e != hipSuccess) return e;
+            __atomic_fetch_or(&configured_w4s, bit, __ATOMIC_RELEASE);
+        }
+        hipLaunchKernelGGL((gemm_bf16_w4_kernel<E, 1>), dim3(m_tiles * n_tiles), dim3(256), W4_RING * W4_UNIT, s, A, W, bias, colscale, R, C, M, N, K,
+                           lda, ldc, m_tiles, n_tiles, raster_group_m(K * 2));
+        return hipGetLastError();
+    }
+    if (plan == 1 && K / BK >= 3) {
         static uint32_t configured_w4 = 0;
         if (!(__atomic_load_n(&configured_w4, __ATOMIC_ACQUIRE) & bit)) {
             e = hipFuncSetAttribute(reinterpret_cast<const void*>(&gemm_bf16_w4_kernel<E>), hipFuncAttributeMaxDynamicSharedMemorySize, W4_RING * W4_UNIT);
@@ -1084,7 +1172,8 @@
                                const float2* cs, bf16_t* q, bf16_t* k, int Hq, int Hkv) {
     static const bool off = getenv("DOTS_OCR_QK_FUSE") && atoi(getenv("DOTS_OCR_QK_FUSE")) == 0;
     static const bool lockstep = getenv("DOTS_OCR_GEMM_LOCKSTEP") != nullptr, force_small = getenv("DOTS_OCR_GEMM_128") != nullptr;
-    if (off || lockstep || force_small || gemm_get_plan() != 1 || N != (Hq + 2 * Hkv) * 128 || N % BN2 != 0 || K % BK != 0 || K / BK < 3 || lda % 8 != 0 || ldc % 8 != 0 ||
+    const int plan = gemm_get_plan();
+    if (off || lockstep || force_small || plan == 0 || N != (Hq + 2 * Hkv) * 128 || N % BN2 != 0 || K % BK != 0 || K / BK < 3 || lda % 8 != 0 || ldc % 8 != 0 ||
         !cs || !q || !k || M > 0x7fffffff)
         return hipErrorNotSupported;
     if (M <= 0) return hipSuccess;
@@ -1094,14 +1183,20 @@
     if (e != hipSuccess) return e;
     const uint32_t bit = 1u << (dev & 31);
     if (!(__atomic_load_n(&configured, __ATOMIC_ACQUIRE) & bit)) {
-        e = hipFuncSetAttribute(reinterpret_cast<const void*>(&gemm_bf16_w4_qkrope_kernel), hipFuncAttributeMaxDynamicSharedMemorySize, W4_RING * W4_UNIT);
+        e = hipFuncSetAttribute(reinterpret_cast<const void*>(&gemm_bf16_w4_qkrope_kernel<0>), hipFuncAttributeMaxDynamicSharedMemorySize, W4_RING * W4_UNIT);
+        if (e == hipSuccess)
+            e = hipFuncSetAttribute(reinterpret_cast<const void*>(&gemm_bf16_w4_qkrope_kernel<1>), hipFuncAttributeMaxDynamicSharedMemorySize, W4_RING * W4_UNIT);
         if (e != hipSuccess) return e;
         __atomic_fetch_or(&configured, bit, __ATOMIC_RELEASE);
     }
     const int m_tiles = (int)((M + BM2 - 1) / BM2), n_tiles = N / BN2;
     const QkRope rope{cs, q, k, (long long)M, Hq, Hq + Hkv};
-    hipLaunchKernelGGL(gemm_bf16_w4_qkrope_kernel, dim3(m_tiles * n_tiles), dim3(256), W4_RING * W4_UNIT, s, A, W, bias, (const float*)nullptr, (void*)qkv, (int)M, N, K,
-                       lda, ldc, m_tiles, n_tiles, raster_group_m(K * 2), rope);
+    if (plan == 2)
+        hipLaunchKernelGGL(gemm_bf16_w4_qkrope_kernel<1>, dim3(m_tiles * n_tiles), dim3(256), W4_RING * W4_UNIT, s, A, W, bias, (const float*)nullptr, (void*)qkv, (int)M, N, K,
+                           lda, ldc, m_tiles, n_tiles, raster_group_m(K * 2), rope);
+    else
+        hipLaunchKernelGGL(gemm_bf16_w4_qkrope_kernel<0>, dim3(m_tiles * n_tiles), dim3(256), W4_RING * W4_UNIT, s, A, W, bias, (const float*)nullptr, (void*)qkv, (int)M, N, K,
+                           lda, ldc, m_tiles, n_tiles, raster_group_m(K * 2), rope);
     return hipGetLastError();
 }
 
diff --git a/dots_ocr_amd/csrc/ops.hip b/dots_ocr_amd/csrc/ops.hip
--- a/dots_ocr_amd/csrc/ops.hip
+++ b/dots_ocr_amd/csrc/ops.hip
@@ -277,6 +277,15 @@
     return DOTS_OK;
 }
 
+int dots_op_gemm_lda(DotsEngine* e, const void* A, const void* W, const void* bias, const void* residual, void* C,
+                     int64_t M, int N, int K, int lda, int epilogue, const float* colscale) {
+    if (!e || lda < K) return DOTS_E_INVALID;
+    CK(hipSetDevice(e->device));
+    const int ldc = epilogue == EPI_SWIGLU ? N / 2 : N;
+    CK(launch_gemm(e->stream, (const bf16_t*)A, (const bf16_t*)W, (const bf16_t*)bias, (const bf16_t*)residual, C, M, N, K, lda, ldc, epilogue, colscale));
+    return DOTS_OK;
+}
+
 int dots_op_gemm_fp8(DotsEngine* e, const void* A, const void* W, const void* bias, const void* residual, void* C, int64_t M, int N, int K,
                      int epilogue) {
     if (!e || !A || !W || !C) return e ? e->fail(DOTS_E_INVALID, "null argument") : DOTS_E_INVALID;
diff --git a/dots_ocr_amd/csrc/probe_mfma.hip b/dots_ocr_amd/csrc/probe_mfma.hip
--- a/dots_ocr_amd/csrc/probe_mfma.hip
+++ b/dots_ocr_amd/csrc/probe_mfma.hip
@@ -54,11 +54,34 @@
     for (int i = 0; i < 4; ++i) out[l * 4 + i] = lds[l * 4 + i];
 }
 
+__global__ void probe_mfma_16x16x32_gemm_tile(const uint16_t* W, const uint16_t* X, float* D) {
+    __shared__ __attribute__((aligned(16))) char lds[2 * 16 * 128];
+    const int l = threadIdx.x;
+#pragma unroll
+    for (int i = 0; i < 4; ++i) {
+        const int piece = l + 64 * i, img = piece >> 7, row = (piece >> 3) & 15, c = piece & 7;
+        const uint4 v = *reinterpret_cast<const uint4*>((img ? X : W) + row * 64 + c * 8);
+        *reinterpret_cast<uint4*>(lds + img * 2048 + row * 128 + ((c ^ ((row >> 1) & 7)) << 4)) = v;
+    }
+    __syncthreads();
+    const int row = l & 15, g = l >> 4;
+    f32x4 c = {0};
+#pragma unroll
+    for (int ks = 0; ks < 2; ++ks) {
+        const int slot = (4 * ks + g) ^ ((row >> 1) & 7);
+        const bf16x8 a = *reinterpret_cast<const bf16x8*>(lds + row * 128 + (slot << 4));
+        const bf16x8 b = *reinterpret_cast<const bf16x8*>(lds + 2048 + row * 128 + (slot << 4));
+        c = __builtin_amdgcn_mfma_f32_16x16x32_bf16(a, b, c, 0, 0, 0);
+    }
+    *reinterpret_cast<f32x4*>(D + (l & 15) * 16 + 4 * g) = c;
+}
+
 extern "C" int dots_probe_mfma(int which, const void* A, const void* Bt, void* D, void* stream) {
     hipStream_t s = (hipStream_t)stream;
     if (which == 0) hipLaunchKernelGGL(probe_mfma_32x32x16, dim3(1), dim3(64), 0, s, (const uint16_t*)A, (const uint16_t*)Bt, (float*)D);
     else if (which == 1) hipLaunchKernelGGL(probe_mfma_16x16x32, dim3(1), dim3(64), 0, s, (const uint16_t*)A, (const uint16_t*)Bt, (float*)D);
     else if (which == 3) hipLaunchKernelGGL(probe_mfma_32x32x64_fp8, dim3(1), dim3(64), 0, s, (const uint8_t*)A, (const uint8_t*)Bt, (float*)D);
+    else if (which == 4) hipLaunchKernelGGL(probe_mfma_16x16x32_gemm_tile, dim3(1), dim3(64), 0, s, (const uint16_t*)A, (const uint16_t*)Bt, (float*)D);
     else hipLaunchKernelGGL(probe_glds, dim3(1), dim3(64), 0, s, (const uint32_t*)A, (uint32_t*)D);
     return (int)hipGetLastError();
 }
diff --git a/dots_ocr_amd/csrc/probe_mfma_shape.hip b/dots_ocr_amd/csrc/probe_mfma_shape.hip
--- /dev/null
+++ b/dots_ocr_amd/csrc/probe_mfma_shape.hip
@@ -0,0 +1,162 @@
+#include <hip/hip_runtime.h>
+#include <stdint.h>
+
+#include <algorithm>
+#include <chrono>
+#include <utility>
+#include <vector>
+
+namespace {
+typedef __attribute__((ext_vector_type(8))) short bf16x8;
+typedef __attribute__((ext_vector_type(16))) float f32x16;
+typedef __attribute__((ext_vector_type(4))) float f32x4;
+typedef __attribute__((ext_vector_type(4))) uint32_t u32x4;
+
+constexpr int UNIT = 256 * 128;
+
+template <int... I, class F> __device__ __forceinline__ void static_for_impl(std::integer_sequence<int, I...>, F&& f) { (f(std::integral_constant<int, I>{}), ...); }
+template <int N, class F> __device__ __forceinline__ void static_for(F&& f) { static_for_impl(std::make_integer_sequence<int, N>{}, f); }
+
+template <int SHAPE>
+__global__ __launch_bounds__(256) void probe_shape_loop(const uint16_t* __restrict__ src, int ktiles, float* __restrict__ sink, unsigned long long* __restrict__ stamps) {
+    __shared__ __attribute__((aligned(16))) char lds[2 * UNIT];
+    const int tid = threadIdx.x, l = tid & 63;
+    const int w = __builtin_amdgcn_readfirstlane(tid >> 6);
+#pragma unroll
+    for (int i = 0; i < 16; ++i) {
+        const int piece = tid + 256 * i, row = piece >> 3, s = piece & 7;
+        const u32x4 v = *reinterpret_cast<const u32x4*>(reinterpret_cast<const char*>(src) + piece * 16);
+        *reinterpret_cast<u32x4*>(lds + row * 128 + ((s ^ ((row >> 1) & 7)) << 4)) = v;
+    }
+    __syncthreads();
+    const int wn = w >> 1, wm = w & 1;
+    const int lds0 = (int)(uintptr_t)(__attribute__((address_space(3))) char*)lds;
+    unsigned long long c0, c1, r0, r1;
+
+    if constexpr (SHAPE == 0) {
+        const int hi = l >> 5, l31 = l & 31, rsw = (l31 >> 1) & 7;
+        const int lane_sw = ((hi ^ (rsw & 1)) << 4) | ((rsw >> 1) << 5);
+        const int a_lane = lds0 + (wn * 128 + l31) * 128 + lane_sw, b_lane = lds0 + UNIT + (wm * 128 + l31) * 128 + lane_sw;
+        auto frag = [&](int base, int ks, int f) {
+            return *reinterpret_cast<const __attribute__((address_space(3))) bf16x8*>((uintptr_t)(uint32_t)((base ^ (ks << 5)) + f * 4096));
+        };
+        f32x16 acc[4][4];
+#pragma unroll
+        for (int i = 0; i < 4; ++i)
+#pragma unroll
+            for (int j = 0; j < 4; ++j)
+#pragma unroll
+                for (int r = 0; r < 16; ++r) acc[i][j][r] = 0.f;
+        bf16x8 fa[2][4], fb[2][4];
+#pragma unroll
+        for (int f = 0; f < 4; ++f) { fa[0][f] = frag(a_lane, 0, f); fb[0][f] = frag(b_lane, 0, f); }
+        c0 = __builtin_amdgcn_s_memtime(); r0 = __builtin_amdgcn_s_memrealtime();
+        for (int t = 0; t < ktiles; ++t) {
+            static_for<64>([&acc, &fa, &fb, &frag, a_lane, b_lane](auto gc) {
+                constexpr int gp = decltype(gc)::value;
+                (void)acc;
+                constexpr int ks = gp >> 4, idx = gp & 15, fn = idx >> 2, fm = idx & 3, cur = ks & 1;
+                if constexpr (idx < 8) {
+                    constexpr int f = idx & 3, nks = (ks + 1) & 3;
+                    if constexpr (idx < 4) fa[cur ^ 1][f] = frag(a_lane, nks, f);
+                    else fb[cur ^ 1][f] = frag(b_lane, nks, f);
+                }
+                asm volatile("v_mfma_f32_32x32x16_bf16 %[d], %[a], %[b], %[d]" : [d] "+a"(acc[fn][fm]) : [a] "v"(fa[cur][fn]), [b] "v"(fb[cur][fm]));
+            });
+        }
+        c1 = __builtin_amdgcn_s_memtime(); r1 = __builtin_amdgcn_s_memrealtime();
+#pragma unroll
+        for (int i = 0; i < 4; ++i)
+#pragma unroll
+            for (int j = 0; j < 4; ++j) asm volatile("" ::"a"(acc[i][j]));
+        sink[blockIdx.x * 256 + tid] = acc[0][0][0];
+    } else {
+        const int g = l >> 4, l15 = l & 15, rsw = (l15 >> 1) & 7;
+        const int lane_sw = (g ^ rsw) << 4;
+        const int a_lane = lds0 + (wn * 128 + l15) * 128 + lane_sw, b_lane = lds0 + UNIT + (wm * 128 + l15) * 128 + lane_sw;
+        auto frag = [&](int base, int ks, int f) {
+            return *reinterpret_cast<const __attribute__((address_space(3))) bf16x8*>((uintptr_t)(uint32_t)((base ^ (ks << 6)) + f * 2048));
+        };
+        f32x4 acc[8][8];
+#pragma unroll
+        for (int i = 0; i < 8; ++i)
+#pragma unroll
+            for (int j = 0; j < 8; ++j)
+#pragma unroll
+                for (int r = 0; r < 4; ++r) acc[i][j][r] = 0.f;
+        bf16x8 fa[2][8], fb[2][8];
+#pragma unroll
+        for (int f = 0; f < 8; ++f) { fa[0][f] = frag(a_lane, 0, f); fb[0][f] = frag(b_lane, 0, f); }
+        c0 = __builtin_amdgcn_s_memtime(); r0 = __builtin_amdgcn_s_memrealtime();
+        for (int t = 0; t < ktiles; ++t) {
+            static_for<128>([&acc, &fa, &fb, &frag, a_lane, b_lane](auto gc) {
+                constexpr int gp = decltype(gc)::value;
+                (void)acc;
+                constexpr int ks = gp >> 6, idx = gp & 63, fn = idx >> 3, fm = idx & 7, cur = ks & 1;
+                if constexpr (idx < 32 && (idx & 1) == 0) {
+                    constexpr int f = (idx >> 1) & 7, nks = (ks + 1) & 1;
+                    if constexpr (idx < 16) fa[cur ^ 1][f] = frag(a_lane, nks, f);
+                    else fb[cur ^ 1][f] = frag(b_lane, nks, f);
+                }
+                asm volatile("v_mfma_f32_16x16x32_bf16 %[d], %[a], %[b], %[d]" : [d] "+a"(acc[fn][fm]) : [a] "v"(fa[cur][fn]), [b] "v"(fb[cur][fm]));
+            });
+        }
+        c1 = __builtin_amdgcn_s_memtime(); r1 = __builtin_amdgcn_s_memrealtime();
+#pragma unroll
+        for (int i = 0; i < 8; ++i)
+#pragma unroll
+            for (int j = 0; j < 8; ++j) asm volatile("" ::"a"(acc[i][j]));
+        sink[blockIdx.x * 256 + tid] = acc[0][0][0];
+    }
+    if (tid == 0) { stamps[blockIdx.x * 2] = c1 - c0; stamps[blockIdx.x * 2 + 1] = r1 - r0; }
+}
+}
+
+extern "C" int dots_probe_mfma_shape(int shape, const uint32_t* mask, int words, int n_wg, int ktiles, float warm_seconds, int launches,
+                                     const void* src_dev, double* out) {
+    if ((shape != 0 && shape != 1) || n_wg < 1 || n_wg > 4096 || ktiles < 1 || launches < 1 || !src_dev || !out) return -1;
+    hipStream_t s = nullptr;
+    hipError_t e = hipSuccess;
+    if (mask && (e = hipExtStreamCreateWithCUMask(&s, (uint32_t)words, mask)) != hipSuccess) return (int)e;
+    float* sink = nullptr;
+    unsigned long long* stamps = nullptr;
+    hipEvent_t ea = nullptr, eb = nullptr;
+    int warm = 0;
+    float ms = 0.f;
+    std::vector<unsigned long long> h((size_t)n_wg * 2);
+    auto launch = [&]() {
+        if (shape == 0) hipLaunchKernelGGL(probe_shape_loop<0>, dim3(n_wg), dim3(256), 0, s, (const uint16_t*)src_dev, ktiles, sink, stamps);
+        else hipLaunchKernelGGL(probe_shape_loop<1>, dim3(n_wg), dim3(256), 0, s, (const uint16_t*)src_dev, ktiles, sink, stamps);
+    };
+    if ((e = hipMalloc(&sink, (size_t)n_wg * 256 * sizeof(float))) != hipSuccess) goto done;
+    if ((e = hipMalloc(&stamps, (size_t)n_wg * 16)) != hipSuccess) goto done;
+    if ((e = hipEventCreate(&ea)) != hipSuccess || (e = hipEventCreate(&eb)) != hipSuccess) goto done;
+    {
+        const auto t0 = std::chrono::steady_clock::now();
+        do {
+            for (int i = 0; i < 4; ++i) launch();
+            warm += 4;
+            if ((e = hipStreamSynchronize(s)) != hipSuccess) goto done;
+        } while (std::chrono::duration<float>(std::chrono::steady_clock::now() - t0).count() < warm_seconds && warm < 100000);
+    }
+    (void)hipEventRecord(ea, s);
+    for (int i = 0; i < launches; ++i) launch();
+    (void)hipEventRecord(eb, s);
+    if ((e = hipStreamSynchronize(s)) != hipSuccess) goto done;
+    (void)hipEventElapsedTime(&ms, ea, eb);
+    if ((e = hipMemcpy(h.data(), stamps, (size_t)n_wg * 16, hipMemcpyDeviceToHost)) != hipSuccess) goto done;
+    {
+        std::vector<double> cyc(n_wg), mhz(n_wg);
+        for (int i = 0; i < n_wg; ++i) { cyc[i] = (double)h[2 * i]; mhz[i] = h[2 * i + 1] ? (double)h[2 * i] / (double)h[2 * i + 1] * 100.0 : 0.0; }
+        std::nth_element(cyc.begin(), cyc.begin() + n_wg / 2, cyc.end());
+        std::nth_element(mhz.begin(), mhz.begin() + n_wg / 2, mhz.end());
+        out[0] = ms / launches; out[1] = cyc[n_wg / 2]; out[2] = mhz[n_wg / 2]; out[3] = warm;
+    }
+done:
+    if (ea) (void)hipEventDestroy(ea);
+    if (eb) (void)hipEventDestroy(eb);
+    if (sink) (void)hipFree(sink);
+    if (stamps) (void)hipFree(stamps);
+    if (s) (void)hipStreamDestroy(s);
+    return (int)e;
+}
diff --git a/dots_ocr_amd/engine.py b/dots_ocr_amd/engine.py
--- a/dots_ocr_amd/engine.py
+++ b/dots_ocr_amd/engine.py
@@ -322,6 +322,7 @@
         "dots_op_rmsnorm": (i32, [vp, vp, vp, vp, i64, i32, f32]),
         "dots_op_layernorm": (i32, [vp, vp, vp, vp, vp, i64, i32, f32]),
         "dots_op_gemm": (i32, [vp, vp, vp, vp, vp, vp, i64, i32, i32, i32, vp]),
+        "dots_op_gemm_lda": (i32, [vp, vp, vp, vp, vp, vp, i64, i32, i32, i32, i32, vp]),
         "dots_op_quant_fp8": (i32, [vp, vp, vp, i64, i32]),
         "dots_op_gemm_fp8": (i32, [vp, vp, vp, vp, vp, vp, i64, i32, i32, i32]),
         "dots_op_flash_attn": (i32, [vp, vp, vp, vp, vp, P(i32), i32, i32, i32, i32, f32]),
@@ -367,6 +368,7 @@
         "dots_op_logprobs": (i32, [vp, vp, i32, i32, i32, P(i32), vp, vp, vp, vp]),
         "dots_bench_logprobs": (i32, [vp, vp, i32, i32, i32, P(i32), i32, i32, P(f32)]),
         "dots_probe_mfma": (i32, [i32, vp, vp, vp, vp]),
+        "dots_probe_mfma_shape": (i32, [i32, P(C.c_uint32), i32, i32, i32, f32, i32, vp, P(C.c_double)]),
         "dots_probe_grid_barrier": (i32, [i32, i32, i32, i32, i32, P(f32), P(i32)]),
         "dots_probe_cu_mask": (i32, [P(C.c_uint32), i32, i32, i32, i32, P(C.c_uint32)]),
     }
@@ -383,9 +385,9 @@
     "dots_set_eos", "dots_slots_prefill", "dots_slots_decode", "dots_slots_poll", "dots_slot_read", "dots_slot_release", "dots_kv_pool_info", "dots_slot_capacity", "dots_slots_reset",
     "dots_set_next_tokens", "dots_get_last_tokens", "dots_get_stats", "dots_synchronize", "dots_debug_capture_hidden",
     "dots_debug_read_hidden", "dots_dev_alloc",
-    "dots_dev_free", "dots_memcpy_h2d", "dots_memcpy_d2h", "dots_op_rmsnorm", "dots_op_layernorm", "dots_op_gemm", "dots_op_quant_fp8", "dots_op_gemm_fp8",
+    "dots_dev_free", "dots_memcpy_h2d", "dots_memcpy_d2h", "dots_op_rmsnorm", "dots_op_layernorm", "dots_op_gemm", "dots_op_gemm_lda", "dots_op_quant_fp8", "dots_op_gemm_fp8",
     "dots_op_flash_attn", "dots_plan_flash_xcd", "dots_op_qkv_rope_split", "dots_op_qkv_proj_rope", "dots_op_dec_qkv", "dots_op_decode_attn", "dots_op_dec_proj", "dots_op_dec_gateup",
-    "dots_op_dec_lmhead", "dots_probe_mfma", "dots_probe_grid_barrier", "dots_probe_cu_mask",
+    "dots_op_dec_lmhead", "dots_probe_mfma", "dots_probe_mfma_shape", "dots_probe_grid_barrier", "dots_probe_cu_mask",
     "dots_set_kv_scales", "dots_debug_read_kv", "dots_op_dec_qkv_kv8", "dots_op_decode_attn_kv8",
     "dots_set_row_sampling", "dots_op_select_tokens", "dots_bench_select_tokens",
     "dots_set_row_logprobs", "dots_row_logprobs", "dots_op_logprobs", "dots_bench_logprobs",
@@ -1063,6 +1065,9 @@
     def op_gemm(self, A, W, bias, residual, Cout, M, N, K, epilogue=EPI_NONE, colscale=None):
         self._ck(self.lib.dots_op_gemm(self.h, A, W, bias or None, residual or None, Cout, M, N, K, epilogue, colscale or None), "dots_op_gemm")
 
+    def op_gemm_lda(self, A, W, bias, residual, Cout, M, N, K, lda, epilogue=EPI_NONE, colscale=None):
+        self._ck(self.lib.dots_op_gemm_lda(self.h, A, W, bias or None, residual or None, Cout, M, N, K, lda, epilogue, colscale or None), "dots_op_gemm_lda")
+
     def op_gemm_fp8(self, A, W, bias, residual, Cout, M, N, K, epilogue=EPI_NONE):
         self._ck(self.lib.dots_op_gemm_fp8(self.h, A, W, bias or None, residual or None, Cout, M, N, K, epilogue), "dots_op_gemm_fp8")
 
diff --git a/include/dots_ocr_hip.h b/include/dots_ocr_hip.h
--- a/include/dots_ocr_hip.h
+++ b/include/dots_ocr_hip.h
@@ -178,6 +178,8 @@
                       int64_t rows, int dim, float eps);
 int dots_op_gemm(DotsEngine* e, const void* A_dev, const void* W_dev, const void* bias_dev,
                  const void* residual_dev, void* C_dev, int64_t M, int N, int K, int epilogue, const float* colscale_dev);
+int dots_op_gemm_lda(DotsEngine* e, const void* A_dev, const void* W_dev, const void* bias_dev,
+                     const void* residual_dev, void* C_dev, int64_t M, int N, int K, int lda, int epilogue, const float* colscale_dev);
 int dots_op_quant_fp8(DotsEngine* e, void* w_inout_dev, float* scale_out_dev, int64_t N, int K);
 int dots_op_gemm_fp8(DotsEngine* e, const void* A_dev, const void* W_dev, const void* bias_dev, const void* residual_dev, void* C_dev,
                      int64_t M, int N, int K, int epilogue);
@@ -235,6 +237,8 @@
                         float* ms_out);
 
 int dots_probe_mfma(int which, const void* A, const void* Bt, void* D, void* stream);
+int dots_probe_mfma_shape(int shape, const uint32_t* mask, int words, int n_wg, int ktiles, float warm_seconds, int launches,
+                          const void* src_dev, double* out);
 int dots_probe_grid_barrier(int n_wg, int threads, int n_barriers, int mode, int lds_bytes, float* ms_out, int32_t* stats_out);
 int dots_probe_cu_mask(const uint32_t* mask, int words, int n_wg, int threads, int lds_bytes, uint32_t* ids_out_host);
 
```

New measurement: 6.369 pages/s (median of 6 runs). No clear change (+0.6%).
